# MichaelAxtmann/InPlaceMSDradixsort

Measured on AMD Instinct MI355X. Metric: Gkeys/s + achieved HBM GB/s, 2^30 uniform u32 keys, 1/2/4/8 MI355X, higher is better.
Workload: dtype u32; 1 GPU; 2^30 uniform u32 keys per GPU, in-place MSD radix sort, 8-bit digits; config_id=c2, elements_per_gpu=1073741824, steps_verified=0, verified_by=not checked in a plain run (bench.py --full verifies every timed step), workspace_bytes=360054784

## Files before the change

### inplacemsdradixsort_amd/csrc/msd_device.hpp

```cpp
#pragma once

#include <hip/hip_runtime.h>
#include <stdint.h>

namespace msd {

constexpr int kP = 256;
constexpr uint32_t kXBase = 0x80000000u;
constexpr uint32_t kNoOwner = 0xFFFFFFFFu;
constexpr uint32_t kRposStride = 32;

struct NoVal {};
typedef uint32_t u32x4 __attribute__((ext_vector_type(4)));

template <typename V> struct has_val { static constexpr bool value = true; };
template <> struct has_val<NoVal> { static constexpr bool value = false; };

template <typename K, typename V> struct Cfg;
template <> struct Cfg<uint32_t, NoVal> {
	static constexpr int B = 64, T = 4096, TH = 1024;
	static constexpr int SORT_TH = 1024, SORT_KPT = 24;
};
template <> struct Cfg<uint64_t, NoVal> {
	static constexpr int B = 32, T = 4096, TH = 1024;
	static constexpr int SORT_TH = 1024, SORT_KPT = 17;
};
template <> struct Cfg<uint64_t, uint64_t> {
	static constexpr int B = 32, T = 2048, TH = 1024;
#ifndef MSD_PAIR_LEAF_TH
#define MSD_PAIR_LEAF_TH 512
#endif
	static constexpr int SORT_TH = MSD_PAIR_LEAF_TH, SORT_KPT = 6;
};

struct Parent {
	uint64_t start, count;
	uint32_t shift;
	uint32_t width;
	uint32_t child_base;
	uint32_t stripe_lo, stripe_hi;
	uint32_t pad;
};

struct Stripe {
	uint64_t begin, end;
	uint64_t lo_base;
	uint32_t parent;
	uint32_t slot_lo, slot_hi;
	uint32_t pad;
};

struct Segment {
	uint64_t start, count;
	uint32_t bits;
	uint32_t pad;
};

struct ListEntry {
	uint32_t slot;
	uint32_t owner;
};

struct Counters {
	uint32_t nholes;
	uint32_t hole_cursor;
	uint32_t next_parents;
	uint32_t nsmall;
	uint32_t errors;
	uint32_t chain_steps;
	uint32_t ncount;
	uint32_t nfallback;
	uint32_t nbig;
	uint32_t count_ticket;
	uint32_t direct_uneven;
	uint32_t nslow;
	uint32_t count_ticket2;
	uint32_t nevict;
	uint32_t leaf_ticket[2];
	uint32_t count_ticket3;
	uint32_t nslow16;
	uint32_t next_max;
	uint32_t rp_children;
	uint32_t nhot;
	uint32_t nslow2;
	uint32_t count_ticket4;
	uint32_t l17_slow;
	uint32_t err_sites;
	uint32_t nexcess;
};
__device__ __forceinline__ void msd_note_error(Counters *ctr, uint32_t site)
{
	atomicAdd(&ctr->errors, 1u);
	atomicOr(&ctr->err_sites, 1u << site);
}
static_assert(sizeof(Counters) % 8 == 0, "the words behind the counters are used for 64-bit atomics");

#ifdef MSD_STAMPS
__device__ unsigned long long g_stamps[2][16];
#define MSD_STAMP_DECL(id)                          \
	constexpr bool kStampThis = MSD_STAMPS == (id); \
	unsigned long long st_acc[12] = {}, st_last = 0
#define MSD_STAMP_START()                                                                              \
	do {                                                                                            \
		if constexpr (kStampThis) {                                                             \
			__builtin_amdgcn_sched_barrier(0);                                              \
			asm volatile("s_memtime %0\n\ts_waitcnt lgkmcnt(0)" : "=s"(st_last)::"memory"); \
			__builtin_amdgcn_sched_barrier(0);                                              \
		}                                                                                       \
	} while (0)
#define MSD_STAMP(i)                                                                                    \
	do {                                                                                            \
		if constexpr (kStampThis) {                                                             \
			unsigned long long now_;                                                        \
			__builtin_amdgcn_sched_barrier(0);                                              \
			asm volatile("s_memtime %0\n\ts_waitcnt lgkmcnt(0)" : "=s"(now_)::"memory");    \
			__builtin_amdgcn_sched_barrier(0);                                              \
			st_acc[i] += now_ - st_last;                                                    \
			st_last = now_;                                                                 \
		}                                                                                       \
	} while (0)
#define MSD_STAMP_TICK(i)                            \
	do {                                         \
		if constexpr (kStampThis) st_acc[i] += 1; \
	} while (0)
#define MSD_STAMP_FLUSH(nwaves)                                                                         \
	do {                                                                                            \
		if constexpr (kStampThis) {                                                             \
			const unsigned wv_ = threadIdx.x >> 6;                                          \
			if ((threadIdx.x & 63) == 0 && (wv_ == 0 || wv_ == (nwaves) - 1)) {            \
				for (int i_ = 0; i_ < 12; ++i_) atomicAdd(&g_stamps[wv_ ? 1 : 0][i_], st_acc[i_]); \
			}                                                                               \
		}                                                                                       \
	} while (0)
#else
#define MSD_STAMP_DECL(id)
#define MSD_STAMP_START() do {} while (0)
#define MSD_STAMP(i) do {} while (0)
#define MSD_STAMP_TICK(i) do {} while (0)
#define MSD_STAMP_FLUSH(nwaves) do {} while (0)
#endif


template <typename K> __device__ __forceinline__ uint32_t digit_of(K key, uint32_t shift, uint32_t mask)
{
	return (uint32_t)(key >> shift) & mask;
}

__device__ __forceinline__ uint32_t lane_id() { return threadIdx.x & 63; }

__device__ __forceinline__ uint32_t wave_incl_scan(uint32_t v)
{
	v += (uint32_t)__builtin_amdgcn_update_dpp(0, (int)v, 0x111, 0xf, 0xf, false);
	v += (uint32_t)__builtin_amdgcn_update_dpp(0, (int)v, 0x112, 0xf, 0xf, false);
	v += (uint32_t)__builtin_amdgcn_update_dpp(0, (int)v, 0x114, 0xf, 0xf, false);
	v += (uint32_t)__builtin_amdgcn_update_dpp(0, (int)v, 0x118, 0xf, 0xf, false);
	v += (uint32_t)__builtin_amdgcn_update_dpp(0, (int)v, 0x142, 0xa, 0xf, false);
	v += (uint32_t)__builtin_amdgcn_update_dpp(0, (int)v, 0x143, 0xc, 0xf, false);
	return v;
}
__device__ __forceinline__ uint64_t wave_incl_scan64(uint64_t v)
{
#pragma unroll
	for (int o = 1; o < 64; o <<= 1) {
		uint64_t t = __shfl_up(v, o);
		if ((int)lane_id() >= o) v += t;
	}
	return v;
}

__device__ __forceinline__ uint32_t popc_below_lane(uint64_t m)
{
	return __builtin_amdgcn_mbcnt_hi((uint32_t)(m >> 32), __builtin_amdgcn_mbcnt_lo((uint32_t)m, 0u));
}
__device__ __forceinline__ bool lane_bit(uint64_t m)
{
	const uint32_t lane = threadIdx.x & 63u;
	const uint32_t half = lane < 32u ? (uint32_t)m : (uint32_t)(m >> 32);
	return (half >> (lane & 31u)) & 1u;
}

__device__ __forceinline__ uint32_t block_excl_scan256(uint32_t v, uint32_t *tmp, uint32_t &total)
{
	const uint32_t tid = threadIdx.x;
	if (tid >= 256) v = 0;
	uint32_t inc = wave_incl_scan(v);
	if (tid < 256 && lane_id() == 63) tmp[tid >> 6] = inc;
	__syncthreads();
	uint32_t base = 0;
	if (tid < 256) {
		const uint32_t w = tid >> 6;
		if (w > 0) base += tmp[0];
		if (w > 1) base += tmp[1];
		if (w > 2) base += tmp[2];
	}
	total = tmp[0] + tmp[1] + tmp[2] + tmp[3];
	__syncthreads();
	return base + inc - v;
}
__device__ __forceinline__ uint64_t block_excl_scan256_64(uint64_t v, uint64_t *tmp, uint64_t &total)
{
	const uint32_t tid = threadIdx.x;
	if (tid >= 256) v = 0;
	uint64_t inc = wave_incl_scan64(v);
	if (tid < 256 && lane_id() == 63) tmp[tid >> 6] = inc;
	__syncthreads();
	uint64_t base = 0;
	if (tid < 256) {
		const uint32_t w = tid >> 6;
		if (w > 0) base += tmp[0];
		if (w > 1) base += tmp[1];
		if (w > 2) base += tmp[2];
	}
	total = tmp[0] + tmp[1] + tmp[2] + tmp[3];
	__syncthreads();
	return base + inc - v;
}

template <typename K> struct Vec16;
template <> struct Vec16<uint32_t> { static constexpr int N = 4; };
template <> struct Vec16<uint64_t> { static constexpr int N = 2; };


struct DirectPlan {
	uint32_t est_cnt[kP];
	uint32_t bound[kP + 1];
	uint32_t adj_seen, adj_same;
};

template <typename K>
__global__ __launch_bounds__(256) void direct_sample_kernel(const K *__restrict__ keys, const Parent *__restrict__ parents,
	DirectPlan *__restrict__ plan, uint32_t every)
{
	__shared__ uint32_t h[kP];
	const Parent pa = parents[0];
	const uint32_t mask = (1u << pa.width) - 1u;
	h[threadIdx.x] = 0;
	uint32_t seen = 0, same = 0;
	__syncthreads();
	const uint64_t nruns = pa.count / 256;
	const uint64_t step = (uint64_t)gridDim.x * every;
	for (uint64_t r = (uint64_t)blockIdx.x * every; r < nruns; r += 4 * step) {
		K k4[4];
#pragma unroll
		for (int u = 0; u < 4; ++u)
			if (r + u * step < nruns) k4[u] = keys[pa.start + (r + u * step) * 256 + threadIdx.x];
#pragma unroll
		for (int u = 0; u < 4; ++u) {
			if (r + u * step < nruns) {
				const uint32_t d = digit_of(k4[u], pa.shift, mask);
				atomicAdd(&h[d], 1u);
				if (u == 0 && (blockIdx.x & 7u) == 0) {
					same += __popcll(__ballot(d == (uint32_t)__shfl_down((int)d, 1) && (threadIdx.x & 63) != 63));
					seen += 63;
				}
			}
		}
	}
	__syncthreads();
	if (h[threadIdx.x]) atomicAdd(&plan->est_cnt[threadIdx.x], h[threadIdx.x]);
	if ((threadIdx.x & 63) == 0 && seen) {
		atomicAdd(&plan->adj_seen, seen);
		atomicAdd(&plan->adj_same, same);
	}
}

template <typename K>
__global__ __launch_bounds__(1024) void direct_hist_kernel(const K *__restrict__ keys, const Stripe *__restrict__ stripes,
	const Parent *__restrict__ parents, DirectPlan *__restrict__ plans,
	unsigned long long *__restrict__ vres)
{
	constexpr int VEC = Vec16<K>::N;
	K v_or = 0, v_and = ~(K)0;
	auto seen_key = [&](K k) {
		v_or |= k;
		v_and &= k;
		return k;
	};
	__shared__ uint32_t h[kP];
	const Stripe st = stripes[blockIdx.x];
	const Parent pa = parents[st.parent];
	const uint32_t shift = pa.shift, mask = (1u << pa.width) - 1u, tid = threadIdx.x;
	if (tid < kP) h[tid] = 0;
	uint32_t seen = 0, same = 0;
	__syncthreads();
	const uint64_t a0 = (st.begin + VEC - 1) / VEC * VEC, a1 = st.end / VEC * VEC;
	if (a0 < a1) {
		for (uint64_t i = st.begin + tid; i < a0; i += 1024) atomicAdd(&h[digit_of(seen_key(keys[i]), shift, mask)], 1u);
		const uint32_t nvec = (uint32_t)((a1 - a0) / VEC);
		const K *kp = keys + a0;
		constexpr int U = 8;
		for (uint32_t v = tid; v < nvec; v += U * 1024) {
			K kk[U][VEC];
#pragma unroll
			for (int u = 0; u < U; ++u) {
				const uint32_t vv = min(v + (uint32_t)u * 1024u, nvec - 1u);
				if constexpr (sizeof(K) == 4) {
					const u32x4 q = __builtin_nontemporal_load(reinterpret_cast<const u32x4 *>(kp + (size_t)vv * VEC));
					kk[u][0] = q.x; kk[u][1] = q.y; kk[u][2] = q.z; kk[u][3] = q.w;
				} else {
					const u32x4 q = __builtin_nontemporal_load(reinterpret_cast<const u32x4 *>(kp + (size_t)vv * VEC));
					kk[u][0] = (K)q.x | ((K)q.y << 32); kk[u][1] = (K)q.z | ((K)q.w << 32);
				}
			}
#pragma unroll
			for (int u = 0; u < U; ++u) {
				if (v + (uint32_t)u * 1024u < nvec) {
#pragma unroll
					for (int e = 0; e < VEC; ++e) atomicAdd(&h[digit_of(seen_key(kk[u][e]), shift, mask)], 1u);
					seen += 1;
					same += digit_of(kk[u][0], shift, mask) == digit_of(kk[u][VEC - 1], shift, mask) ? 1u : 0u;
				}
			}
		}
		for (uint64_t i = a1 + tid; i < st.end; i += 1024) atomicAdd(&h[digit_of(seen_key(keys[i]), shift, mask)], 1u);
	} else
		for (uint64_t i = st.begin + tid; i < st.end; i += 1024) atomicAdd(&h[digit_of(seen_key(keys[i]), shift, mask)], 1u);
	__syncthreads();
	if (tid < kP && h[tid]) atomicAdd(&plans[st.parent].est_cnt[tid], h[tid]);
	if (vres) {
		unsigned long long o = (unsigned long long)v_or, a = (unsigned long long)v_and | (sizeof(K) == 4 ? 0xFFFFFFFF00000000ull : 0ull);
#pragma unroll
		for (int s = 32; s > 0; s >>= 1) {
			o |= __shfl_xor(o, s);
			a &= __shfl_xor(a, s);
		}
		if ((tid & 63) == 0) {
			atomicOr(&vres[0], o);
			atomicAnd(&vres[1], a);
		}
	}
#pragma unroll
	for (int o = 32; o > 0; o >>= 1) {
		seen += (uint32_t)__shfl_xor((int)seen, o);
		same += (uint32_t)__shfl_xor((int)same, o);
	}
	if ((tid & 63) == 0 && seen) {
		atomicAdd(&plans[st.parent].adj_seen, seen);
		atomicAdd(&plans[st.parent].adj_same, same);
	}
}

template <int B>
__global__ __launch_bounds__(256) void direct_plan_kernel(const Parent *__restrict__ parents, DirectPlan *__restrict__ plans,
	Counters *__restrict__ ctr)
{
	__shared__ uint64_t tmp[8];
	__shared__ uint32_t s_mn, s_mx;
	const Parent pa = parents[blockIdx.x];
	DirectPlan *plan = plans + blockIdx.x;
	const uint32_t d = threadIdx.x;
	if (d == 0) {
		s_mn = 0xFFFFFFFFu;
		s_mx = 0;
	}
	const uint64_t s0 = (pa.start + B - 1) / B, s1 = (pa.start + pa.count) / B;
	uint64_t total;
	const uint64_t c = plan->est_cnt[d];
	const uint64_t ex = block_excl_scan256_64(c, tmp, total);
	const uint64_t ns = s1 > s0 ? s1 - s0 : 0;
	plan->bound[d] = (uint32_t)(s0 + (total ? ex * ns / total : (uint64_t)d * ns / kP));
	if (d == 0) plan->bound[kP] = (uint32_t)s1;
	if (d < (1u << pa.width)) {
		atomicMin(&s_mn, (uint32_t)c);
		atomicMax(&s_mx, (uint32_t)c);
	}
	__syncthreads();
	const bool runs = (uint64_t)plan->adj_same * 8u > plan->adj_seen;
#ifndef MSD_UNEVEN_PCT
#define MSD_UNEVEN_PCT 125
#endif
	if (d == 0 && (runs || !(s_mn > 0 && (double)s_mx * 100.0 <= (double)MSD_UNEVEN_PCT * (double)s_mn))) atomicAdd(&ctr->direct_uneven, 1u);
}

__device__ __forceinline__ bool wave_select_smallest(uint32_t v, bool elig, int need, uint64_t &mask_out)
{
	uint64_t cand = __ballot(elig), selm = 0;
	if ((int)__popcll(cand) > need) {
#pragma unroll
		for (int bit = 9; bit >= 0; --bit) {
			const uint64_t zeros = cand & ~__ballot((v >> bit) & 1u);
			const int cz = __popcll(zeros);
			if (cz >= need)
				cand = zeros;
			else {
				selm |= zeros;
				need -= cz;
				cand &= ~zeros;
			}
		}
		const bool mine = lane_bit(cand) && (int)popc_below_lane(cand) < need;
		selm |= __ballot(mine);
	} else
		selm = cand;
	mask_out = selm;
	return lane_bit(selm);
}

}
#include "msd_direct.hpp"
#include "msd_stream2.hpp"
namespace msd {


struct ChildArrays {
	uint64_t *start;
	uint64_t *count;
// ... 615 lines not shown
		for (int i = 0; i < NI; ++i) {
			const int chain = i * BPI + (int)(lane / LPB);
			const uint32_t s = __shfl(src_safe, chain);
			kd[i] = *reinterpret_cast<const u32x4 *>(slot_ptr<K, B>(keys, xkeys, s) + sub * VEC);
			if constexpr (HV)
				vd[i] = *reinterpret_cast<const u32x4 *>(slot_ptr<uint64_t, B>(vals, xvals, s) + sub * VEC);
		}
#pragma unroll
		for (int i = 0; i < NI; ++i) {
			const int chain = i * BPI + (int)(lane / LPB);
			const uint32_t hdst = __shfl(hole, chain);
			if ((mv >> chain) & 1ull) {
				*reinterpret_cast<u32x4 *>(slot_ptr<K, B>(keys, xkeys, hdst) + sub * VEC) = kd[i];
				if constexpr (HV)
					*reinterpret_cast<u32x4 *>(slot_ptr<uint64_t, B>(vals, xvals, hdst) + sub * VEC) = vd[i];
			}
		}
		if (active && !retry) {
			if (last)
				active = false;
			else {
				hole = src;
				owner = src_owner;
				om = nom;
				ofl = nfl;
			}
		}
		MSD_STAMP(4);
	}
	MSD_STAMP_FLUSH(4);
	if (lane == 0 && steps) atomicAdd(&ctr->chain_steps, steps);
}

__device__ __forceinline__ void chains_verify(const ChildArrays &ca, uint32_t ci, uint32_t flags, Counters *ctr)
{
	const uint32_t len = (uint32_t)ca.list_len[ci], hot = flags >> 8;
	if (!hot) {
		if (ca.rpos[(size_t)ci * kRposStride] != len) msd_note_error(ctr, 3u);
		return;
	}
	const uint32_t nint = ca.n_int[ci];
	for (uint32_t sh = 0; sh < kHotShards; ++sh) {
		const uint32_t sb = (uint32_t)((uint64_t)nint * sh / kHotShards), se = (uint32_t)((uint64_t)nint * (sh + 1) / kHotShards);
		if (ca.hot_cur[(size_t)((hot - 1) * kHotShards + sh) * kRposStride] < se - sb) msd_note_error(ctr, 4u);
	}
	if (ca.rpos[(size_t)ci * kRposStride] != len - nint) msd_note_error(ctr, 5u);
}


template <int B>
__device__ __forceinline__ uint64_t fringe_pos(uint64_t start, uint32_t is, uint32_t I, uint64_t o)
{
	if (I == 0) return start + o;
	const uint64_t head = (uint64_t)is * B - start;
	return o < head ? start + o : (uint64_t)(is + I) * B + (o - head);
}

template <typename K, typename V>
__global__ __launch_bounds__(256) void cleanup_kernel(const Stripe *__restrict__ stripes,
	const Parent *__restrict__ parents, const uint32_t *__restrict__ lo_cnt,
	const uint32_t *__restrict__ lo_off, const uint32_t *__restrict__ lo_dst, ChildArrays ca,
	const K *__restrict__ lo_keys, const uint64_t *__restrict__ lo_vals,
	K *__restrict__ keys, uint64_t *__restrict__ vals,
	const K *__restrict__ xkeys, const uint64_t *__restrict__ xvals, Counters *__restrict__ ctr)
{
	constexpr int B = Cfg<K, V>::B;
	constexpr bool HV = has_val<V>::value;
	__shared__ uint32_t s_off[kP + 1], s_dst[kP], s_is[kP], s_I[kP], s_ex[kP], s_nex;
	__shared__ uint64_t s_start[kP];
	const Stripe st = stripes[blockIdx.x];
	const Parent pa = parents[st.parent];
	const uint32_t tid = threadIdx.x, W = 1u << pa.width;
	const bool first = blockIdx.x == pa.stripe_lo;
	const size_t so = (size_t)blockIdx.x * kP + tid;
	s_off[tid] = lo_off[so];
	s_dst[tid] = lo_dst[so];
	if (tid == kP - 1) s_off[kP] = lo_off[so] + lo_cnt[so];
	if (tid == 0) s_nex = 0;
	if (tid < W) {
		s_is[tid] = ca.is[pa.child_base + tid];
		s_I[tid] = ca.I[pa.child_base + tid];
		s_start[tid] = ca.start[pa.child_base + tid];
	}
	__syncthreads();
	if (first && tid < W) {
		const uint32_t fl = ca.flags[pa.child_base + tid];
		chains_verify(ca, pa.child_base + tid, fl, ctr);
		if (fl & 2u) s_ex[atomicAdd(&s_nex, 1u)] = tid;
	}
	{
		constexpr uint32_t LG = 32, NB = 4, NG = 256 / LG;
		const uint32_t grp = tid / LG, l = tid % LG;
		for (uint32_t d0 = grp; d0 < kP; d0 += NG * NB) {
			K k[NB];
			uint64_t v[NB];
			uint32_t off[NB], cnt[NB];
#pragma unroll
			for (uint32_t q = 0; q < NB; ++q) {
				const uint32_t d = d0 + q * NG;
				off[q] = s_off[d];
				cnt[q] = s_off[d + 1] - off[q];
				if (l < cnt[q]) {
					k[q] = lo_keys[st.lo_base + off[q] + l];
					if constexpr (HV) v[q] = lo_vals[st.lo_base + off[q] + l];
				}
			}
#pragma unroll
			for (uint32_t q = 0; q < NB; ++q) {
				const uint32_t d = d0 + q * NG;
				if (l < cnt[q]) {
					const uint64_t p = fringe_pos<B>(s_start[d], s_is[d], s_I[d], (uint64_t)s_dst[d] + l);
					keys[p] = k[q];
					if constexpr (HV) vals[p] = v[q];
				}
			}
#pragma unroll
			for (uint32_t q = 0; q < NB; ++q) {
				const uint32_t d = d0 + q * NG;
				for (uint32_t j = l + LG; j < cnt[q]; j += LG) {
					const uint64_t p = fringe_pos<B>(s_start[d], s_is[d], s_I[d], (uint64_t)s_dst[d] + j);
					keys[p] = lo_keys[st.lo_base + off[q] + j];
					if constexpr (HV) vals[p] = lo_vals[st.lo_base + off[q] + j];
				}
			}
		}
		static_assert(kP % (NG * NB) == 0, "every bucket has its half-wave");
	}
	if (!first) return;
	__syncthreads();
	const uint32_t nex = s_nex;
	if (tid == 0 && nex) atomicAdd(&ctr->nexcess, nex);
	for (uint32_t e = tid / B; e < nex; e += 256 / B) {
		const uint32_t d = s_ex[e], ci = pa.child_base + d, j = tid % B;
		const uint64_t p = fringe_pos<B>(s_start[d], s_is[d], s_I[d], (uint64_t)ca.lsum[ci] + j);
		keys[p] = xkeys[(uint64_t)(2 * ci + 1) * B + j];
		if constexpr (HV) vals[p] = xvals[(uint64_t)(2 * ci + 1) * B + j];
	}
}

enum Route : int { kRouteDone = -1, kRouteSmall = 0, kRouteCount = 1, kRouteBig = 2, kRouteNext = 3 };
__host__ __device__ inline Route route_child(uint64_t count, uint32_t bits, uint32_t stop_bits, uint32_t count_bits, uint64_t small_max,
	uint64_t med_max, bool has_big)
{
	if (count <= 1 || bits <= stop_bits) return kRouteDone;
	const bool countable = bits <= count_bits;
	if (countable && count >= 64 && count <= med_max) return kRouteCount;
	if (count > small_max) return has_big && countable && count < 0xFFFF0000ull ? kRouteBig : kRouteNext;
	return kRouteSmall;
}

__global__ __launch_bounds__(256) void collect_kernel(const Parent *__restrict__ parents, uint32_t nparents, uint32_t wmax, ChildArrays ca,
	uint64_t small_max, uint64_t med_max, uint32_t small_cap, uint32_t count_bits, Segment *__restrict__ next_parents,
	Segment *__restrict__ small, Segment *__restrict__ small_count, Segment *__restrict__ big, uint32_t big_cap,
	Counters *__restrict__ ctr, uint64_t *__restrict__ count_out, uint32_t count_n, uint32_t stop_bits)
{
	__shared__ uint32_t s_n[4], s_base[4], s_max;
	const uint32_t tid = threadIdx.x;
	if (tid < 4) s_n[tid] = 0;
	if (tid == 0) s_max = 0;
	__syncthreads();
	const uint32_t pi = blockIdx.x * (256u >> wmax) + (tid >> wmax), d = tid & ((1u << wmax) - 1u);
	int which = -1;
	uint32_t rank = 0;
	Segment s = {};
	if (pi < nparents) {
		const Parent pa = parents[pi];
		if (d < (1u << pa.width)) {
			const uint32_t ci = pa.child_base + d;
			const uint64_t c = ca.count[ci];
			if (count_out && ci < count_n) count_out[ci] = c;
			which = route_child(c, pa.shift, stop_bits, count_bits, small_max, med_max, big != nullptr);
			if (which >= 0) {
				s.start = ca.start[ci];
				s.count = c;
				s.bits = pa.shift;
				s.pad = 0;
				rank = atomicAdd(&s_n[which], 1u);
				if (which == 3) atomicMax(&s_max, (uint32_t)(c < 0xFFFFFFFFull ? c : 0xFFFFFFFFull));
			}
		}
	}
	__syncthreads();
	if (tid < 4 && s_n[tid]) {
		uint32_t *cnt = tid == 0 ? &ctr->nsmall : tid == 1 ? &ctr->ncount : tid == 2 ? &ctr->nbig : &ctr->next_parents;
		s_base[tid] = atomicAdd(cnt, s_n[tid]);
		if (tid == 3) atomicMax(&ctr->next_max, s_max);
	}
	__syncthreads();
	if (which < 0) return;
	uint32_t at = s_base[which] + rank;
	if (which == 2 && at >= big_cap) {
		which = 3;
		at = atomicAdd(&ctr->next_parents, 1u);
		atomicMax(&ctr->next_max, (uint32_t)(s.count < 0xFFFFFFFFull ? s.count : 0xFFFFFFFFull));
	}
	if (which == 3)
		next_parents[at] = s;
	else if (which == 2)
		big[at] = s;
	else if (at < small_cap)
		(which == 0 ? small : small_count)[at] = s;
	else
		msd_note_error(ctr, 6u);
}

}
#include "msd_regpart.hpp"
namespace msd {


constexpr int kCountTh = 1024;
constexpr int kCountMaxBits = 16;
#ifndef MSD_COUNT_MED_LOG
#define MSD_COUNT_MED_LOG 17
#endif
constexpr uint64_t kCountMedMax = 1ull << MSD_COUNT_MED_LOG;
constexpr size_t kCountCwBytes = (((size_t)1 << kCountMaxBits) / 4 + ((size_t)1 << kCountMaxBits) / 128 + 4) * 4;
constexpr int kCountStageBytes = 14080;
constexpr size_t kCountLds = kCountCwBytes + kCountStageBytes + 128;
__device__ __forceinline__ uint32_t cw_at(uint32_t i) { return i + (i >> 5); }

template <typename K>
__global__ __launch_bounds__(kCountTh, 8) void count_place_kernel(K *__restrict__ keys,
	const Segment *__restrict__ segs, uint32_t nsegs_host, const uint32_t *__restrict__ nsegs_dev,
	Segment *__restrict__ slow, Counters *__restrict__ ctr)
{
	const uint32_t nsegs = nsegs_dev ? *nsegs_dev : nsegs_host;
	constexpr int PF = sizeof(K) == 4 ? 17 : 9;
	extern __shared__ __attribute__((aligned(16))) unsigned char smem[];
	uint32_t *cw = reinterpret_cast<uint32_t *>(smem);
	uint32_t *tbase = reinterpret_cast<uint32_t *>(smem + kCountCwBytes);
	K *out = reinterpret_cast<K *>(smem);
	uint32_t *wtot = reinterpret_cast<uint32_t *>(smem + kCountCwBytes + kCountStageBytes);
	uint32_t *nexti = wtot + 17;
	K *hi_l = reinterpret_cast<K *>(wtot + 18);
	uint32_t *crowded = wtot + 21;
	static_assert((size_t)PF * kCountTh * sizeof(K) <= kCountCwBytes + kCountStageBytes, "output buffer");
	const uint32_t tid = threadIdx.x, lane = tid & 63, w = tid >> 6;
	if (blockIdx.x >= nsegs) return;
	Segment sg = segs[blockIdx.x];
	K pk[PF];
	auto prefetch = [&](const Segment &g) {
		const K *src = keys + g.start;
		const uint32_t cnt = g.count <= (uint64_t)(PF * kCountTh) ? (uint32_t)g.count : 1u;
#pragma unroll
		for (int u = 0; u < PF; ++u) {
			const uint32_t idx = min((uint32_t)(u * kCountTh) + tid, cnt - 1u);
			pk[u] = src[idx];
		}
	};
	prefetch(sg);
	MSD_STAMP_DECL(2);
	MSD_STAMP_START();
	for (;;) {
		const uint32_t n = (uint32_t)sg.count;
		const uint32_t nv = 1u << sg.bits, mask = nv - 1u;
		const uint32_t nwords = nv >= 4 ? nv / 4 : 1;
		K *seg = keys + sg.start;
		const bool in_regs = n <= (uint32_t)(PF * kCountTh);
		MSD_STAMP(9);
		MSD_STAMP_TICK(11);

		if (in_regs)
			for (uint32_t j = tid; j < cw_at(nwords) + 1; j += kCountTh) cw[j] = 0;
		if (tid == 0) {
			*nexti = atomicAdd(&ctr->count_ticket, 1u) + gridDim.x;
			*crowded = 0;
			*hi_l = pk[0] & ~(K)mask;
		}
		MSD_STAMP(0);
		__syncthreads();
		MSD_STAMP(1);
		uint32_t rk[PF];
		if (in_regs) {
#pragma unroll
			for (int u = 0; u < PF; ++u) {
				const uint32_t left = n > (uint32_t)(u * kCountTh) ? n - u * kCountTh : 0u;
				rk[u] = 0;
				if (tid < left) {
					const uint32_t v = (uint32_t)pk[u] & mask, sh = (v & 3u) * 8u;
					rk[u] = v | (((atomicAdd(&cw[cw_at(v >> 2)], 1u << sh) >> sh) & 0xFFu) << 16);
				}
			}
		}
		MSD_STAMP(2);
		__syncthreads();
		MSD_STAMP(3);
		const uint32_t nxt = *nexti;
		const K hi = *hi_l;
		const uint32_t wpt = nwords >= kCountTh ? nwords / kCountTh : 1;
		const uint32_t w0 = tid * wpt;
		uint32_t *cww = cw + cw_at(w0);
		uint32_t tot = 0;
		if (in_regs && w0 < nwords) {
#pragma unroll 4
			for (uint32_t j = 0; j < wpt; ++j) tot = __builtin_amdgcn_sad_u8(cww[j], 0u, tot);
		}
		if (tot > 255u) *crowded = 1;
		const uint32_t inc = wave_incl_scan(tot);
		if (lane == 63) wtot[w] = inc;
		MSD_STAMP(4);
		__syncthreads();
		uint32_t pos = inc - tot, all = 0;
#pragma unroll 2
		for (uint32_t ww = 0; ww < kCountTh / 64; ++ww) {
			const uint32_t t = wtot[ww];
			if (ww < w) pos += t;
			all += t;
		}
		const bool ok = in_regs && all == n && *crowded == 0;
		MSD_STAMP(5);
		if (ok) {
			uint32_t run = 0;
			if (w0 < nwords) {
#pragma unroll 4
				for (uint32_t j = 0; j < wpt; ++j) {
					const uint32_t x = cww[j], y = x * 0x01010101u;
					cww[j] = (y - x) + run * 0x01010101u;
					run += y >> 24;
				}
			}
			tbase[tid] = pos;
			MSD_STAMP(6);
			__syncthreads();
			const uint32_t lgw = (uint32_t)__builtin_ctz(wpt);
#pragma unroll
			for (int u = 0; u < PF; ++u) {
				const uint32_t left = n > (uint32_t)(u * kCountTh) ? n - u * kCountTh : 0u;
				if (tid < left) {
					const uint32_t v = rk[u] & 0xFFFFu, wi = v >> 2;
					rk[u] += (tbase[wi >> lgw] + ((cw[cw_at(wi)] >> ((v & 3u) * 8u)) & 0xFFu)) << 16;
				}
			}
			MSD_STAMP(7);
			__syncthreads();
#pragma unroll
			for (int u = 0; u < PF; ++u) {
				const uint32_t left = n > (uint32_t)(u * kCountTh) ? n - u * kCountTh : 0u;
				if (tid < left) out[rk[u] >> 16] = hi | (K)(rk[u] & 0xFFFFu);
			}
			__syncthreads();
			MSD_STAMP(8);
		} else if (tid == 0)
			slow[atomicAdd(&ctr->nslow, 1u)] = sg;
		Segment nsg = sg;
		if (nxt < nsegs) {
			nsg = segs[nxt];
			prefetch(nsg);
		}
		if (ok) {
			for (uint32_t i = tid; i < n; i += kCountTh) seg[i] = out[i];
		}
		MSD_STAMP(10);
		if (nxt >= nsegs) break;
		sg = nsg;
		__syncthreads();
	}
	MSD_STAMP_FLUSH(kCountTh / 64);
}

template <typename K>
__global__ __launch_bounds__(kCountTh, 8) void count_walk_kernel(K *__restrict__ keys,
	const Segment *__restrict__ segs, const uint32_t *__restrict__ nsegs_dev, Segment *__restrict__ fallback,
	uint32_t fallback_base, uint32_t lds_cap, Segment *__restrict__ big, uint32_t big_cap, Counters *__restrict__ ctr)
{
	constexpr uint32_t WS = kCountStageBytes / sizeof(K);
	extern __shared__ __attribute__((aligned(16))) unsigned char smem[];
	uint32_t *cw = reinterpret_cast<uint32_t *>(smem);
	K *stage = reinterpret_cast<K *>(smem + kCountCwBytes);
	uint32_t *wtot = reinterpret_cast<uint32_t *>(smem + kCountCwBytes + kCountStageBytes);
	uint32_t *nexti = wtot + 17;
	K *hi_l = reinterpret_cast<K *>(wtot + 18);
	uint32_t *tfree = wtot + 20;
	const uint32_t tid = threadIdx.x, lane = tid & 63, w = tid >> 6;
	const uint32_t nsegs = *nsegs_dev;
	if (blockIdx.x >= nsegs) return;
	Segment sg = segs[blockIdx.x];
	for (;;) {
		const uint32_t n = (uint32_t)sg.count;
		const uint32_t nv = 1u << sg.bits, mask = nv - 1u;
		const uint32_t nwords = nv >= 4 ? nv / 4 : 1;
		K *seg = keys + sg.start;

		for (uint32_t j = tid; j < cw_at(nwords) + 1; j += kCountTh) cw[j] = 0;
		if (tid == 0) {
			*nexti = atomicAdd(&ctr->count_ticket2, 1u) + gridDim.x;
			*hi_l = seg[0] & ~(K)mask;
		}
		__syncthreads();
		constexpr int LB = 16 / (int)sizeof(K) * 4;
		for (uint32_t i0 = 0; i0 < n; i0 += LB * kCountTh) {
			K kb[LB];
#pragma unroll
			for (int u = 0; u < LB; ++u) kb[u] = seg[min(i0 + u * kCountTh + tid, n - 1u)];
#pragma unroll
			for (int u = 0; u < LB; ++u) {
				if (i0 + u * kCountTh + tid < n) {
					const uint32_t v = (uint32_t)kb[u] & mask;
					atomicAdd(&cw[cw_at(v >> 2)], 1u << ((v & 3u) * 8u));
				}
			}
		}
		__syncthreads();
		const uint32_t nxt = *nexti;
		const K hi = *hi_l;
		const uint32_t wpt = nwords >= kCountTh ? nwords / kCountTh : 1;
		const uint32_t w0 = tid * wpt;
		const uint32_t *cwp = cw + cw_at(w0);
		uint32_t tot = 0;
		uint64_t nz = 0;
		if (w0 < nwords) {
#pragma unroll 4
			for (uint32_t j = 0; j < wpt; ++j) {
				const uint32_t x = cwp[j];
				tot = __builtin_amdgcn_sad_u8(x, 0u, tot);
				const uint32_t hb = (x | ((x & 0x7F7F7F7Fu) + 0x7F7F7F7Fu)) & 0x80808080u;
				nz |= (uint64_t)((((hb >> 7) * 0x01020408u) >> 24) & 0xFu) << (4u * j);
			}
		}
		const uint32_t inc = wave_incl_scan(tot);
		if (lane == 63) wtot[w] = inc;
		__syncthreads();
		uint32_t pos = inc - tot, all = 0;
#pragma unroll 2
		for (uint32_t ww = 0; ww < kCountTh / 64; ++ww) {
			const uint32_t t = wtot[ww];
			if (ww < w) pos += t;
			all += t;
		}
		if (all != n) {
			if (tid == 0) {
				if (n <= lds_cap) {
					const uint32_t at = atomicAdd(&ctr->nfallback, 1u);
					fallback[fallback_base + at] = sg;
				} else {
					const uint32_t at = big ? atomicAdd(&ctr->nbig, 1u) : 0xFFFFFFFFu;
					if (at < big_cap) big[at] = sg; else msd_note_error(ctr, 7u);
				}
			}
		} else {
			const uint32_t end = pos + tot;
			const K hi4 = hi | (K)(w0 * 4u);
			uint32_t c = 0;
			K cur = 0;
			K *cwk = reinterpret_cast<K *>(cw);
			auto window = [&](uint32_t wbeg, uint32_t wend) -> uint32_t {
				if (pos <= wend && wend < end) *tfree = tid;
				while (pos < end && pos < wend) {
					if (c == 0) {
						const uint32_t i = (uint32_t)__ffsll((long long)nz) - 1u;
						nz &= nz - 1;
						c = (cwp[i >> 2] >> (8u * (i & 3u))) & 0xFFu;
						cur = hi4 + (K)i;
					}
					const uint32_t r = pos - wbeg;
					if (r < WS) stage[r]= cur; else cwk[r - WS] = cur;
					++pos;
					--c;
				}
				__syncthreads();
				const uint32_t tf = *tfree;
				for (uint32_t i = tid; i < wend - wbeg; i += kCountTh) seg[wbeg + i] = i < WS ? stage[i] : cwk[i - WS];
				__syncthreads();
				return (uint32_t)(cw_at(tf * wpt) * 4u / sizeof(K));
			};
			uint32_t wbeg = 0, wend = WS < n ? WS : n;
			for (;;) {
				const uint32_t room = window(wbeg, wend);
				if (wend >= n) break;
				wbeg = wend;
				wend = wbeg + WS + room < n ? wbeg + WS + room : n;
			}
		}
		if (nxt >= nsegs) break;
		sg = segs[nxt];
		__syncthreads();
	}
}

}
#include "msd_count16.hpp"
#include "msd_merge16.hpp"
#include "msd_scatter16.hpp"
namespace msd {


constexpr int kLeafCountBits = 14;
template <typename K, typename V> struct LeafBits {
	static constexpr int value = (sizeof(K) == 8 && (!has_val<V>::value || Cfg<K, V>::SORT_TH < 1024)) ? 13 : kLeafCountBits;
};
template <typename K, typename V> struct LeafCountLds {
	static constexpr int CAP = Cfg<K, V>::SORT_TH * Cfg<K, V>::SORT_KPT;
	static constexpr size_t bytes = (size_t)CAP * (sizeof(K) + (has_val<V>::value ? 8 : 0)) +
					((size_t)1 << LeafBits<K, V>::value) * 2 + 192;
};

template <typename K, typename V>
__global__ __launch_bounds__((Cfg<K, V>::SORT_TH)) void leaf_count_sort_kernel(K *__restrict__ keys,
	uint64_t *__restrict__ vals, const Segment *__restrict__ segs, uint32_t nsegs,
	Segment *__restrict__ fallback, Counters *__restrict__ ctr, uint32_t *__restrict__ ticket,
	const uint32_t *__restrict__ nsegs_dev)
{
	if (nsegs_dev) nsegs = *nsegs_dev;
	using C = Cfg<K, V>;
	constexpr bool HV = has_val<V>::value;
	constexpr int TH = C::SORT_TH, KPT = C::SORT_KPT, CAP = TH * KPT, LB = LeafBits<K, V>::value;
	extern __shared__ __attribute__((aligned(16))) unsigned char smem[];
	K *xk = reinterpret_cast<K *>(smem);
	uint64_t *xv = reinterpret_cast<uint64_t *>(smem + (size_t)CAP * sizeof(K));
	uint32_t *cw = reinterpret_cast<uint32_t *>(smem + (size_t)CAP * (sizeof(K) + (HV ? 8 : 0)));
	uint32_t *wtot = cw + ((size_t)1 << LB) / 2;
	K *s_or = reinterpret_cast<K *>(wtot + 32);
	if (blockIdx.x >= nsegs) return;
	const uint32_t tid = threadIdx.x, lane = tid & 63, w = tid >> 6;
	Segment sg = segs[blockIdx.x];
	K kr[KPT];
	uint64_t vr[HV ? KPT : 1];
	auto prefetch = [&](const Segment &g) {
		const uint32_t cnt = (uint32_t)g.count;
#pragma unroll
		for (int i = 0; i < KPT; ++i) {
			if ((uint32_t)(i * TH) < cnt) {
				const uint32_t idx = min((uint32_t)(i * TH) + tid, cnt - 1u);
				kr[i] = keys[g.start + idx];
				if constexpr (HV) vr[i] = vals[g.start + idx];
			}
		}
	};
	prefetch(sg);
	if (tid == 0) wtot[19] = 0;
	MSD_STAMP_DECL(3);
	MSD_STAMP_START();
	for (;;) {
		MSD_STAMP(9);
		MSD_STAMP_TICK(11);
		const uint32_t n = (uint32_t)sg.count;
#ifndef MSD_LEAF_NARROW
#define MSD_LEAF_NARROW 1
#endif
		const bool narrow = MSD_LEAF_NARROW && sg.bits <= (uint32_t)LB;
		K k_or = 0, k_and = ~(K)0;
		if (!narrow) {
#pragma unroll
			for (int i = 0; i < KPT; ++i) {
				if ((uint32_t)(i * TH) + tid < n) {
					k_or |= kr[i];
					k_and &= kr[i];
				}
			}
		}
		if (tid == 0) {
			s_or[0] = 0;
			s_or[1] = ~(K)0;
			wtot[16] = 0;
			if (wtot[19] == 0) {
				const uint32_t take = nsegs > 64u * gridDim.x ? 4u : 1u;
				wtot[18] = atomicAdd(ticket, take) + gridDim.x;
				wtot[19] = take;
			}
			wtot[17] = wtot[18];
			wtot[18] += 1;
			wtot[19] -= 1;
		}
		for (uint32_t j = tid; j < ((uint32_t)1 << LB) / 2; j += TH) cw[j] = 0;
		MSD_STAMP(0);
		__syncthreads();
		if (!narrow) {
#pragma unroll
			for (int o = 32; o > 0; o >>= 1) {
				k_or |= __shfl_xor(k_or, o);
				k_and &= __shfl_xor(k_and, o);
			}
			if (lane == 0) {
				if constexpr (sizeof(K) == 4) {
					atomicOr(reinterpret_cast<unsigned int *>(&s_or[0]), (unsigned int)k_or);
					atomicAnd(reinterpret_cast<unsigned int *>(&s_or[1]), (unsigned int)k_and);
				} else {
					atomicOr(reinterpret_cast<unsigned long long *>(&s_or[0]), (unsigned long long)k_or);
					atomicAnd(reinterpret_cast<unsigned long long *>(&s_or[1]), (unsigned long long)k_and);
				}
			}
			__syncthreads();
		}
		MSD_STAMP(1);
		const uint32_t nxt = wtot[17];
		const Segment nraw = segs[nxt < nsegs ? nxt : blockIdx.x];
		const K openmask = sg.bits >= sizeof(K) * 8 ? ~(K)0 : (((K)1 << sg.bits) - 1);
		const K vopen = narrow ? openmask : (s_or[0] ^ s_or[1]) & openmask;
		Segment nsg = sg;
		bool fetched = false;
		if (vopen != 0) {
			const uint32_t nbits = (uint32_t)(64 - __builtin_clzll((unsigned long long)vopen));
			const uint32_t shift = nbits > (uint32_t)LB ? nbits - LB : 0;
			const uint32_t mask = (1u << (nbits - shift)) - 1u;
			uint32_t rk[KPT];
#pragma unroll
			for (int i = 0; i < KPT; ++i) {
				rk[i] = 0;
				if ((uint32_t)(i * TH) + tid < n) {
					const uint32_t v = (uint32_t)(kr[i] >> shift) & mask, sh = 16u * (v & 1u);
					rk[i] = (atomicAdd(&cw[v >> 1], 1u << sh) >> sh) & 0xFFFFu;
				}
			}
			MSD_STAMP(2);
			__syncthreads();
			constexpr uint32_t WPT = (((uint32_t)1 << LB) / 2) / TH;
			static_assert(WPT >= 1, "counter words per thread");
			const uint32_t w0 = tid * WPT;
			uint32_t tot = 0;
#pragma unroll
			for (uint32_t j = 0; j < WPT; ++j) {
				const uint32_t x = cw[w0 + j];
				tot += (x & 0xFFFFu) + (x >> 16);
			}
			const uint32_t inc = wave_incl_scan(tot);
			if (lane == 63) wtot[w] = inc;
			__syncthreads();
			uint32_t run = inc - tot;
			for (uint32_t ww = 0; ww < w; ++ww) run += wtot[ww];
#pragma unroll
			for (uint32_t j = 0; j < WPT; ++j) {
				const uint32_t x = cw[w0 + j];
				const uint32_t lo = x & 0xFFFFu, hi = x >> 16;
				cw[w0 + j] = run | ((run + lo) << 16);
				run += lo + hi;
			}
			MSD_STAMP(3);
			__syncthreads();
#pragma unroll
			for (int i = 0; i < KPT; ++i) {
				if ((uint32_t)(i * TH) + tid < n) {
					const uint32_t v = (uint32_t)(kr[i] >> shift) & mask;
					const uint32_t p = ((cw[v >> 1] >> (16u * (v & 1u))) & 0xFFFFu) + rk[i];
					xk[p] = kr[i];
					if constexpr (HV) xv[p] = vr[i];
				}
			}
			MSD_STAMP(4);
			if (nxt < nsegs) {
				nsg = nraw;
				prefetch(nsg);
				fetched = true;
			}
			MSD_STAMP(5);
			__syncthreads();
			bool bad = false;
			const K lowmask = shift ? ((K)1 << shift) - 1 : (K)0;
			const bool groups = shift && (vopen & lowmask) != 0;
			constexpr uint32_t kMaxGroup = 48;
			const K glim = (K)1 << shift;
			if (groups) {
				bool too_long = false;
				for (uint32_t i = tid; i + kMaxGroup < n; i += TH)
					if ((K)(xk[i] ^ xk[i + kMaxGroup]) < glim) too_long = true;
				if (too_long) wtot[16] = 1;
				__syncthreads();
				bad = wtot[16] != 0;
				if (bad && tid == 0) fallback[atomicAdd(&ctr->nfallback, 1u)] = sg;
			}
			MSD_STAMP(6);
			if (!bad && groups) {
				constexpr uint32_t WIN = 3;
#pragma unroll 1
				for (uint32_t idx = tid; idx < n; idx += TH) {
					const K me = xk[idx];
					K lk[WIN], rkk[WIN];
#pragma unroll
					for (uint32_t d = 0; d < WIN; ++d) {
						lk[d] = xk[idx > d ? idx - d - 1 : 0u];
						rkk[d] = xk[min(idx + d + 1, n - 1u)];
					}
					uint32_t left = 0, before = 0, right = 0;
					bool ml = true, mr = true;
#pragma unroll
					for (uint32_t d = 0; d < WIN; ++d) {
						ml = ml && idx > d && (K)(lk[d] ^ me) < glim;
						before += ml && lk[d] <= me ? 1u : 0u;
						left += ml ? 1u : 0u;
						mr = mr && idx + d + 1 < n && (K)(rkk[d] ^ me) < glim;
						before += mr && rkk[d] < me ? 1u : 0u;
						right += mr ? 1u : 0u;
					}
					if (ml) {
						while (idx > left) {
							const K o = xk[idx - left - 1];
							if ((K)(o ^ me) >= glim) break;
							before += o <= me ? 1u : 0u;
							++left;
						}
					}
					if (mr) {
						for (uint32_t e = idx + right + 1; e < n; ++e) {
							const K o = xk[e];
							if ((K)(o ^ me) >= glim) break;
							before += o < me ? 1u : 0u;
						}
					}
					const uint64_t at = sg.start + idx - left + before;
					keys[at] = me;
					if constexpr (HV) vals[at] = xv[idx];
				}
			} else if (!bad) {
				for (uint32_t idx = tid; idx < n; idx += TH) {
					keys[sg.start + idx] = xk[idx];
					if constexpr (HV) vals[sg.start + idx] = xv[idx];
				}
			}
		}
		MSD_STAMP(7);
		if (nxt >= nsegs) break;
		if (!fetched) {
			nsg = nraw;
			prefetch(nsg);
		}
		sg = nsg;
		__syncthreads();
	}
	MSD_STAMP_FLUSH(TH / 64);
}

}
#include "msd_leaf17.hpp"
#include "msd_bigcount.hpp"
namespace msd {

__global__ __launch_bounds__(256) void round_init_kernel(Counters *__restrict__ ctr, uint32_t *__restrict__ plan_words,
	uint64_t nplan_words, unsigned long long *__restrict__ scan_state, uint64_t ntiles, uint32_t *__restrict__ scan_ctr,
	const uint32_t *__restrict__ staged, uint32_t *__restrict__ parents_out, uint64_t parent_words,
	uint32_t *__restrict__ stripes_out, uint64_t stripe_words, Counters *__restrict__ park)
{
	const uint64_t i0 = (uint64_t)blockIdx.x * 256 + threadIdx.x, step = (uint64_t)gridDim.x * 256;
	if (i0 == 0) {
		if (park) *park = *ctr;
		ctr->nholes = 0;
		ctr->hole_cursor = 0;
		ctr->next_parents = 0;
		ctr->nevict = 0;
		ctr->direct_uneven = 0;
		ctr->next_max = 0;
		ctr->rp_children = 0;
		ctr->nhot = 0;
		scan_ctr[0] = scan_ctr[1] = scan_ctr[2] = scan_ctr[3] = 0;
	}
	for (uint64_t i = i0; i < nplan_words; i += step) plan_words[i] = 0;
	for (uint64_t i = i0; i < ntiles; i += step) scan_state[i] = 0;
	if (staged) {
		for (uint64_t i = i0; i < parent_words; i += step) parents_out[i] = staged[i];
		for (uint64_t i = i0; i < stripe_words; i += step) stripes_out[i] = staged[parent_words + i];
	}
}


template <typename K, typename V>
__global__ __launch_bounds__((Cfg<K, V>::SORT_TH)) void lds_sort_kernel(K *__restrict__ keys,
	uint64_t *__restrict__ vals, const Segment *__restrict__ segs, uint32_t nsegs,
	const uint32_t *__restrict__ nsegs_dev)
{
	using C = Cfg<K, V>;
	constexpr bool HV = has_val<V>::value;
	constexpr int TH = C::SORT_TH, KPT = C::SORT_KPT, NW = TH / 64, CAP = TH * KPT;
	if (nsegs_dev) nsegs = *nsegs_dev;
	for (uint32_t sgi = blockIdx.x; sgi < nsegs; sgi += gridDim.x) {
	__syncthreads();
	extern __shared__ __attribute__((aligned(16))) unsigned char smem[];
	K *xk = reinterpret_cast<K *>(smem);
	uint64_t *xv = reinterpret_cast<uint64_t *>(smem + (size_t)CAP * sizeof(K));
	uint32_t *wcnt = reinterpret_cast<uint32_t *>(smem + (size_t)CAP * sizeof(K) + (HV ? (size_t)CAP * 8 : 0));
	uint32_t *dbase = wcnt + NW * kP;
	uint32_t *tmp = dbase + kP;
	K *s_or = reinterpret_cast<K *>(tmp + 8);

	const Segment sg = segs[sgi];
	const uint32_t n = (uint32_t)sg.count;
	const uint32_t tid = threadIdx.x, lane = tid & 63, w = tid >> 6;
	const int nitems = (int)((n + TH - 1) / TH);
	const uint32_t wbase = w * (uint32_t)nitems * 64;
	const uint64_t lt_mask = (1ull << lane) - 1ull;

	K kr[KPT];
	uint64_t vr[HV ? KPT : 1];
	K k_or = 0, k_and = ~(K)0;
#pragma unroll
	for (int i = 0; i < KPT; ++i) {
		kr[i] = ~(K)0;
		if constexpr (HV) vr[i] = 0;
		if (i < nitems) {
			const uint32_t idx = wbase + i * 64 + lane;
			if (idx < n) {
				kr[i] = keys[sg.start + idx];
				if constexpr (HV) vr[i] = vals[sg.start + idx];
				k_or |= kr[i];
				k_and &= kr[i];
			}
		}
	}
	if (tid == 0) { s_or[0] = 0; s_or[1] = ~(K)0; }
	__syncthreads();
#pragma unroll
	for (int o = 32; o > 0; o >>= 1) {
		k_or |= __shfl_xor(k_or, o);
		k_and &= __shfl_xor(k_and, o);
	}
	if (lane == 0) {
		if constexpr (sizeof(K) == 4) {
			atomicOr(reinterpret_cast<unsigned int *>(&s_or[0]), (unsigned int)k_or);
			atomicAnd(reinterpret_cast<unsigned int *>(&s_or[1]), (unsigned int)k_and);
		} else {
			atomicOr(reinterpret_cast<unsigned long long *>(&s_or[0]), (unsigned long long)k_or);
			atomicAnd(reinterpret_cast<unsigned long long *>(&s_or[1]), (unsigned long long)k_and);
		}
	}
	__syncthreads();
	const K vary = s_or[0] ^ s_or[1];
	__syncthreads();

	uint32_t *mycnt = wcnt + w * kP;
	bool in_lds = false;
	const K openmask = sg.bits >= sizeof(K) * 8 ? ~(K)0 : (((K)1 << sg.bits) - 1);
	const K vopen = vary & openmask;
	const uint32_t nbits = vopen ? (uint32_t)(64 - __builtin_clzll((unsigned long long)vopen)) : 0u;
	const uint32_t first_shift = nbits > 24 ? nbits - 16 : 0;
	bool msd_mode = first_shift != 0;
	for (uint32_t shift = first_shift; shift < nbits; shift += 8) {
		const uint32_t width = nbits - shift < 8 ? nbits - shift : 8;
		const uint32_t mask = (1u << width) - 1u;
		if (((uint32_t)(vary >> shift) & mask) == 0) continue;
		for (uint32_t j = tid; j < NW * kP; j += TH) wcnt[j] = 0;
		__syncthreads();
		uint32_t rk[(KPT + 1) / 2];
#pragma unroll
		for (int i = 0; i < KPT; ++i) {
			if (i < nitems) {
				const uint32_t d = digit_of(kr[i], shift, mask);
				uint32_t plo = ~0u, phi = ~0u;
#pragma unroll
				for (int b = 0; b < 8; ++b) {
					const uint32_t bit = (d >> b) & 1u;
					const uint64_t m = __ballot(bit != 0);
					const uint32_t ext = bit - 1u;
					plo &= (uint32_t)m ^ ext;
					phi &= (uint32_t)(m >> 32) ^ ext;
				}
				const uint32_t below = __popc(plo & (uint32_t)lt_mask) + __popc(phi & (uint32_t)(lt_mask >> 32));
				const uint32_t old = mycnt[d];
				if (below == 0) mycnt[d] = old + __popc(plo) + __popc(phi);
				const uint32_t r = old + below;
				if (i & 1) rk[i / 2] |= r << 16; else rk[i / 2] = r;
			}
			__builtin_amdgcn_sched_barrier(0);
		}
		__syncthreads();
		uint32_t tot_d = 0;
		if (tid < kP) {
#pragma unroll
			for (int ww = 0; ww < NW; ++ww) {
				const uint32_t t = wcnt[ww * kP + tid];
				wcnt[ww * kP + tid] = tot_d;
				tot_d += t;
			}
		}
		uint32_t gt;
		const uint32_t ex = block_excl_scan256(tot_d, tmp, gt);
		if (tid < kP) dbase[tid] = ex;
		__syncthreads();
#pragma unroll
		for (int i = 0; i < KPT; ++i) {
			if (i < nitems) {
				const uint32_t d = digit_of(kr[i], shift, mask);
				const uint32_t r = (i & 1) ? rk[i / 2] >> 16 : rk[i / 2] & 0xFFFFu;
				const uint32_t p = dbase[d] + mycnt[d] + r;
				xk[p] = kr[i];
				if constexpr (HV) xv[p] = vr[i];
			}
		}
		__syncthreads();
		in_lds = true;
		bool more = false;
		for (uint32_t s2 = shift + 8; s2 < nbits; s2 += 8) {
			const uint32_t w2 = nbits - s2 < 8 ? nbits - s2 : 8;
			if (((uint32_t)(vary >> s2) & ((1u << w2) - 1u)) != 0) more = true;
		}
		if (!more && msd_mode) {
			const K lowmask = ((K)1 << first_shift) - 1;
			if (tid == 0) tmp[0] = 0;
			__syncthreads();
			bool too_long = false;
			if ((vary & lowmask) != 0) {
				for (uint32_t i = tid; i < n; i += TH) {
					const K hi = xk[i] >> first_shift;
					if ((i == 0 || (xk[i - 1] >> first_shift) != hi) && i + 1 < n && (xk[i + 1] >> first_shift) == hi) {
						uint32_t e = i + 2;
						while (e < n && (xk[e] >> first_shift) == hi) ++e;
						if (e - i > 48) {
							too_long = true;
// ... 61 lines not shown
	const uint32_t parts = 1u << radix_bits, mask = parts - 1u;
	for (uint32_t j = threadIdx.x; j < parts; j += 256) h[j] = 0;
	__syncthreads();
	constexpr int VEC = Vec16<K>::N;
	const uint64_t nvec = n / VEC;
	const uint64_t stride = (uint64_t)gridDim.x * 256;
	for (uint64_t v = (uint64_t)blockIdx.x * 256 + threadIdx.x; v < nvec; v += stride) {
		if constexpr (sizeof(K) == 4) {
			const uint4 q = reinterpret_cast<const uint4 *>(keys)[v];
			atomicAdd(&h[(q.x >> shift) & mask], 1u);
			atomicAdd(&h[(q.y >> shift) & mask], 1u);
			atomicAdd(&h[(q.z >> shift) & mask], 1u);
			atomicAdd(&h[(q.w >> shift) & mask], 1u);
		} else {
			const ulonglong2 q = reinterpret_cast<const ulonglong2 *>(keys)[v];
			atomicAdd(&h[(uint32_t)(q.x >> shift) & mask], 1u);
			atomicAdd(&h[(uint32_t)(q.y >> shift) & mask], 1u);
		}
	}
	if (blockIdx.x == 0)
		for (uint64_t i = nvec * VEC + threadIdx.x; i < n; i += 256)
			atomicAdd(&h[(uint32_t)(keys[i] >> shift) & mask], 1u);
	__syncthreads();
	for (uint32_t j = threadIdx.x; j < parts; j += 256)
		if (h[j]) atomicAdd(&count[j], (unsigned long long)h[j]);
}


constexpr int kScanTh = 256, kScanIpt = 8, kScanTile = kScanTh * kScanIpt;
constexpr uint64_t kFlagAgg = 1ull << 62, kFlagPre = 2ull << 62, kFlagMask = 3ull << 62;

__global__ __launch_bounds__(kScanTh) void scan_lookback_kernel(const uint64_t *__restrict__ in,
	uint64_t *__restrict__ out, uint64_t n, unsigned long long *__restrict__ tile_state,
	uint32_t *__restrict__ tile_counter, uint32_t *__restrict__ err)
{
	__shared__ uint64_t tmp[8];
	__shared__ uint32_t s_tile;
	__shared__ uint64_t s_prefix;
	const uint32_t tid = threadIdx.x;
	if (tid == 0) s_tile = atomicAdd(tile_counter, 1u);
	__syncthreads();
	const uint32_t tile = s_tile;
	const uint64_t base = (uint64_t)tile * kScanTile + (uint64_t)tid * kScanIpt;
	uint64_t v[kScanIpt], sum = 0;
#pragma unroll
	for (int i = 0; i < kScanIpt; ++i) {
		v[i] = base + i < n ? in[base + i] : 0;
		sum += v[i];
	}
	uint64_t agg;
	const uint64_t tex = block_excl_scan256_64(sum, tmp, agg);
	if (tid == 0) {
		uint64_t prefix = 0;
		if (tile == 0) {
			__hip_atomic_store(&tile_state[0], kFlagPre | agg, __ATOMIC_RELAXED, __HIP_MEMORY_SCOPE_AGENT);
		} else {
			__hip_atomic_store(&tile_state[tile], kFlagAgg | agg, __ATOMIC_RELAXED, __HIP_MEMORY_SCOPE_AGENT);
			uint32_t t = tile - 1;
			uint32_t spins = 0;
			for (;;) {
				const uint64_t s = __hip_atomic_load(&tile_state[t], __ATOMIC_RELAXED, __HIP_MEMORY_SCOPE_AGENT);
				const uint64_t f = s & kFlagMask;
				if (f == 0) {
					if (++spins > (1u << 26)) {
						atomicAdd(err, 1u);
						break;
					}
					__builtin_amdgcn_s_sleep(1);
					continue;
				}
				prefix += s & ~kFlagMask;
				if (f == kFlagPre) break;
				--t;
			}
			__hip_atomic_store(&tile_state[tile], kFlagPre | (prefix + agg), __ATOMIC_RELAXED, __HIP_MEMORY_SCOPE_AGENT);
		}
		s_prefix = prefix;
	}
	__syncthreads();
	uint64_t run = s_prefix + tex;
#pragma unroll
	for (int i = 0; i < kScanIpt; ++i) {
		if (base + i < n) out[base + i] = run;
		run += v[i];
	}
}


struct GatherRun {
	uint64_t src, dst, len;
	uint32_t first_chunk;
	uint32_t pad;
};
#ifndef MSD_GATHER_CHUNK
#define MSD_GATHER_CHUNK 2048
#endif
constexpr uint32_t kGatherChunk = MSD_GATHER_CHUNK;

template <typename K>
__global__ __launch_bounds__(256) void gather_runs_kernel(K *__restrict__ dst, const K *__restrict__ src,
	const GatherRun *__restrict__ runs, uint32_t nruns, uint32_t nchunks, const uint32_t *__restrict__ coarse)
{
	constexpr int VEC = 16 / (int)sizeof(K);
	for (uint32_t c = blockIdx.x; c < nchunks; c += gridDim.x) {
		uint32_t lo = coarse[c >> 6], hi = min(coarse[(c >> 6) + 1] + 1u, nruns);
		while (hi - lo > 1) {
			const uint32_t mid = (lo + hi) >> 1;
			if (runs[mid].first_chunk <= c) lo = mid; else hi = mid;
		}
		const GatherRun r = runs[lo];
		const uint64_t off = (uint64_t)(c - r.first_chunk) * kGatherChunk;
		const uint32_t len = (uint32_t)(r.len - off < (uint64_t)kGatherChunk ? r.len - off : (uint64_t)kGatherChunk);
		K *d = dst + r.dst + off;
		const K *s = src + r.src + off;
		const uint32_t lead = min(len, (uint32_t)((VEC - (int)(((uintptr_t)d / sizeof(K)) % VEC)) % VEC));
		const uint32_t nvec = (len - lead) / VEC, tail0 = lead + nvec * VEC;
		if (threadIdx.x < lead) d[threadIdx.x] = s[threadIdx.x];
		if (tail0 + threadIdx.x < len) d[tail0 + threadIdx.x] = s[tail0 + threadIdx.x];
		const uint32_t kw = (uint32_t)(((uintptr_t)(s + lead) & 15u) >> 2);
		const u32x4 *sa = reinterpret_cast<const u32x4 *>(reinterpret_cast<const unsigned char *>(s + lead) - 4u * kw);
		u32x4 *dv = reinterpret_cast<u32x4 *>(d + lead);
		const bool last_lane = (threadIdx.x & 63u) == 63u;
#ifndef MSD_GATHER_NF
#define MSD_GATHER_NF 2
#endif
		constexpr int NF = MSD_GATHER_NF;
		for (uint32_t q0 = 0; q0 < nvec; q0 += NF * 256) {
			const uint32_t q = q0 + threadIdx.x;
			u32x4 a[NF], nx[NF];
#pragma unroll
			for (int u = 0; u < NF; ++u) {
				const uint32_t qq = min(q + u * 256u, kw ? nvec : nvec - 1u);
				a[u] = sa[qq];
				if (kw && last_lane) nx[u] = sa[min(qq + 1u, nvec)];
			}
#pragma unroll
			for (int u = 0; u < NF; ++u) {
				u32x4 o = a[u];
				if (kw) {
					const uint32_t sx = (uint32_t)__shfl_down((int)a[u].x, 1), sy = (uint32_t)__shfl_down((int)a[u].y, 1),
						       sz = (uint32_t)__shfl_down((int)a[u].z, 1);
					const uint32_t bx = last_lane ? nx[u].x : sx, by = last_lane ? nx[u].y : sy, bz = last_lane ? nx[u].z : sz;
					o = kw == 1 ? u32x4{ a[u].y, a[u].z, a[u].w, bx } : kw == 2 ? u32x4{ a[u].z, a[u].w, bx, by } : u32x4{ a[u].w, bx, by, bz };
				}
				if (q + u * 256u < nvec) dv[q + u * 256u] = o;
			}
		}
	}
}


template <typename K>
__global__ __launch_bounds__(256) void vary_kernel(const K *__restrict__ keys, uint64_t n, uint64_t stride,
	unsigned long long *__restrict__ res)
{
	K o = 0, a = ~(K)0;
	const uint64_t cnt = (n + stride - 1) / stride;
	const uint64_t step = (uint64_t)gridDim.x * 256, t0 = (uint64_t)blockIdx.x * 256 + threadIdx.x;
	if (stride == 1) {
		constexpr int VEC = 16 / (int)sizeof(K);
		const uint64_t lead = min(n, (uint64_t)((VEC - (int)(((uintptr_t)keys / sizeof(K)) % VEC)) % VEC));
		const uint64_t nvec = (n - lead) / VEC;
		const u32x4 *v = reinterpret_cast<const u32x4 *>(keys + lead);
		auto take = [&](const u32x4 &q) {
			if constexpr (sizeof(K) == 4) {
				o |= (K)(q.x | q.y | q.z | q.w);
				a &= (K)(q.x & q.y & q.z & q.w);
			} else {
				const K k0 = (K)q.x | ((K)q.y << 32), k1 = (K)q.z | ((K)q.w << 32);
				o |= k0 | k1;
				a &= k0 & k1;
			}
		};
		uint64_t i = t0;
		for (; i + 3 * step < nvec; i += 4 * step) {
			const u32x4 q0 = __builtin_nontemporal_load(v + i), q1 = __builtin_nontemporal_load(v + i + step);
			const u32x4 q2 = __builtin_nontemporal_load(v + i + 2 * step), q3 = __builtin_nontemporal_load(v + i + 3 * step);
			take(q0); take(q1); take(q2); take(q3);
		}
		for (; i < nvec; i += step) take(__builtin_nontemporal_load(v + i));
		const uint64_t tail0 = lead + nvec * VEC;
		if (t0 < lead) {
			o |= keys[t0];
			a &= keys[t0];
		}
		if (tail0 + t0 < n) {
			o |= keys[tail0 + t0];
			a &= keys[tail0 + t0];
		}
	} else
		for (uint64_t i = t0; i < cnt; i += step) {
			const K k = keys[i * stride];
			o |= k;
			a &= k;
		}
#pragma unroll
	for (int s = 32; s > 0; s >>= 1) {
		o |= __shfl_xor(o, s);
		a &= __shfl_xor(a, s);
	}
	if (lane_id() == 0) {
		atomicOr(&res[0], (unsigned long long)o);
		atomicAnd(&res[1], (unsigned long long)a | (sizeof(K) == 4 ? 0xFFFFFFFF00000000ull : 0ull));
	}
}


struct CheckResult {
	unsigned long long violations, sum, xr;
};

template <typename K>
__global__ __launch_bounds__(256) void check_kernel(const K *__restrict__ keys, const uint64_t *__restrict__ rids,
	uint64_t n, CheckResult *__restrict__ res)
{
	unsigned long long bad = 0, sum = 0, xr = 0;
	const uint64_t stride = (uint64_t)gridDim.x * 256;
	for (uint64_t i = (uint64_t)blockIdx.x * 256 + threadIdx.x; i < n; i += stride) {
		const K k = keys[i];
		if (i > 0 && k < keys[i - 1]) ++bad;
		if (rids && rids[i] != (uint64_t)k) ++bad;
		sum += (unsigned long long)k;
		xr ^= (unsigned long long)k;
	}
#pragma unroll
	for (int o = 32; o > 0; o >>= 1) {
		bad += __shfl_xor(bad, o);
		sum += __shfl_xor(sum, o);
		xr ^= __shfl_xor(xr, o);
	}
	if (lane_id() == 0) {
		if (bad) atomicAdd(&res->violations, bad);
		atomicAdd(&res->sum, sum);
		atomicXor(&res->xr, xr);
	}
}


__device__ __forceinline__ uint64_t splitmix64(uint64_t x)
{
	x += 0x9E3779B97F4A7C15ull;
	uint64_t z = (x ^ (x >> 30)) * 0xBF58476D1CE4E5B9ull;
	z = (z ^ (z >> 27)) * 0x94D049BB133111EBull;
	return z ^ (z >> 31);
}

__global__ void gen_uniform_u32_kernel(uint32_t *out, uint64_t n, uint64_t seed)
{
	const uint64_t stride = (uint64_t)gridDim.x * blockDim.x;
	for (uint64_t i = (uint64_t)blockIdx.x * blockDim.x + threadIdx.x; i < n; i += stride)
		out[i] = (uint32_t)(splitmix64(seed + i) >> 32);
}
__global__ void gen_uniform_u64_kernel(uint64_t *out, uint64_t n, uint64_t seed, int shr)
{
	const uint64_t stride = (uint64_t)gridDim.x * blockDim.x;
	for (uint64_t i = (uint64_t)blockIdx.x * blockDim.x + threadIdx.x; i < n; i += stride)
		out[i] = splitmix64(seed + i) >> shr;
}
__global__ void gen_zipf_u32_kernel(uint32_t *out, uint64_t n, uint64_t seed)
{
	const double U = 4294967296.0;
	const double lnU1 = log(U + 1.0);
	const uint64_t stride = (uint64_t)gridDim.x * blockDim.x;
	for (uint64_t i = (uint64_t)blockIdx.x * blockDim.x + threadIdx.x; i < n; i += stride) {
		const double u = (double)(splitmix64(seed + i) >> 11) * 0x1.0p-53;
		double r = floor(exp(u * lnU1));
		r = r < 1.0 ? 1.0 : (r > U ? U : r);
		out[i] = (uint32_t)((uint64_t)r - 1);
	}
}
__global__ void gen_iota_u64_kernel(uint64_t *out, uint64_t n, uint64_t first)
{
	const uint64_t stride = (uint64_t)gridDim.x * blockDim.x;
	for (uint64_t i = (uint64_t)blockIdx.x * blockDim.x + threadIdx.x; i < n; i += stride)
		out[i] = first + i;
}

__global__ void gen_dup_u32_kernel(uint32_t *out, uint64_t n, uint64_t seed, uint64_t distinct)
{
	const uint64_t stride = (uint64_t)gridDim.x * blockDim.x;
	for (uint64_t i = (uint64_t)blockIdx.x * blockDim.x + threadIdx.x; i < n; i += stride)
		out[i] = (uint32_t)(splitmix64((splitmix64(seed + i) % distinct) ^ 0xD0B1E5ull) >> 32);
}

__global__ __launch_bounds__(320) void gen_mt19937_64_kernel(uint64_t *out, uint64_t n, uint64_t seed, int shr)
{
	__shared__ uint64_t st[313];
	const uint32_t t = threadIdx.x;
	if (t == 0) {
		st[0] = seed;
		for (uint32_t i = 0; i != 311; ++i) st[i + 1] = 6364136223846793005ull * (st[i] ^ (st[i] >> 62)) + i + 1;
	}
	__syncthreads();
	auto twist = [](uint64_t a, uint64_t b, uint64_t far) -> uint64_t {
		const uint64_t x = (a & 0xffffffff80000000ull) | (b & 0x7fffffffull);
		return far ^ (x >> 1) ^ (0xb5026f5aa96619e9ull & (0ull - (x & 1ull)));
	};
	for (uint64_t base = 0; base < n; base += 312) {
		uint64_t v = 0;
		if (t < 156) v = twist(st[t], st[t + 1], st[t + 156]);
		__syncthreads();
		if (t < 156) st[t] = v;
		__syncthreads();
		if (t >= 156 && t < 312) v = twist(st[t], t == 311 ? st[0] : st[t + 1], st[t - 156]);
		__syncthreads();
		if (t >= 156 && t < 312) st[t] = v;
		__syncthreads();
		if (t < 312 && base + t < n) {
			uint64_t x = st[t];
			x ^= (x >> 29) & 0x5555555555555555ull;
			x ^= (x << 17) & 0x71d67fffeda60000ull;
			x ^= (x << 37) & 0xfff7eee000000000ull;
			x ^= (x >> 43);
			out[base + t] = x >> shr;
		}
	}
}


template <typename K>
__global__ __launch_bounds__(256) void sample_kernel(const K *__restrict__ keys, uint64_t n, uint64_t m, uint64_t seed,
	K *__restrict__ out)
{
	const uint64_t stride = (uint64_t)gridDim.x * blockDim.x;
	for (uint64_t i = (uint64_t)blockIdx.x * blockDim.x + threadIdx.x; i < m; i += stride)
		out[i] = keys[__umul64hi(splitmix64(seed + i), n)];
}

template <typename K>
__global__ __launch_bounds__(256) void splitters_kernel(const K *__restrict__ sample, uint64_t m, uint32_t parts, K *__restrict__ delim)
{
	const uint32_t i = blockIdx.x * blockDim.x + threadIdx.x;
	if (i + 1 >= parts) return;
	const double pct = __ddiv_rn((double)m, (double)parts);
	const uint64_t idx = (uint64_t)__dsub_rn(__dmul_rn(pct, (double)(i + 1)), 0.001);
	K v = sample[idx];
	uint64_t lo = 0, hi = idx;
	while (lo < hi) {
		const uint64_t mid = (lo + hi) >> 1;
		if (sample[mid] < v) lo = mid + 1; else hi = mid;
	}
	const uint64_t start = lo ? lo - 1 : 0;
	uint64_t lo2 = idx, hi2 = m;
	while (lo2 < hi2) {
		const uint64_t mid = (lo2 + hi2) >> 1;
		if (sample[mid] <= v) lo2 = mid + 1; else hi2 = mid;
	}
	if (idx - start < lo2 - idx && v) --v;
	delim[i] = v;
}

}
```

### inplacemsdradixsort_amd/csrc/msd_radix.hip

```cpp
#include "msd_device.hpp"
#include "msd_select.hpp"
#include "msd_select_rows.hpp"
#include "msd_reverse.hpp"
#include "msd_sort_rows.hpp"
#include "msd_runs.hpp"
#include "msd_reduce.hpp"
#include "msd_search.hpp"
#include "msd_merge2.hpp"
#include "msd_setops.hpp"
#include "msd_args.hpp"
#include "../../include/msd_radix_hip.h"
#include "../../include/msd_sort_keys_hip.h"
#include "../../include/msd_sort_rows_hip.h"
#include "../../include/msd_runs_hip.h"
#include "../../include/msd_reduce_hip.h"
#include "../../include/msd_search_hip.h"
#include "../../include/msd_merge_hip.h"
#include "../../include/msd_setops_hip.h"

#include <algorithm>
#include <cstdarg>
#include <cstdio>
#include <cstring>
#include <initializer_list>
#include <string>
#include <type_traits>
#include <vector>

using namespace msd;

#define MSD_VERSION "inplacemsdradixsort_amd 0.2 (gfx950)"

struct PhaseRec {
	const char *name;
	hipEvent_t ev;
};

struct msd_ctx {
	int device = 0;
	hipStream_t stream = nullptr;
	char *slab = nullptr;
	size_t slab_bytes = 0;
	char *keep = nullptr;
	size_t keep_bytes = 0;
	Segment *lists = nullptr;
	size_t lists_cap = 0;
	void *pinned = nullptr;
	size_t pinned_bytes = 0;
	hipEvent_t ev_early = nullptr;
	std::string err;
	bool profiling = false;
	hipEvent_t ev_start = nullptr;
	std::vector<PhaseRec> phases;
	std::vector<hipEvent_t> ev_pool;
	size_t ev_used = 0;
	std::vector<std::pair<std::string, double>> phase_us;
	std::vector<std::pair<std::string, uint64_t>> stats;
	int sm_count = 256;
	int chains_per_cu[3] = { 4, 4, 2 };
	int direct_mode = 1;
	uint64_t direct_min = 1ull << 22;
	uint64_t direct_min_parent = 1ull << 17;
	int regpart = 1;
	int count16 = 1;
	int leaf17 = 1;
	int mid_leaf = 1;
	int early_leaves = 1;
	int early_plan = 1;
	const uint32_t *order_keys = nullptr;
	uint64_t order_n = 0;
	int merge_leaf = 0;
	char *sel = nullptr;
	size_t sel_bytes = 0;
	uint64_t select_cap = 1ull << 20;
	int topk_rows_mode = 0;
	int topk_rows_lanes = 0;
	char *rows_stage = nullptr;
	size_t rows_stage_bytes = 0;
	int sort_rows_mode = 0;
	int sort_rows_lanes = 0;
	uint64_t *fix_plan = nullptr;
	int fix_stats = 0;
	uint64_t fix_split = 0;
	int search_mode = 0;
	uint64_t search_merge_ratio = 32;
};

static int fail(msd_ctx *c, int code, const char *fmt, ...)
{
	char buf[512];
	va_list ap;
	va_start(ap, fmt);
	vsnprintf(buf, sizeof buf, fmt, ap);
	va_end(ap);
	if (c) c->err = buf;
	return code;
}

#define HIPCHK(c, call)                                                                   \
	do {                                                                              \
		hipError_t e_ = (call);                                                   \
		if (e_ != hipSuccess)                                                     \
			return fail(c, MSD_EHIP, "%s failed: %s (%s:%d)", #call,          \
				    hipGetErrorString(e_), __FILE__, __LINE__);           \
	} while (0)

template <typename... P, typename... A>
static int launch_at(msd_ctx *c, const char *what, const char *file, int line, void (*kernel)(P...), dim3 grid, dim3 block, size_t lds, const A &...args)
{
	hipLaunchKernelGGL(kernel, grid, block, lds, c->stream, static_cast<P>(args)...);
	const hipError_t e = hipGetLastError();
	return e == hipSuccess ? MSD_OK : fail(c, MSD_EHIP, "launch of %s failed: %s (%s:%d)", what, hipGetErrorString(e), file, line);
}
#define LAUNCH_RC(c, kernel, grid, block, lds, ...) launch_at(c, #kernel, __FILE__, __LINE__, kernel, dim3(grid), dim3(block), lds, __VA_ARGS__)
#define LAUNCH(c, kernel, grid, block, lds, ...)                                                    \
	do {                                                                                        \
		if (int rc_ = LAUNCH_RC(c, kernel, grid, block, lds, __VA_ARGS__)) return rc_;      \
	} while (0)

static void set_stat(msd_ctx *c, const char *name, uint64_t v)
{
	for (auto &s : c->stats)
		if (s.first == name) {
			s.second = v;
			return;
		}
	c->stats.emplace_back(name, v);
}
static void add_stat(msd_ctx *c, const char *name, uint64_t v)
{
	for (auto &s : c->stats)
		if (s.first == name) {
			s.second += v;
			return;
		}
	c->stats.emplace_back(name, v);
}


static size_t align_up(size_t x, size_t a) { return (x + a - 1) / a * a; }

static int dev_reserve(msd_ctx *c, char *&p, size_t &have, size_t bytes, bool exact = false)
{
	if (bytes <= have) return MSD_OK;
	if (p) {
		HIPCHK(c, hipStreamSynchronize(c->stream));
		HIPCHK(c, hipFree(p));
		p = nullptr;
		have = 0;
	}
	bytes = align_up(exact ? bytes : bytes + bytes / 8, 1 << 20);
	hipError_t e = hipMalloc((void **)&p, bytes);
	if (e != hipSuccess) return fail(c, MSD_ENOMEM, "workspace hipMalloc(%zu) failed: %s", bytes, hipGetErrorString(e));
	have = bytes;
	return MSD_OK;
}
static int slab_reserve(msd_ctx *c, size_t bytes, bool exact = false)
{
	c->order_keys = nullptr;
	return dev_reserve(c, c->slab, c->slab_bytes, bytes, exact);
}
static int keep_reserve(msd_ctx *c, size_t bytes, bool exact = false) { return dev_reserve(c, c->keep, c->keep_bytes, bytes, exact); }

static int lists_reserve(msd_ctx *c, size_t need, size_t live_general, size_t live_count, bool exact = false)
{
	if (need <= c->lists_cap) return MSD_OK;
	const size_t cap = align_up(exact ? need : need + need / 2, 4096);
	Segment *nb = nullptr;
	hipError_t e = hipMalloc((void **)&nb, 4 * cap * sizeof(Segment));
	if (e != hipSuccess) return fail(c, MSD_ENOMEM, "leaf list hipMalloc failed: %s", hipGetErrorString(e));
	if (c->lists) {
		HIPCHK(c, hipStreamSynchronize(c->stream));
		if (live_general) HIPCHK(c, hipMemcpy(nb, c->lists, live_general * sizeof(Segment), hipMemcpyDeviceToDevice));
		if (live_count) HIPCHK(c, hipMemcpy(nb + 3 * cap, c->lists + 3 * c->lists_cap, live_count * sizeof(Segment), hipMemcpyDeviceToDevice));
		HIPCHK(c, hipFree(c->lists));
	}
	c->lists = nb;
	c->lists_cap = cap;
	return MSD_OK;
}

struct Bump {
	char *base;
	size_t off = 0;
	explicit Bump(char *b) : base(b) {}
	template <typename T> T *take(size_t n)
	{
		off = align_up(off, 256);
		T *p = base ? reinterpret_cast<T *>(base + off) : nullptr;
		off += n * sizeof(T);
		return p;
	}
};

static int pinned_reserve(msd_ctx *c, size_t bytes)
{
	if (bytes <= c->pinned_bytes) return MSD_OK;
	if (c->pinned) {
		HIPCHK(c, hipStreamSynchronize(c->stream));
		HIPCHK(c, hipHostFree(c->pinned));
		c->pinned = nullptr;
	}
	bytes = align_up(bytes * 2, 4096);
	HIPCHK(c, hipHostMalloc(&c->pinned, bytes, hipHostMallocDefault));
	c->pinned_bytes = bytes;
	return MSD_OK;
}

template <typename F> static int slab_carve(msd_ctx *c, F &&carve, size_t min_bytes = 0, bool exact = false)
{
	Bump sz(nullptr);
	carve(sz);
	if (int rc = slab_reserve(c, std::max(sz.off + 4096, min_bytes), exact)) return rc;
	Bump real(c->slab);
	carve(real);
	return MSD_OK;
}


struct ToDevice { void *dst; const void *src; size_t bytes; };
static int upload(msd_ctx *c, std::initializer_list<ToDevice> pieces)
{
	HIPCHK(c, hipStreamSynchronize(c->stream));
	char *at = (char *)c->pinned;
	for (const ToDevice &p : pieces) {
		if (!p.bytes) continue;
		memcpy(at, p.src, p.bytes);
		HIPCHK(c, hipMemcpyAsync(p.dst, at, p.bytes, hipMemcpyHostToDevice, c->stream));
		at += p.bytes;
	}
	return MSD_OK;
}

struct ToHost { size_t at; const void *src; size_t bytes; };
static int read_counters(msd_ctx *c, const Counters *ctr, Counters &hc, std::initializer_list<ToHost> extra = {})
{
	HIPCHK(c, hipMemcpyAsync(c->pinned, ctr, sizeof(Counters), hipMemcpyDeviceToHost, c->stream));
	for (const ToHost &p : extra)
		if (p.bytes) HIPCHK(c, hipMemcpyAsync((char *)c->pinned + p.at, p.src, p.bytes, hipMemcpyDeviceToHost, c->stream));
	HIPCHK(c, hipStreamSynchronize(c->stream));
	memcpy(&hc, c->pinned, sizeof hc);
	return MSD_OK;
}

template <typename T> static int fetch(msd_ctx *c, const T *src, size_t count, std::vector<T> &out)
{
	if (int rc = pinned_reserve(c, count * sizeof(T))) return rc;
	HIPCHK(c, hipMemcpyAsync(c->pinned, src, count * sizeof(T), hipMemcpyDeviceToHost, c->stream));
	HIPCHK(c, hipStreamSynchronize(c->stream));
	out.insert(out.end(), (const T *)c->pinned, (const T *)c->pinned + count);
	return MSD_OK;
}

static void sort_by_start(std::vector<Segment> &v)
{
	std::sort(v.begin(), v.end(), [](const Segment &a, const Segment &b) { return a.start < b.start; });
}

static int fetch_segments(msd_ctx *c, const Segment *src, uint32_t count, std::vector<Segment> &out, const void *pre = nullptr,
			  size_t ahead = 0)
{
	if (count <= ahead)
		out.insert(out.end(), (const Segment *)pre, (const Segment *)pre + count);
	else if (int rc = fetch(c, src, count, out))
		return rc;
	sort_by_start(out);
	return MSD_OK;
}


static void phase_begin(msd_ctx *c)
{
	c->phases.clear();
	c->ev_used = 0;
	c->phase_us.clear();
	if (!c->profiling) return;
	if (!c->ev_start) (void)hipEventCreate(&c->ev_start);
	(void)hipEventRecord(c->ev_start, c->stream);
}
static void phase_mark(msd_ctx *c, const char *name)
{
	if (!c->profiling) return;
	if (c->ev_used == c->ev_pool.size()) {
		hipEvent_t e;
		(void)hipEventCreate(&e);
		c->ev_pool.push_back(e);
	}
	hipEvent_t e = c->ev_pool[c->ev_used++];
	(void)hipEventRecord(e, c->stream);
	c->phases.push_back({ name, e });
}
static void phase_add(std::vector<std::pair<std::string, double>> &list, const std::string &name, double us)
{
	for (auto &q : list)
		if (q.first == name) {
			q.second += us;
			return;
		}
	list.emplace_back(name, us);
}
static void phase_end(msd_ctx *c)
{
	if (!c->profiling) return;
	(void)hipStreamSynchronize(c->stream);
	hipEvent_t prev = c->ev_start;
	for (auto &p : c->phases) {
		float ms = 0;
		(void)hipEventElapsedTime(&ms, prev, p.ev);
		phase_add(c->phase_us, p.name, ms * 1000.0);
		prev = p.ev;
	}
}


struct RoundPlan {
	std::vector<Parent> parents;
	std::vector<Stripe> stripes;
	uint32_t nchildren = 0;
	uint64_t lo_elems = 0;
	uint64_t nslots = 0;
	uint64_t round_keys = 0;
};

static uint32_t ceil_log2_u64(uint64_t x)
{
	uint32_t p = 0;
	while (((uint64_t)1 << p) < x) ++p;
	return p;
}

static uint32_t pick_width(uint64_t count, uint32_t bits, uint64_t small_max, uint32_t leaf_bits)
{
	uint64_t target = small_max / 2;
	uint32_t w = ceil_log2_u64((count + target - 1) / target);
	w = std::max(1u, std::min(8u, w));
	w = std::min(w, bits);
	if (leaf_bits && bits - w > leaf_bits && bits <= leaf_bits + 8 && (count >> (bits - leaf_bits)) <= small_max &&
	    (count >> (bits - leaf_bits)) >= 2048)
		w = bits - leaf_bits;
	return w;
}

template <typename K, typename V>
static void plan_round(const std::vector<Segment> &segs, uint64_t small_max, int sm_count, RoundPlan &rp, uint32_t leaf_bits = 0,
		       uint32_t forced_width = 0, uint32_t nsplit = 0)
{
	using C = Cfg<K, V>;
	constexpr uint64_t B = C::B, T = C::T;
	rp = RoundPlan();
	uint64_t total = 0;
	for (auto &s : segs) total += s.count;
	rp.round_keys = total;
#ifndef MSD_STRIPE_WANT
#define MSD_STRIPE_WANT 4
#endif
#ifndef MSD_STRIPE_CAP_LOG
#define MSD_STRIPE_CAP_LOG 20
#endif
	static_assert(MSD_STRIPE_WANT >= 1 && MSD_STRIPE_WANT <= 64 && MSD_STRIPE_CAP_LOG >= 12 && MSD_STRIPE_CAP_LOG <= 20, "stripe geometry knobs out of range (a stripe has at most 2^20 elements)");
	constexpr int want_mul = MSD_STRIPE_WANT, cap_log = MSD_STRIPE_CAP_LOG;
	uint64_t want = std::max<uint64_t>(1, (uint64_t)sm_count * want_mul);
	uint64_t slen = (total + want - 1) / want;
	slen = std::max<uint64_t>(slen, 4 * T);
	slen = std::min<uint64_t>(slen, (uint64_t)1 << cap_log);
	slen = (slen + T - 1) / T * T;
	for (auto &s : segs) {
		Parent p;
		p.start = s.start;
		p.count = s.count;
		p.width = forced_width ? forced_width : pick_width(s.count, s.bits, small_max, leaf_bits);
		p.shift = s.bits - p.width;
		p.child_base = rp.nchildren;
		p.stripe_lo = (uint32_t)rp.stripes.size();
		p.pad = nsplit;
		rp.nchildren += 1u << p.width;
		const uint64_t end = s.start + s.count;
		const uint64_t a0 = (s.start + B - 1) / B * B;
		uint64_t b = s.start;
		while (b < end) {
			uint64_t e = (b == s.start ? a0 : b) + slen;
			if (e + slen / 2 > end) e = end;
			Stripe st;
			st.begin = b;
			st.end = e;
			st.parent = (uint32_t)rp.parents.size();
			st.slot_lo = (uint32_t)((b + B - 1) / B);
			st.slot_hi = (uint32_t)(e / B);
			if (st.slot_hi < st.slot_lo) st.slot_hi = st.slot_lo;
			st.lo_base = rp.lo_elems;
			st.pad = 0;
			rp.lo_elems += std::min<uint64_t>(e - b, ((uint64_t)1 << p.width) * (B - 1) + 2 * B);
			rp.nslots += st.slot_hi - st.slot_lo;
			rp.stripes.push_back(st);
			b = e;
		}
// ... 87 lines not shown

namespace {

struct KeepBufs {
	uint8_t *block_map, *slot_full;
	Counters *ctr;
	uint32_t big_cap;
	Segment *big;
	Segment *dev_list;
	template <typename K, typename V> void carve_keep(Bump &b, uint64_t n)
	{
		constexpr uint64_t B = Cfg<K, V>::B, small_max = (uint64_t)Cfg<K, V>::SORT_TH * Cfg<K, V>::SORT_KPT;
		block_map = b.take<uint8_t>(n / B + 2);
		slot_full = b.take<uint8_t>(n / B + 2);
		ctr = b.take<Counters>(3);
		big_cap = (uint32_t)std::min<uint64_t>(n / small_max + 16, 0x7FFFFFFFu);
		big = b.take<Segment>(big_cap);
		dev_list = sizeof(K) == 8 ? b.take<Segment>(n / (small_max + 1) + 2) : nullptr;
	}
};

template <typename K, typename V> static size_t keep_bytes_for(uint64_t n)
{
	Bump b(nullptr);
	KeepBufs().carve_keep<K, V>(b, n);
	return b.off + 4096;
}

template <typename K, typename V>
static size_t round_bytes_estimate(uint64_t n, int sm_count)
{
	using C = Cfg<K, V>;
	const uint64_t small_max = (uint64_t)C::SORT_TH * C::SORT_KPT;
	size_t worst = 0;
	for (int shape = 0; shape < 2; ++shape) {
		std::vector<Segment> segs;
		if (shape == 0)
			segs.push_back({ 0, n, (uint32_t)(sizeof(K) * 8), 0 });
		else if (n > 512 * small_max)
			for (int i = 0; i < 256; ++i) segs.push_back({ n / 256 * i, n / 256, (uint32_t)(sizeof(K) * 8 - 8), 0 });
		if (segs.empty()) continue;
		RoundPlan rp;
		plan_round<K, V>(segs, small_max, sm_count, rp);
		Bump b(nullptr);
		RoundBufs rb;
		carve_round<K, V>(b, rp, small_max, rb);
		worst = std::max(worst, b.off);
	}
	return worst + 4096;
}

template <typename K> struct SortJob {
	enum Kind {
		kWhole,
		kDigit,
		kRanges,
		kOffsets,
		kList,
	} kind = kWhole;
	uint32_t stop_bits = 0;
	unsigned shift = 0, width = 0;
	uint64_t *counts = nullptr;
	const K *splitters = nullptr;
	const uint64_t *seg_off = nullptr;
	uint32_t nsplit = 0, nseg = 0;
	const std::vector<Segment> *segs = nullptr;

	static SortJob whole(uint32_t stop_bits = 0) { return { kWhole, stop_bits }; }
	static SortJob digit(unsigned shift, unsigned width, uint64_t *counts) { return { kDigit, 0, shift, width, counts }; }
	static SortJob ranges(const K *delims, uint32_t nsplit, unsigned width, uint64_t *counts) { return { kRanges, 0, 0, width, counts, delims, nullptr, nsplit }; }
	static SortJob offsets(const uint64_t *seg_off, uint32_t nseg) { return { kOffsets, 0, 0, 0, nullptr, nullptr, seg_off, 0, nseg }; }
	static SortJob list(const std::vector<Segment> &segs) { return { kList, 0, 0, 0, nullptr, nullptr, nullptr, 0, 0, &segs }; }
	bool single_pass() const { return kind == kDigit || kind == kRanges; }
	bool segmented() const { return kind == kOffsets || kind == kList; }
};

constexpr int kRestart = 1;

template <typename K, typename V> struct SortRun : KeepBufs {
	using C = Cfg<K, V>;
	static constexpr bool HV = has_val<V>::value;
	static constexpr int B = C::B;
	static constexpr uint64_t small_max = (uint64_t)C::SORT_TH * C::SORT_KPT;
	static constexpr uint32_t count_bits = HV ? (uint32_t)kLeafCountBits : (uint32_t)kCountMaxBits;

	msd_ctx *const c;
	K *const keys;
	uint64_t *const vals;
	const uint64_t n, low_mask;
	const int end_bit;
	const SortJob<K> &job;

	std::vector<Segment> cur;
	uint32_t dev_np = 0;
	uint32_t nsmall_host = 0, ncount_host = 0, nbig_host = 0;
	unsigned long long *vres = nullptr;
	int round = 0;
	bool prev_direct;
	bool unverified = false;
	uint64_t claimed_const = 0;
	uint64_t exact_vary = 0;
	bool leaf17_ok = true;
	uint32_t nfallback_known = 0xFFFFFFFFu;

	SortRun(msd_ctx *c_, K *keys_, uint64_t *vals_, uint64_t n_, int end_bit_, const SortJob<K> &job_)
		: c(c_), keys(keys_), vals(vals_), n(n_), low_mask(end_bit_ >= 64 ? ~0ull : ((1ull << end_bit_) - 1ull)), end_bit(end_bit_), job(job_),
		  prev_direct(job_.kind == SortJob<K>::kOffsets) {}

	Segment *small() const { return c->lists; }
	Segment *small_count() const { return c->lists + 3 * c->lists_cap; }

	int initial_segments()
	{
		if (job.single_pass()) {
			if (job.width < 1 || job.width > 8 || job.shift + job.width > sizeof(K) * 8)
				return fail(c, MSD_EINVAL, "partition: radix_bits must be 1..8 and shift+radix_bits within the key");
			cur.push_back({ 0, n, job.shift + job.width, 0 });
		} else if (job.kind == SortJob<K>::kOffsets) {
			const uint64_t *off = job.seg_off;
			for (uint32_t i = 0; i < job.nseg; ++i) {
				if (off[i] > off[i + 1] || off[i + 1] > n) return fail(c, MSD_EINVAL, "segments: offsets must ascend and stay within n");
				if (end_bit > 0 && off[i + 1] - off[i] > 1) cur.push_back({ off[i], off[i + 1] - off[i], (uint32_t)end_bit, 0 });
			}
		} else if (job.kind == SortJob<K>::kList) {
			for (auto &sg : *job.segs) {
				if (sg.start + sg.count > n || sg.bits > sizeof(K) * 8) return fail(c, MSD_EINVAL, "segments: a segment lies outside the array");
				if (sg.bits > 0 && sg.count > 1) cur.push_back(sg);
			}
			sort_by_start(cur);
		} else if (end_bit > 0 && n > 1 && (uint32_t)end_bit > job.stop_bits)
			cur.push_back({ 0, n, (uint32_t)end_bit, 0 });
		return MSD_OK;
	}

	int reserve_keep()
	{
		int rc = keep_reserve(c, keep_bytes_for<K, V>(n), true);
		if (!rc) rc = pinned_reserve(c, 1 << 16);
		if (!rc) rc = lists_reserve(c, 4096, 0, 0);
		if (rc) return rc;
		Bump kb(c->keep);
		carve_keep<K, V>(kb, n);
		vres = reinterpret_cast<unsigned long long *>(ctr + 1);
		HIPCHK(c, hipMemsetAsync(ctr, 0, sizeof(Counters), c->stream));
		return MSD_OK;
	}

	int vres_init()
	{
		HIPCHK(c, hipMemsetAsync(vres, 0x00, sizeof(unsigned long long), c->stream));
		HIPCHK(c, hipMemsetAsync(vres + 1, 0xFF, sizeof(unsigned long long), c->stream));
		return MSD_OK;
	}
	int run_vary(uint64_t stride, uint64_t *vary_out)
	{
		if (int rc = vres_init()) return rc;
		const uint64_t cnt = (n + stride - 1) / stride;
		const unsigned grid = (unsigned)std::min<uint64_t>((uint64_t)c->sm_count * 8, (cnt + 255) / 256);
		LAUNCH(c, (vary_kernel<K>), grid, 256, 0, keys, n, stride, vres);
		HIPCHK(c, hipMemcpyAsync(c->pinned, vres, 2 * sizeof(unsigned long long), hipMemcpyDeviceToHost, c->stream));
		HIPCHK(c, hipStreamSynchronize(c->stream));
		const unsigned long long *h = (const unsigned long long *)c->pinned;
		*vary_out = h[0] ^ h[1];
		return MSD_OK;
	}

	int skip_leading_bits()
	{
		if (job.single_pass() || job.segmented() || cur.empty() || n < 4096) return MSD_OK;
		uint64_t vary = 0;
		int rc = run_vary(std::max<uint64_t>(1, n / 8192), &vary);
		if (rc) return rc;
		vary &= low_mask;
		const int top_sample = vary ? 64 - __builtin_clzll(vary) : 0;
		if (top_sample + 8 <= end_bit) {
			if (top_sample > 0 && c->direct_mode != 0 && n >= c->direct_min && n >= ((uint64_t)1 << 24)) {
				unverified = true;
				claimed_const = low_mask & ~(((uint64_t)1 << top_sample) - 1ull);
				cur[0].bits = (uint32_t)top_sample;
				set_stat(c, "skipped_bits", (uint64_t)(end_bit - top_sample));
			} else {
				rc = run_vary(1, &vary);
				if (rc) return rc;
				vary &= low_mask;
				const int top = vary ? 64 - __builtin_clzll(vary) : 0;
				set_stat(c, "skipped_bits", (uint64_t)(end_bit - top));
				if (top == 0)
					cur.clear();
				else
					cur[0].bits = (uint32_t)top;
			}
		}
		phase_mark(c, "bit skip");
		if (!cur.empty() && cur[0].bits <= job.stop_bits) cur.clear();
		return MSD_OK;
	}

	int route_to_leaves()
	{
		if (job.segmented() && !cur.empty()) {
			std::vector<Segment> l_small, l_count, l_big, parents;
			for (auto &sg : cur) {
				Route to = route_child(sg.count, sg.bits, job.stop_bits, HV ? 0u : count_bits, small_max, std::max<uint64_t>(small_max, kCountMedMax), !HV);
				if (to == kRouteDone) continue;
				if (to == kRouteBig && l_big.size() >= big_cap) to = kRouteNext;
				(to == kRouteSmall ? l_small : to == kRouteCount ? l_count : to == kRouteBig ? l_big : parents).push_back(sg);
			}
			int rc = lists_reserve(c, std::max(l_small.size(), l_count.size()) + 16, 0, 0);
			if (!rc) rc = pinned_reserve(c, (l_small.size() + l_count.size() + l_big.size()) * sizeof(Segment) + sizeof(Counters));
			if (rc) return rc;
			nsmall_host = (uint32_t)l_small.size();
			ncount_host = (uint32_t)l_count.size();
			nbig_host = (uint32_t)l_big.size();
			Counters hc0 = {};
			hc0.nsmall = nsmall_host;
			hc0.ncount = ncount_host;
			hc0.nbig = nbig_host;
			rc = upload(c, { { small(), l_small.data(), l_small.size() * sizeof(Segment) },
					 { small_count(), l_count.data(), l_count.size() * sizeof(Segment) },
					 { big, l_big.data(), l_big.size() * sizeof(Segment) },
					 { ctr, &hc0, sizeof hc0 } });
			if (rc) return rc;
			cur = parents;
		}
		const bool whole = !job.single_pass() && !job.segmented();
		if constexpr (!HV) {
			if (whole && !cur.empty() && n > small_max && cur[0].bits <= count_bits && n < 0xFFFF0000ull) {
				if (int rc = upload(c, { { big, &cur[0], sizeof(Segment) } })) return rc;
				nbig_host = 1;
				cur.clear();
			}
		}
		if (whole && !cur.empty() && n <= small_max) {
			if (int rc = upload(c, { { small(), &cur[0], sizeof(Segment) } })) return rc;
			nsmall_host = 1;
			cur.clear();
		}
		return MSD_OK;
	}

	int rounds()
	{
		while (!cur.empty() || dev_np) {
			int rc;
			if constexpr (sizeof(K) == 8) {
				if (!job.single_pass() && c->regpart) {
					std::vector<Segment> fit, rest;
					if (!dev_np)
						for (auto &sg : cur) (sg.count + 1 <= kRpCap && sg.count > small_max ? fit : rest).push_back(sg);
					if (dev_np || fit.size() >= 64 || (!fit.empty() && rest.empty())) {
						if constexpr (HV)
							rc = c->leaf17 && leaf17_ok && !unverified ? leaf17_pass(fit, rest) : regpart_round(fit, rest);
						else
							rc = regpart_round(fit, rest);
						if (rc) return rc;
						continue;
					}
				}
			}
			Round r;
			if ((rc = plan_upload(r)) || (rc = classify(r)) || (rc = permute_blocks(r)) || (rc = cleanup_collect(r)) ||
			    (rc = r.leaves_follow ? early_summary(r) : r.plan_ahead ? plan_next_early(r) : round_summary(r)))
				return rc;
		}
		return MSD_OK;
	}

	int leaf17_pass(const std::vector<Segment> &fit, const std::vector<Segment> &rest)
	{
		const bool on_device = dev_np != 0;
		const uint32_t np = on_device ? dev_np : (uint32_t)fit.size();
		dev_np = 0;
		int rc = slab_reserve(c, 2 * (size_t)np * sizeof(Segment) + 4096);
		if (!rc) rc = pinned_reserve(c, (size_t)np * sizeof(Segment) + 4096);
		if (rc) return rc;
		Segment *d_segs = reinterpret_cast<Segment *>(c->slab), *d_rej = d_segs + np;
		if (on_device)
			HIPCHK(c, hipMemcpyAsync(d_segs, dev_list, (size_t)np * sizeof(Segment), hipMemcpyDeviceToDevice, c->stream));
		else if ((rc = upload(c, { { d_segs, fit.data(), (size_t)np * sizeof(Segment) } })))
			return rc;
		HIPCHK(c, hipMemsetAsync(&ctr->nslow2, 0, sizeof(uint32_t), c->stream));
		HIPCHK(c, hipMemsetAsync(&ctr->l17_slow, 0, sizeof(uint32_t), c->stream));
		phase_mark(c, "plan+upload");
		LAUNCH(c, (leaf17_kernel<V>), std::min<uint32_t>(np, (uint32_t)c->sm_count), kL17Th, kL17Lds, keys, vals, d_segs, np, d_rej, &ctr->nslow2, ctr, 0);
		phase_mark(c, "leaf17");
		Counters hc;
		if ((rc = read_counters(c, ctr, hc))) return rc;
		if (hc.errors) return fail(c, MSD_EINTERNAL, "leaf17: %u internal invariant violations (checks 0x%x)", hc.errors, hc.err_sites);
		add_stat(c, "leaf17_segments", np - hc.nslow2);
		add_stat(c, "leaf17_slow_segments", hc.l17_slow);
		cur = rest;
		if (hc.nslow2) {
			if ((rc = fetch_segments(c, d_rej, hc.nslow2, cur))) return rc;
			leaf17_ok = false;
			add_stat(c, "leaf17_rejected", hc.nslow2);
		}
		phase_mark(c, "readback");
		return MSD_OK;
	}

	int regpart_round(const std::vector<Segment> &fit, const std::vector<Segment> &rest)
	{
		const bool on_device = dev_np != 0;
		const uint32_t wmax = regpart_width(kRpCap, 64, small_max);
		std::vector<Parent> ps;
		uint32_t nc = 0;
		for (const Segment &sg : fit) {
			const uint32_t w = regpart_width(sg.count, sg.bits, small_max);
			ps.push_back({ sg.start, sg.count, sg.bits - w, w, nc, 0, 0, 0 });
			nc += 1u << w;
		}
		if (on_device) nc = dev_np << wmax;
		const uint32_t np = on_device ? dev_np : (uint32_t)ps.size();
		dev_np = 0;
		const size_t next_cap = (size_t)nc + 2;
		Parent *d_parents = nullptr;
		ChildArrays ca = {};
		Segment *d_next = nullptr;
		uint32_t *d_scr = nullptr;
		int rc = slab_carve(c, [&](Bump &b) {
			d_parents = b.take<Parent>(np);
			ca.start = b.take<uint64_t>(nc);
			ca.count = b.take<uint64_t>(nc);
			d_next = b.take<Segment>(next_cap);
			d_scr = b.take<uint32_t>(64);
		});
		if (!rc) rc = lists_reserve(c, (size_t)std::max(nsmall_host, ncount_host) + nc + 16, nsmall_host, ncount_host);
		if (!rc) rc = pinned_reserve(c, std::max<size_t>(on_device ? 0 : np * sizeof(Parent), 256 + 2048 * sizeof(Segment)));
		if (rc) return rc;
		LAUNCH(c, round_init_kernel, 1, 256, 0, ctr, d_scr + 16, 0, reinterpret_cast<unsigned long long *>(d_scr + 32), 0, d_scr,
		       nullptr, nullptr, 0, nullptr, 0, nullptr);
		if (on_device)
			LAUNCH(c, regpart_plan_kernel, (np + 255) / 256, 256, 0, dev_list, np, small_max, d_parents, ctr);
		else if ((rc = upload(c, { { d_parents, ps.data(), np * sizeof(Parent) } })))
			return rc;
		phase_mark(c, "plan+upload");
		LAUNCH(c, (regpart_kernel<V>), std::min<uint32_t>(np, (uint32_t)c->sm_count), kRpTh, kRpLds, keys, vals, d_parents, np, ca, ctr);
		phase_mark(c, "A register partition");
		LAUNCH(c, collect_kernel, (np + (256u >> wmax) - 1) / (256u >> wmax), 256, 0, d_parents, np, wmax, ca, small_max, small_max,
		       std::min<size_t>(c->lists_cap, 0xFFFFFFFFu), count_bits, d_next, small(), small_count(), HV ? nullptr : big, big_cap, ctr,
		       nullptr, nc, job.stop_bits);
		phase_mark(c, "C cleanup");
		Counters hc;
		const size_t ahead = std::min<size_t>(next_cap, 2048);
		if ((rc = read_counters(c, ctr, hc, { { 256, d_next, ahead * sizeof(Segment) } }))) return rc;
		if (hc.errors) return fail(c, MSD_EINTERNAL, "register partition round: %u internal invariant violations (checks 0x%x)", hc.errors, hc.err_sites);
		nsmall_host = hc.nsmall;
		ncount_host = hc.ncount;
		nbig_host = hc.nbig;
		add_stat(c, "rounds", 1);
		add_stat(c, "regpart_rounds", 1);
		add_stat(c, "parents", np);
		add_stat(c, "children", nc);
		cur = rest;
		if (hc.next_parents && (rc = fetch_segments(c, d_next, hc.next_parents, cur, (char *)c->pinned + 256, ahead))) return rc;
		phase_mark(c, "readback");
		prev_direct = false;
		++round;
		return MSD_OK;
	}

	struct Round {
		RoundPlan rp;
		RoundBufs rb;
		uint32_t np = 0, ns = 0, nc = 0;
		bool tried_direct = false;
		bool hist_checks = false;
		bool leaves_follow = false;
		size_t plan_ahead = 0;
	};
	static constexpr size_t kReadAhead = 2048, kSegOff = 256, kVresOff = kSegOff - 2 * sizeof(unsigned long long);
	static constexpr size_t kEarlyOff = kSegOff + kReadAhead * sizeof(Segment), kStagingBytes = kEarlyOff + sizeof(Counters);
	static_assert(sizeof(Counters) <= kVresOff, "counters and the OR/AND words share the head of the staging buffer");
	static constexpr size_t kPlanCtrOff = (kStagingBytes + 255) / 256 * 256, kPlanSegOff = kPlanCtrOff + 256;
	static constexpr size_t kParkOff = kPlanSegOff + kReadAhead * sizeof(Segment), kStage2Off = (kParkOff + sizeof(Counters) + 255) / 256 * 256;
	static_assert(sizeof(Counters) <= 256, "the early copy of the counters has 256 bytes");
	struct Pending {
		bool open = false;
		int round = 0;
		uint32_t np = 0, ns = 0, nc = 0;
		uint64_t nslots = 0;
	} pending;
	Pending parked;
	bool parked_direct = false;
	bool enqueue_ahead = false;
	Counters *park() const { return ctr + 2; }
	static size_t stage2_bytes(size_t np, size_t ns) { return kStage2Off + np * sizeof(Parent) + ns * sizeof(Stripe); }
	void plan_next(const std::vector<Segment> &segs, RoundPlan &rp) const
	{
		plan_round<K, V>(segs, small_max, c->sm_count, rp, count_bits, job.single_pass() ? job.width : 0u, job.splitters ? job.nsplit : 0u);
	}
	int plan_upload(Round &r)
	{
		const bool ahead = enqueue_ahead;
		enqueue_ahead = false;
		plan_next(cur, r.rp);
		const bool first = round == 0;
		int rc = slab_carve(c, [&](Bump &b) { carve_round<K, V>(b, r.rp, small_max, r.rb); },
				    first && !job.single_pass() ? round_bytes_estimate<K, V>(n, c->sm_count) : 0, first);
		if (rc) return rc;
		r.np = (uint32_t)r.rp.parents.size(), r.ns = (uint32_t)r.rp.stripes.size(), r.nc = r.rp.nchildren;
		if constexpr (!HV) {
			r.leaves_follow = !job.single_pass() && !unverified && c->early_leaves;
			for (size_t i = 0; i < r.np && r.leaves_follow; ++i) r.leaves_follow = r.rp.parents[i].shift <= count_bits;
		}
		if ((rc = lists_reserve(c, (size_t)std::max(nsmall_host, ncount_host) + r.nc + 16, nsmall_host, ncount_host))) return rc;
		{
			static_assert(sizeof(Parent) % 4 == 0 && sizeof(Stripe) % 4 == 0, "the plan travels as 32-bit words");
			const uint64_t plan_words = (r.np <= kDirectMaxParents ? r.np : 1) * sizeof(DirectPlan) / sizeof(uint32_t);
			const uint64_t ntiles = (r.nc + kScanTile - 1) / kScanTile + 1;
			const uint64_t parent_words = r.np * sizeof(Parent) / 4, stripe_words = r.ns * sizeof(Stripe) / 4;
			const size_t next_stripes = (size_t)std::max<uint64_t>((uint64_t)c->sm_count * MSD_STRIPE_WANT, n >> MSD_STRIPE_CAP_LOG) + 2 * kReadAhead + 64;
			const size_t want = !ahead && c->early_plan && !job.single_pass() ? stage2_bytes(kReadAhead, next_stripes) : 0;
			if ((rc = pinned_reserve(c, std::max({ kStagingBytes, r.np * sizeof(Parent) + r.ns * sizeof(Stripe), want })))) return rc;
			char *stage = (char *)c->pinned + (ahead ? kStage2Off : 0);
			if (!ahead) HIPCHK(c, hipStreamSynchronize(c->stream));
			memcpy(stage, r.rp.parents.data(), r.np * sizeof(Parent));
			memcpy(stage + r.np * sizeof(Parent), r.rp.stripes.data(), r.ns * sizeof(Stripe));
			void *staged = nullptr;
			HIPCHK(c, hipHostGetDevicePointer(&staged, c->pinned, 0));
			staged = (char *)staged + (stage - (char *)c->pinned);
			const unsigned grid = (unsigned)std::min<uint64_t>(1024, (std::max({ plan_words, ntiles, parent_words, stripe_words }) + 255) / 256 + 1);
			LAUNCH(c, round_init_kernel, grid, 256, 0, ctr, reinterpret_cast<uint32_t *>(r.rb.plans), plan_words, r.rb.scan_state, ntiles, r.rb.scan_ctr,
			       static_cast<const uint32_t *>(staged), reinterpret_cast<uint32_t *>(r.rb.parents), parent_words,
			       reinterpret_cast<uint32_t *>(r.rb.stripes), stripe_words, ahead ? park() : nullptr);
		}
		phase_mark(c, "plan+upload");
		return MSD_OK;
	}

	int classify_direct(Round &r)
	{
		const RoundPlan &rp = r.rp;
		const uint32_t np = r.np, ns = r.ns;
		bool try_direct = c->direct_mode != 0 && rp.round_keys >= c->direct_min && !job.splitters;
		for (size_t i = 0; i < np && try_direct; ++i) try_direct = rp.parents[i].width == 8 || c->direct_mode == 2;
		if (try_direct && np > 1) {
			try_direct = prev_direct && np <= kDirectMaxParents;
			for (size_t i = 0; i < np && try_direct; ++i) try_direct = rp.parents[i].count >= c->direct_min_parent;
		}
		for (size_t i = 0; i < ns && try_direct; ++i)
			try_direct = rp.stripes[i].end - rp.stripes[i].begin >= (((uint64_t)1 << rp.parents[rp.stripes[i].parent].width) * (B - 1) + 2 * B);
		uint64_t max_piece = 0;
		for (size_t i = 0; i < np && try_direct; ++i)
			max_piece = std::max<uint64_t>(max_piece, rp.parents[i].count / B / (rp.parents[i].stripe_hi - rp.parents[i].stripe_lo) + 2);
		if (!try_direct || max_piece >= 65535) return MSD_OK;
		const RoundBufs &rb = r.rb;
		if (np == 1) {
			const uint64_t nruns = rp.parents[0].count / 256;
			const uint32_t every = (uint32_t)std::min<uint64_t>(64, std::max<uint64_t>(1, nruns / 16384));
			const uint32_t sgrid = (uint32_t)std::min<uint64_t>(1024, std::max<uint64_t>(1, nruns / every / 4));
			LAUNCH(c, (direct_sample_kernel<K>), sgrid, 256, 0, keys, rb.parents, rb.plans, every);
		} else {
			r.hist_checks = unverified && rp.round_keys == n;
			if (r.hist_checks) {
				if (int rc = vres_init()) return rc;
				add_stat(c, "bit_skip_checked_by_histogram", 1);
			}
			LAUNCH(c, (direct_hist_kernel<K>), ns, 1024, 0, keys, rb.stripes, rb.parents, rb.plans, r.hist_checks ? vres : nullptr);
		}
		LAUNCH(c, (direct_plan_kernel<B>), np, 256, 0, rb.parents, rb.plans, ctr);
		phase_mark(c, np == 1 ? "A sample" : "A histogram");
		r.tried_direct = true;
		const uint32_t force = c->direct_mode == 2 ? 1u : 0u;
		LAUNCH(c, (classify_direct2_kernel<K, V>), ns, (Direct2Cfg<K, V>::TH), (Direct2Lds<K, V>::bytes), keys, vals, rb.stripes, rb.parents, rb.plans,
		       block_map, slot_full, rb.fb, rb.lo_cnt, rb.lo_off, rb.lo_keys, rb.lo_vals, rb.nfull, ctr, force);
		phase_mark(c, "A classify direct");
		return MSD_OK;
	}

	int classify(Round &r)
	{
		if (int rc = classify_direct(r)) return rc;
		if (!r.tried_direct || c->direct_mode != 2) {
			const RoundBufs &rb = r.rb;
			const uint32_t *run_if = r.tried_direct ? &ctr->direct_uneven : nullptr;
			if (job.splitters)
				LAUNCH(c, (classify_stream2_kernel<K, V, true>), r.ns, (Stream2Cfg<K, V>::TH), (Stream2Lds<K, V>::range_bytes), keys, vals, rb.stripes,
				       rb.parents, block_map, rb.fb, rb.lo_cnt, rb.lo_off, rb.lo_keys, rb.lo_vals, rb.nfull, job.splitters, run_if);
			else
				LAUNCH(c, (classify_stream2_kernel<K, V, false>), r.ns, (Stream2Cfg<K, V>::TH), (Stream2Lds<K, V>::bytes), keys, vals, rb.stripes,
				       rb.parents, block_map, rb.fb, rb.lo_cnt, rb.lo_off, rb.lo_keys, rb.lo_vals, rb.nfull, nullptr, run_if);
		}
		phase_mark(c, "A classify");
		return MSD_OK;
	}

	int permute_blocks(Round &r)
	{
		const RoundBufs &rb = r.rb;
		const uint32_t np = r.np, ns = r.ns, nc = r.nc;
		const uint8_t *full_map = r.tried_direct ? slot_full : nullptr;
		const uint32_t force_map = c->direct_mode == 2 ? 1u : 0u;
		if (const uint32_t groups = child_scan_groups(r.rp); groups > 1) {
			LAUNCH(c, child_scan_part_kernel, dim3(np, groups), 256, 0, rb.parents, rb.fb, rb.lo_cnt, rb.scan_part);
			LAUNCH(c, (child_scan_split_kernel<B>), dim3(np, groups), 256, 0, rb.parents, rb.lo_cnt, rb.scan_part, rb.lo_dst, rb.ca);
			add_stat(c, "child_scan_split_rounds", 1);
		} else
			LAUNCH(c, (child_scan_kernel<B>), np, 1024, 0, rb.parents, rb.fb, rb.lo_cnt, rb.lo_dst, rb.ca);
		if (int rc = collect(r)) return rc;
		LAUNCH(c, (slot_classify_kernel<false>), ns * kSlotParts, 256, 0, rb.stripes, rb.parents, block_map, rb.nfull, rb.ca, rb.list, rb.holes, ctr,
		       full_map, force_map);
		LAUNCH(c, list_prepare_kernel, (nc + 255) / 256, 256, 0, nc, rb.ca, ctr, std::min<uint64_t>(r.rp.nslots, 0xFFFFFFFFu), 2 * nc + kMinChains);
		LAUNCH(c, scan_lookback_kernel, (unsigned)((nc + kScanTile - 1) / kScanTile), kScanTh, 0,
		       rb.ca.list_len, rb.ca.list_base, nc, rb.scan_state, rb.scan_ctr, &ctr->errors);
		LAUNCH(c, (slot_classify_kernel<true>), ns * kSlotParts, 256, 0, rb.stripes, rb.parents, block_map, rb.nfull, rb.ca, rb.list, rb.holes, ctr,
		       full_map, force_map);
		const uint32_t evict_waves = nc > 16384 ? 0u : (uint32_t)std::min<uint64_t>(64, std::max<uint64_t>(1, 16384 / nc));
		const unsigned evict_grid = evict_waves ? (unsigned)(((uint64_t)nc * evict_waves + 3) / 4) : (unsigned)((nc + 255) / 256);
		LAUNCH(c, (evict_kernel<K, V>), evict_grid, 256, 0, nc, rb.ca, rb.list, rb.holes, ctr, keys, vals, rb.xkeys, rb.xvals, evict_waves);
		phase_mark(c, "B metadata");

		const unsigned grid = (unsigned)std::min<uint64_t>((uint64_t)c->sm_count * c->chains_per_cu[HV ? 2 : sizeof(K) == 8 ? 1 : 0],
								 std::max<uint64_t>(1, (r.rp.nslots + 255) / 256));
		LAUNCH(c, (chains_kernel<K, V>), grid, 256, 0, rb.ca, rb.list, rb.holes, ctr, keys, vals, rb.xkeys, rb.xvals, n / B, 4 * nc + kMinChains);
		phase_mark(c, "B block permute");
		return MSD_OK;
	}

	bool may_leave_parents(const Round &r) const
	{
		uint64_t leaf_max = small_max;
		if constexpr (sizeof(K) == 8)
			if (c->regpart) leaf_max = std::max<uint64_t>(leaf_max, kRpCap - 1);
		for (const Parent &p : r.rp.parents)
			if ((p.count >> p.width) > leaf_max) return true;
		return false;
	}

	int collect(Round &r)
	{
		const RoundBufs &rb = r.rb;
		const uint32_t np = r.np, nc = r.nc;
		const bool sp = job.single_pass();
		uint32_t wmax = 1;
		for (size_t i = 0; i < np; ++i) wmax = std::max(wmax, r.rp.parents[i].width);
		const uint32_t small_cap = (uint32_t)std::min<size_t>(c->lists_cap, 0xFFFFFFFFu);
		LAUNCH(c, collect_kernel, (np + (256u >> wmax) - 1) / (256u >> wmax), 256, 0, rb.parents, np, wmax, rb.ca,
		       sp ? ~0ull : small_max, (HV || sp) ? small_max : std::max<uint64_t>(small_max, kCountMedMax),
		       small_cap, sp ? 0u : count_bits,
		       rb.next_parents, small(), small_count(), (HV || sp) ? nullptr : big, big_cap, ctr,
		       (sp && job.counts) ? job.counts : nullptr, job.splitters ? job.nsplit + 1u : nc, job.stop_bits);
		if (r.leaves_follow) {
			if (!c->ev_early) HIPCHK(c, hipEventCreateWithFlags(&c->ev_early, hipEventDisableTiming));
			HIPCHK(c, hipMemcpyAsync((char *)c->pinned + kEarlyOff, ctr, sizeof(Counters), hipMemcpyDeviceToHost, c->stream));
			HIPCHK(c, hipEventRecord(c->ev_early, c->stream));
		} else if (c->early_plan && !sp && !r.hist_checks && !parked.open && c->pinned_bytes >= kStage2Off && may_leave_parents(r)) {
			r.plan_ahead = std::min<size_t>(r.rp.round_keys / (small_max + 1) + 2, kReadAhead);
			if (!c->ev_early) HIPCHK(c, hipEventCreateWithFlags(&c->ev_early, hipEventDisableTiming));
			HIPCHK(c, hipMemcpyAsync((char *)c->pinned + kPlanCtrOff, ctr, sizeof(Counters), hipMemcpyDeviceToHost, c->stream));
			HIPCHK(c, hipMemcpyAsync((char *)c->pinned + kPlanSegOff, rb.next_parents, r.plan_ahead * sizeof(Segment), hipMemcpyDeviceToHost, c->stream));
			HIPCHK(c, hipEventRecord(c->ev_early, c->stream));
		}
		return MSD_OK;
	}

	int cleanup_collect(Round &r)
	{
		const RoundBufs &rb = r.rb;
		LAUNCH(c, (cleanup_kernel<K, V>), r.ns, 256, 0, rb.stripes, rb.parents, rb.lo_cnt, rb.lo_off, rb.lo_dst, rb.ca, rb.lo_keys, rb.lo_vals, keys, vals,
		       rb.xkeys, rb.xvals, ctr);
		phase_mark(c, "C cleanup");
		return MSD_OK;
	}

	int round_errors(const Counters &hc, int rnd, uint32_t np, uint32_t ns, const char *direct)
	{
		return fail(c, MSD_EINTERNAL, "round %d: %u internal invariant violations (checks 0x%x: bit = site of msd_note_error in csrc/; 0 = a scan tile's look-back timed out; "
					      "%u parents, %u stripes, direct placement %s)",
			    rnd, hc.errors, hc.err_sites, np, ns, direct);
	}
	void round_stats(const Counters &hc, uint32_t np, uint32_t ns, uint32_t nc, uint64_t nslots)
	{
		add_stat(c, "rounds", 1);
		add_stat(c, "parents", np);
		add_stat(c, "stripes", ns);
		add_stat(c, "children", nc);
		add_stat(c, "slots", nslots);
		add_stat(c, "holes", hc.nholes);
		set_stat(c, "chain_steps", hc.chain_steps);
		set_stat(c, "excess_blocks", hc.nexcess);
	}

	int parked_summary()
	{
		if (!parked.open) return MSD_OK;
		parked.open = false;
		Counters pc;
		memcpy(&pc, (char *)c->pinned + kParkOff, sizeof pc);
		if (pc.errors) return round_errors(pc, parked.round, parked.np, parked.ns, parked_direct ? "used" : "not used");
		round_stats(pc, parked.np, parked.ns, parked.nc, parked.nslots);
		return MSD_OK;
	}
	ToHost parked_piece() const { return { kParkOff, park(), parked.open ? sizeof(Counters) : 0 }; }

	int plan_next_early(Round &r)
	{
		HIPCHK(c, hipEventSynchronize(c->ev_early));
		Counters hc;
		memcpy(&hc, (char *)c->pinned + kPlanCtrOff, sizeof hc);
		bool ok = !hc.errors && hc.next_parents != 0 && hc.next_parents <= r.plan_ahead;
		std::vector<Segment> next;
		if (ok) {
			const Segment *sg = (const Segment *)((char *)c->pinned + kPlanSegOff);
			next.assign(sg, sg + hc.next_parents);
			sort_by_start(next);
			if constexpr (sizeof(K) == 8) {
				if (c->regpart) {
					size_t fit = 0;
					for (auto &s : next) fit += s.count + 1 <= kRpCap && s.count > small_max;
					if (fit >= 64 || (fit && fit == next.size())) ok = false;
				}
			}
		}
		if (ok) {
			RoundPlan rp;
			RoundBufs rb;
			plan_next(next, rp);
			Bump sz(nullptr);
			carve_round<K, V>(sz, rp, small_max, rb);
			ok = sz.off + 4096 <= c->slab_bytes && (size_t)std::max(hc.nsmall, hc.ncount) + rp.nchildren + 16 <= c->lists_cap &&
			     stage2_bytes(rp.parents.size(), rp.stripes.size()) <= c->pinned_bytes;
		}
		if (!ok) return round_summary(r);
		prev_direct = r.tried_direct && (hc.direct_uneven == 0 || c->direct_mode == 2);
		if (prev_direct) add_stat(c, "direct_rounds", 1);
		nsmall_host = hc.nsmall;
		ncount_host = hc.ncount;
		nbig_host = hc.nbig;
		parked = { true, round, r.np, r.ns, r.nc, r.rp.nslots };
		parked_direct = prev_direct;
		enqueue_ahead = true;
		add_stat(c, "rounds_planned_early", 1);
		cur = std::move(next);
		phase_mark(c, "readback");
		++round;
		return MSD_OK;
	}

	int early_summary(Round &r)
	{
		HIPCHK(c, hipEventSynchronize(c->ev_early));
		Counters hc;
		memcpy(&hc, (char *)c->pinned + kEarlyOff, sizeof hc);
		if (hc.next_parents || hc.ncount == 0 || hc.errors) return round_summary(r);
		prev_direct = r.tried_direct && (hc.direct_uneven == 0 || c->direct_mode == 2);
		if (prev_direct) add_stat(c, "direct_rounds", 1);
		nsmall_host = hc.nsmall;
		ncount_host = hc.ncount;
		nbig_host = hc.nbig;
		pending = { true, round, r.np, r.ns, r.nc, r.rp.nslots };
		add_stat(c, "leaves_behind_round", 1);
		cur.clear();
		phase_mark(c, "readback");
		++round;
		return MSD_OK;
	}

	int round_summary(Round &r)
	{
		const size_t np_cap = r.rp.round_keys / (small_max + 1) + 2, ahead = job.single_pass() ? 0 : std::min(np_cap, kReadAhead);
		Counters hc;
		int rc = pinned_reserve(c, kStagingBytes);
		if (rc || (rc = read_counters(c, ctr, hc, { { kSegOff, r.rb.next_parents, ahead * sizeof(Segment) },
							    { kVresOff, vres, r.hist_checks ? 2 * sizeof(unsigned long long) : 0 }, parked_piece() })))
			return rc;
		if ((rc = parked_summary())) return rc;
		if (hc.errors) return round_errors(hc, round, r.np, r.ns, r.tried_direct ? (hc.direct_uneven ? "declined" : "used") : "not tried");
		if (r.hist_checks) {
			const unsigned long long *h = (const unsigned long long *)((char *)c->pinned + kVresOff);
			if ((h[0] ^ h[1]) & claimed_const) {
				exact_vary = h[0] ^ h[1];
				phase_mark(c, "readback");
				return kRestart;
			}
			unverified = false;
		}
		prev_direct = r.tried_direct && (hc.direct_uneven == 0 || c->direct_mode == 2);
		if (prev_direct) add_stat(c, "direct_rounds", 1);
		nsmall_host = hc.nsmall;
		ncount_host = hc.ncount;
		nbig_host = hc.nbig;
		round_stats(hc, r.np, r.ns, r.nc, r.rp.nslots);
		cur.clear();
		if (job.single_pass()) return MSD_OK;
		bool stays_on_device = false;
		if constexpr (sizeof(K) == 8) {
			if (c->regpart && hc.next_parents >= 64 && (uint64_t)hc.next_max + 1 <= kRpCap) {
				HIPCHK(c, hipMemcpyAsync(dev_list, r.rb.next_parents, (size_t)hc.next_parents * sizeof(Segment), hipMemcpyDeviceToDevice, c->stream));
				dev_np = hc.next_parents;
				stays_on_device = true;
			}
		}
		if (hc.next_parents && !stays_on_device &&
		    (rc = fetch_segments(c, r.rb.next_parents, hc.next_parents, cur, (char *)c->pinned + kSegOff, ahead)))
			return rc;
		phase_mark(c, "readback");
		++round;
		return MSD_OK;
	}

	int verify_skip()
	{
		if (!unverified) return MSD_OK;
		uint64_t vary = 0;
		if (int rc = run_vary(1, &vary)) return rc;
		phase_mark(c, "bit skip");
		if (vary & claimed_const) {
			exact_vary = vary;
			return kRestart;
		}
		unverified = false;
		return MSD_OK;
	}

	int start_over()
	{
		const uint64_t vary = exact_vary & low_mask;
		const int top = vary ? 64 - __builtin_clzll(vary) : 0;
		set_stat(c, "skipped_bits", (uint64_t)(end_bit - top));
		add_stat(c, "bit_skip_restarts", 1);
		cur.clear();
		if (top > 0 && (uint32_t)top > job.stop_bits) cur.push_back({ 0, n, (uint32_t)top, 0 });
		nsmall_host = ncount_host = nbig_host = dev_np = 0;
		round = 0;
		pending.open = parked.open = enqueue_ahead = false;
		prev_direct = unverified = false;
		HIPCHK(c, hipMemsetAsync(ctr, 0, sizeof(Counters), c->stream));
		return MSD_OK;
	}

	int count_leaves()
	{
		if constexpr (!HV) {
			if (!ncount_host || job.single_pass()) return MSD_OK;
			int rc = slab_reserve(c, 3 * (size_t)ncount_host * sizeof(Segment) + 4096);
			if (rc) return rc;
			Segment *slow = reinterpret_cast<Segment *>(c->slab), *rej16 = slow + ncount_host, *slow2 = rej16 + ncount_host;
			const uint32_t count_grid = std::min<uint32_t>(ncount_host, (uint32_t)c->sm_count * 2);
			const bool c16 = sizeof(K) == 4 && (c->count16 == 2 || (c->count16 == 1 && n / ncount_host >= 12000));
			if constexpr (sizeof(K) == 4)
				if (c16) LAUNCH(c, count_place16_kernel, count_grid, kC16Th, kC16Lds, keys, small_count(), ncount_host, rej16, ctr, n);
			LAUNCH(c, (count_place_kernel<K>), count_grid, kCountTh, kCountLds, keys, c16 ? rej16 : small_count(), c16 ? 0u : ncount_host,
			       c16 ? &ctr->nslow16 : nullptr, slow, ctr);
			const uint32_t *walk_n = &ctr->nslow;
			const Segment *walk_list = slow;
			if constexpr (sizeof(K) == 4) {
				if (c->mid_leaf) {
					LAUNCH(c, (merge_count_kernel<true>), std::min<uint32_t>(ncount_host, (uint32_t)c->sm_count), kMcTh, kMcLds, keys, keys, nullptr,
					       nullptr, nullptr, 0, 0, 0, 0, slow, &ctr->nslow, slow2, &ctr->nslow2, &ctr->count_ticket4, nullptr);
					walk_n = &ctr->nslow2;
					walk_list = slow2;
				}
			}
			LAUNCH(c, (count_walk_kernel<K>), count_grid, kCountTh, kCountLds, keys, walk_list, walk_n, small(), nsmall_host, small_max, big, big_cap, ctr);
			phase_mark(c, "count sort");
			Counters hc;
			if ((rc = read_counters(c, ctr, hc, { parked_piece() })) || (rc = parked_summary())) return rc;
			if (pending.open) {
				pending.open = false;
				if (hc.errors && (hc.err_sites & ~0x80u || !hc.err_sites))
					return round_errors(hc, pending.round, pending.np, pending.ns, prev_direct ? "used" : "not used");
				round_stats(hc, pending.np, pending.ns, pending.nc, pending.nslots);
			}
			if (hc.errors) return fail(c, MSD_EINTERNAL, "counting leaf: %u segments could not be queued", hc.errors);
			set_stat(c, "count16_rejected", hc.nslow16);
			set_stat(c, "count_slow_segments", hc.nslow);
			nbig_host = hc.nbig;
			nfallback_known = hc.nfallback;
		}
		return MSD_OK;
	}

	int big_count_sort()
	{
		if constexpr (!HV) {
			if (!nbig_host || job.single_pass()) return MSD_OK;
			std::vector<Segment> bs;
			int rc = fetch(c, big, nbig_host, bs);
			if (rc) return rc;
			const uint32_t batch_max = 4096;
			for (uint32_t b0 = 0; b0 < nbig_host; b0 += batch_max) {
				const uint32_t nb = std::min(batch_max, nbig_host - b0);
				constexpr uint32_t tile_elems = big_tile_elems<K>() * kBigGroup;
				std::vector<uint32_t> first(2 * ((size_t)nb + 1));
				uint32_t *first_chunk = first.data(), *first_tile = first.data() + nb + 1;
				uint64_t nchunks = 0, ntiles = 0;
				for (uint32_t i = 0; i < nb; ++i) {
					first_chunk[i] = (uint32_t)nchunks;
					first_tile[i] = (uint32_t)ntiles;
					nchunks += (bs[b0 + i].count + kBigChunk - 1) / kBigChunk;
					ntiles += (bs[b0 + i].count + tile_elems - 1) / tile_elems;
				}
				first_chunk[nb] = (uint32_t)nchunks;
				first_tile[nb] = (uint32_t)ntiles;
				uint32_t *ghist = nullptr, *d_first = nullptr;
				K *seg_hi = nullptr;
				uint16_t *tile_v = nullptr;
				rc = slab_carve(c, [&](Bump &b) {
					ghist = b.take<uint32_t>((size_t)nb * 65536);
					seg_hi = b.take<K>(nb);
					d_first = b.take<uint32_t>(first.size());
					tile_v = b.take<uint16_t>(ntiles * kBigGroup + nb + 8);
				});
				if (!rc) rc = pinned_reserve(c, first.size() * sizeof(uint32_t));
				if (!rc) rc = upload(c, { { d_first, first.data(), first.size() * sizeof(uint32_t) } });
				if (rc) return rc;
				HIPCHK(c, hipMemsetAsync(ghist, 0, (size_t)nb * 65536 * sizeof(uint32_t), c->stream));
				LAUNCH(c, (bigcount_hist_kernel<K>), (unsigned)std::min<uint64_t>(nchunks, (uint64_t)c->sm_count), kBigHistTh, kBigHistLds, keys, big + b0,
				       d_first, nb, ghist);
				LAUNCH(c, (bigcount_scan_kernel<K>), nb, 1024, 0, keys, big + b0, d_first + nb + 1, ghist, seg_hi, tile_v, ctr);
				LAUNCH(c, (bigcount_write_kernel<K>), (unsigned)ntiles, kBigWriteTh, kBigWriteLds, keys, big + b0, d_first + nb + 1, nb, ghist, seg_hi, tile_v);
			}
			phase_mark(c, "big count sort");
			Counters hc;
			if ((rc = read_counters(c, ctr, hc))) return rc;
			if (hc.errors) return fail(c, MSD_EINTERNAL, "counting sort: %u histogram totals disagree with segment sizes", hc.errors);
		}
		return MSD_OK;
	}

	int lds_leaves()
	{
		if (job.single_pass()) return MSD_OK;
		constexpr size_t leaf_lds = LeafCountLds<K, V>::bytes;
		const uint32_t leaf_per_cu = (uint32_t)std::max<size_t>(1, std::min<size_t>(2048 / C::SORT_TH, (160 * 1024) / (leaf_lds + 512)));
		const auto leaf_grid = [&](uint32_t nsegs) { return std::min<uint32_t>(nsegs, (uint32_t)c->sm_count * leaf_per_cu); };
		bool small_done = false;
		if constexpr (!HV && sizeof(K) == 8) {
			if (c->leaf17 && nsmall_host && n / nsmall_host >= 8192) {
				if (int rc = slab_reserve(c, (size_t)nsmall_host * sizeof(Segment) + 4096)) return rc;
				Segment *d_rej = reinterpret_cast<Segment *>(c->slab);
				HIPCHK(c, hipMemsetAsync(&ctr->nslow2, 0, sizeof(uint32_t), c->stream));
				HIPCHK(c, hipMemsetAsync(&ctr->l17_slow, 0, sizeof(uint32_t), c->stream));
				LAUNCH(c, (leaf17_kernel<NoVal>), std::min<uint32_t>(nsmall_host, (uint32_t)c->sm_count), kL17Th, kL17Lds, keys, nullptr, small(), nsmall_host,
				       d_rej, &ctr->nslow2, ctr, 4096);
				LAUNCH(c, (leaf_count_sort_kernel<K, V>), leaf_grid(nsmall_host), C::SORT_TH, leaf_lds, keys, vals, d_rej, nsmall_host, small() + nsmall_host,
				       ctr, &ctr->leaf_ticket[0], &ctr->nslow2);
				add_stat(c, "leaf17_launches", 1);
				small_done = true;
			}
		}
		if (nsmall_host && !small_done)
			LAUNCH(c, (leaf_count_sort_kernel<K, V>), leaf_grid(nsmall_host), C::SORT_TH, leaf_lds, keys, vals, small(), nsmall_host, small() + nsmall_host, ctr,
			       &ctr->leaf_ticket[0], nullptr);
		if (HV && ncount_host)
			LAUNCH(c, (leaf_count_sort_kernel<K, V>), leaf_grid(ncount_host), C::SORT_TH, leaf_lds, keys, vals, small_count(), ncount_host, small() + nsmall_host,
			       ctr, &ctr->leaf_ticket[1], nullptr);
		const bool may_fall_back = HV || nsmall_host != 0 || nfallback_known != 0;
		if (may_fall_back && nsmall_host + ncount_host)
			LAUNCH(c, (lds_sort_kernel<K, V>), std::min<uint32_t>(nsmall_host + ncount_host, 2 * c->sm_count), C::SORT_TH, (SortLds<K, V>::bytes), keys, vals,
			       small() + nsmall_host, 0, &ctr->nfallback);
		phase_mark(c, "LDS sort");
		return MSD_OK;
	}
};

}

template <typename K, typename V>
static int sort_impl(msd_ctx *c, K *keys, uint64_t *vals, uint64_t n, int end_bit, const SortJob<K> &job)
{
	constexpr bool HV = has_val<V>::value;
	if (n == 0) return MSD_OK;
	if (!keys || (HV && !vals)) return fail(c, MSD_EINVAL, "null data pointer");
	if (!aligned16(keys) || (HV && !aligned16(vals)))
		return fail(c, MSD_EINVAL, "keys/rids must be 16-byte aligned (the reference asserts the same, src/msb_64.c:2273)");
	if (end_bit < 0 || end_bit > (int)sizeof(K) * 8) return fail(c, MSD_EINVAL, "end_bit out of range");
	if (n >= ((uint64_t)1 << 36)) return fail(c, MSD_EINVAL, "n too large for 32-bit block slots");
	HIPCHK(c, hipSetDevice(c->device));
	c->stats.clear();
	phase_begin(c);
	SortRun<K, V> s(c, keys, vals, n, end_bit, job);
	int rc = s.initial_segments();
	if (!rc) rc = s.reserve_keep();
	if (!rc) rc = s.skip_leading_bits();
	if (!rc) rc = s.route_to_leaves();
	while (!rc) {
		rc = s.rounds();
		if (!rc) rc = s.verify_skip();
		if (rc != kRestart) break;
		rc = s.start_over();
	}
	if (!rc) rc = s.count_leaves();
	if (!rc) rc = s.big_count_sort();
	if (rc) return rc;
	set_stat(c, "big_count_segments", s.nbig_host);
	if ((rc = s.lds_leaves())) return rc;
	set_stat(c, "count_segments", s.ncount_host);
	set_stat(c, "small_segments", s.nsmall_host);
	set_stat(c, "workspace_bytes", c->slab_bytes + c->keep_bytes + 4 * c->lists_cap * sizeof(Segment));
	phase_end(c);
	return MSD_OK;
}

template <typename K, typename V> static int reserve_for(msd_ctx *c, uint64_t n)
{
	int rc = slab_reserve(c, round_bytes_estimate<K, V>(n, c->sm_count), true);
	if (!rc) rc = keep_reserve(c, keep_bytes_for<K, V>(n), true);
	if (!rc) rc = pinned_reserve(c, 1 << 20);
	if (!rc) rc = lists_reserve(c, leaf_list_guess<K, V>(n), 0, 0, true);
	return rc;
}

constexpr int kNoLayout = 1;
template <typename F> static int with_layout(int key_bytes, int val_bytes, F &&f)
{
	if (key_bytes == 4 && val_bytes == 0) return f(uint32_t(), NoVal());
	if (key_bytes == 8 && val_bytes == 0) return f(uint64_t(), NoVal());
	if (key_bytes == 8 && val_bytes == 8) return f(uint64_t(), uint64_t());
	return kNoLayout;
}

template <typename K, typename V> static int sort_bits(msd_ctx *c, K *k, uint64_t *r, uint64_t n, int end_bit)
{
	if (!c) return MSD_EINVAL;
	return sort_impl<K, V>(c, k, r, n, end_bit, SortJob<K>::whole());
}
template <typename K, typename V> static int partition(msd_ctx *c, K *k, uint64_t *r, uint64_t n, unsigned shift, unsigned rb, uint64_t *cnt)
{
	if (!c) return MSD_EINVAL;
	HIPCHK(c, hipSetDevice(c->device));
	if (cnt && rb <= 8) HIPCHK(c, hipMemsetAsync(cnt, 0, sizeof(uint64_t) << rb, c->stream));
	return sort_impl<K, V>(c, k, r, n, (int)sizeof(K) * 8, SortJob<K>::digit(shift, rb, cnt));
}
template <typename K, typename V> static int sort_top(msd_ctx *c, K *k, uint64_t *r, uint64_t n, int end_bit, int begin_bit)
{
	if (!c) return MSD_EINVAL;
	if (begin_bit < 0 || begin_bit > end_bit) return fail(c, MSD_EINVAL, "begin_bit must lie in [0, end_bit]");
	return sort_impl<K, V>(c, k, r, n, end_bit, SortJob<K>::whole((uint32_t)begin_bit));
}
template <typename K, typename V>
static int sort_segments(msd_ctx *c, K *k, uint64_t *r, uint64_t n, const uint64_t *seg_off, uint32_t nseg, int end_bit)
{
	if (!c) return MSD_EINVAL;
	if (nseg == 0) return MSD_OK;
	if (!seg_off) return fail(c, MSD_EINVAL, "segments: null offsets");
	return sort_impl<K, V>(c, k, r, n, end_bit, SortJob<K>::offsets(seg_off, nseg));
}

template <typename F> static hipError_t max_lds(F *kernel, size_t bytes)
{
	return hipFuncSetAttribute(reinterpret_cast<const void *>(kernel), hipFuncAttributeMaxDynamicSharedMemorySize, (int)bytes);
}

template <typename K, bool IDX, int LANES> static int set_row_kernels_lds_attrs_for(msd_ctx *c)
{
	HIPCHK(c, max_lds(&topk_rows_kernel<K, IDX, LANES>, RowsLds<K, IDX, LANES>::bytes));
	HIPCHK(c, max_lds(&sort_rows_kernel<K, IDX, LANES>, SortRowsLds<K, IDX, LANES>::bytes));
	return MSD_OK;
}
static int set_row_kernels_lds_attrs(msd_ctx *c)
{
	int rc = MSD_OK;
	for (const int key_bytes : { 4, 8 })
		for (const bool with_idx : { false, true })
			for (const int lanes_per_row : { 64, 256, 1024 })
				if (!rc) rc = with_width(key_bytes, [&](auto k0) {
					return with_flag(with_idx, [&](auto idx) {
						return with_lanes(lanes_per_row, [&](auto lanes) { return set_row_kernels_lds_attrs_for<decltype(k0), decltype(idx)::value, decltype(lanes)::value>(c); });
					});
				});
	return rc;
}

template <typename K, typename V> static int set_lds_attrs(msd_ctx *c)
{
	{
		int per_cu = 0;
		HIPCHK(c, hipOccupancyMaxActiveBlocksPerMultiprocessor(&per_cu, chains_kernel<K, V>, 256, 0));
		c->chains_per_cu[has_val<V>::value ? 2 : sizeof(K) == 8 ? 1 : 0] = std::max(1, per_cu);
	}
	HIPCHK(c, max_lds(&classify_stream2_kernel<K, V, false>, Stream2Lds<K, V>::bytes));
	HIPCHK(c, max_lds(&classify_stream2_kernel<K, V, true>, Stream2Lds<K, V>::range_bytes));
	HIPCHK(c, max_lds(&lds_sort_kernel<K, V>, SortLds<K, V>::bytes));
	HIPCHK(c, max_lds(&classify_direct2_kernel<K, V>, Direct2Lds<K, V>::bytes));
	if constexpr (sizeof(K) == 8) {
		HIPCHK(c, max_lds(&regpart_kernel<V>, kRpLds));
		HIPCHK(c, max_lds(&leaf17_kernel<V>, kL17Lds));
	}
	HIPCHK(c, max_lds(&leaf_count_sort_kernel<K, V>, LeafCountLds<K, V>::bytes));
	if constexpr (!has_val<V>::value) {
		if constexpr (sizeof(K) == 4) {
			HIPCHK(c, max_lds(&count_place16_kernel, kC16Lds));
			HIPCHK(c, max_lds(&merge_place16_kernel<2>, kC16Lds));
			HIPCHK(c, max_lds(&merge_place16_kernel<4>, kC16Lds));
			HIPCHK(c, max_lds(&merge_place16_kernel<8>, kC16Lds));
			HIPCHK(c, max_lds(&merge_count_kernel<false, uint32_t>, kMcLds));
			HIPCHK(c, max_lds(&merge_count_kernel<false, uint16_t>, kMcLds));
			HIPCHK(c, max_lds(&merge_count_kernel<false, Hist2>, kMcLds));
			HIPCHK(c, max_lds(&hist2_pack_kernel<uint32_t>, kH2Lds));
			HIPCHK(c, max_lds(&hist2_pack_kernel<uint16_t>, kH2Lds));
			HIPCHK(c, max_lds(&scatter_low16_kernel, kS16Lds));
			HIPCHK(c, max_lds(&merge_count_kernel<true, uint32_t>, kMcLds));
		}
		HIPCHK(c, max_lds(&count_place_kernel<K>, kCountLds));
		HIPCHK(c, max_lds(&count_walk_kernel<K>, kCountLds));
		HIPCHK(c, max_lds(&bigcount_hist_kernel<K>, kBigHistLds));
		HIPCHK(c, max_lds(&bigcount_write_kernel<K>, kBigWriteLds));
	}
	return MSD_OK;
}

template <typename K>
static int gather_impl(msd_ctx *c, K *dst, const K *src, const uint64_t *src_off, const uint64_t *dst_off, const uint64_t *len, uint32_t nruns)
{
	if (!c) return MSD_EINVAL;
	if (nruns == 0) return MSD_OK;
	if (!dst || !src || !src_off || !dst_off || !len) return fail(c, MSD_EINVAL, "gather: null pointer");
	HIPCHK(c, hipSetDevice(c->device));
	std::vector<GatherRun> runs;
	uint64_t nchunks = 0;
	for (uint32_t i = 0; i < nruns; ++i) {
		if (!len[i]) continue;
		runs.push_back({ src_off[i], dst_off[i], len[i], (uint32_t)nchunks, 0 });
		nchunks += (len[i] + kGatherChunk - 1) / kGatherChunk;
	}
	if (runs.empty()) return MSD_OK;
	if (nchunks >= 0xFFFFFFFFull) return fail(c, MSD_EINVAL, "gather: too many elements");
	runs.push_back({ 0, 0, 0, (uint32_t)nchunks, 0 });
	const size_t nreal = runs.size() - 1, ncoarse = (size_t)(nchunks >> 6) + 2;
	std::vector<uint32_t> coarse(ncoarse);
	for (size_t i = 0, r = 0; i < ncoarse; ++i) {
		const uint64_t ch = std::min<uint64_t>((uint64_t)i << 6, nchunks - 1);
		while (r + 1 < nreal && runs[r + 1].first_chunk <= ch) ++r;
		coarse[i] = (uint32_t)r;
	}
	const size_t runs_bytes = align_up(runs.size() * sizeof(GatherRun), 256), bytes = runs_bytes + ncoarse * sizeof(uint32_t);
	int rc = pinned_reserve(c, bytes);
	if (!rc) rc = slab_reserve(c, bytes + 4096);
	if (rc) return rc;
	HIPCHK(c, hipStreamSynchronize(c->stream));
	memcpy(c->pinned, runs.data(), runs.size() * sizeof(GatherRun));
	memcpy((char *)c->pinned + runs_bytes, coarse.data(), ncoarse * sizeof(uint32_t));
	GatherRun *d_runs = reinterpret_cast<GatherRun *>(c->slab);
	const uint32_t *d_coarse = reinterpret_cast<const uint32_t *>(c->slab + runs_bytes);
	HIPCHK(c, hipMemcpyAsync(d_runs, c->pinned, bytes, hipMemcpyHostToDevice, c->stream));
	const unsigned grid = (unsigned)nchunks;
	LAUNCH(c, (gather_runs_kernel<K>), grid, 256, 0, dst, src, d_runs, runs.size() - 1, nchunks, d_coarse);
	return MSD_OK;
}


extern "C" {

const char *msd_version(void) { return MSD_VERSION; }

int msd_create(msd_ctx **out, int device, void *stream)
{
	if (!out) return MSD_EINVAL;
	*out = nullptr;
	int ndev = 0;
	if (hipGetDeviceCount(&ndev) != hipSuccess || ndev == 0) return MSD_EHIP;
	if (device < 0 || device >= ndev) return MSD_EINVAL;
	msd_ctx *c = new msd_ctx();
	c->device = device;
	c->stream = (hipStream_t)stream;
	if (hipSetDevice(device) != hipSuccess) {
		delete c;
		return MSD_EHIP;
	}
	hipDeviceProp_t prop;
	if (hipGetDeviceProperties(&prop, device) == hipSuccess) c->sm_count = prop.multiProcessorCount;
	for (const char *name : { "direct_mode", "regpart", "count16" }) {
		const char *env = !strcmp(name, "direct_mode") ? "MSD_DIRECT" : !strcmp(name, "regpart") ? "MSD_REGPART" : "MSD_COUNT16";
		const char *v = getenv(env);
		if (!v) continue;
		char *end = nullptr;
		const long x = strtol(v, &end, 10);
		if (end == v || *end || msd_set_option(c, name, x) != MSD_OK) fprintf(stderr, "msd_create: ignoring %s=%s\n", env, v);
	}
	const auto attrs = [c](auto k, auto v) { return set_lds_attrs<decltype(k), decltype(v)>(c); };
	int rc = with_layout(4, 0, attrs);
	if (!rc) rc = with_layout(8, 0, attrs);
	if (!rc) rc = with_layout(8, 8, attrs);
	if (!rc) rc = set_row_kernels_lds_attrs(c);
	if (!rc && hipMalloc((void **)&c->fix_plan, kFixWords * sizeof(uint64_t)) != hipSuccess) rc = fail(c, MSD_ENOMEM, "plan words hipMalloc failed");
	if (rc) {
		fprintf(stderr, "msd_create: %s\n", c->err.c_str());
		delete c;
		return rc;
	}
	*out = c;
	return MSD_OK;
}

int msd_destroy(msd_ctx *c)
{
	if (!c) return MSD_EINVAL;
	(void)hipSetDevice(c->device);
	(void)hipStreamSynchronize(c->stream);
	if (c->slab) (void)hipFree(c->slab);
	if (c->keep) (void)hipFree(c->keep);
	if (c->lists) (void)hipFree(c->lists);
	if (c->sel) (void)hipFree(c->sel);
	if (c->rows_stage) (void)hipFree(c->rows_stage);
	if (c->fix_plan) (void)hipFree(c->fix_plan);
	if (c->pinned) (void)hipHostFree(c->pinned);
	if (c->ev_start) (void)hipEventDestroy(c->ev_start);
	if (c->ev_early) (void)hipEventDestroy(c->ev_early);
	for (auto e : c->ev_pool) (void)hipEventDestroy(e);
	delete c;
	return MSD_OK;
}

int msd_set_stream(msd_ctx *c, void *stream)
{
	if (!c) return MSD_EINVAL;
	c->stream = (hipStream_t)stream;
	return MSD_OK;
}

void *msd_get_stream(const msd_ctx *c) { return c ? (void *)c->stream : nullptr; }
int msd_get_device(const msd_ctx *c) { return c ? c->device : -1; }

int msd_reserve(msd_ctx *c, uint64_t n, int key_bytes, int val_bytes)
{
	if (!c) return MSD_EINVAL;
	HIPCHK(c, hipSetDevice(c->device));
	const int rc = with_layout(key_bytes, val_bytes, [&](auto k, auto v) { return reserve_for<decltype(k), decltype(v)>(c, n); });
	return rc != kNoLayout ? rc : fail(c, MSD_EINVAL, "unsupported element layout %d+%d bytes", key_bytes, val_bytes);
}

uint64_t msd_workspace_bytes(const msd_ctx *c) { return c ? c->slab_bytes + c->keep_bytes + 4 * c->lists_cap * sizeof(Segment) + c->sel_bytes + c->rows_stage_bytes : 0; }
const char *msd_last_error(const msd_ctx *c) { return c ? c->err.c_str() : "null context"; }

int msd_sort_u32_bits(msd_ctx *c, uint32_t *k, uint64_t n, int end_bit) { return sort_bits<uint32_t, NoVal>(c, k, nullptr, n, end_bit); }
int msd_sort_u64_bits(msd_ctx *c, uint64_t *k, uint64_t n, int end_bit) { return sort_bits<uint64_t, NoVal>(c, k, nullptr, n, end_bit); }
int msd_sort_pairs_u64_bits(msd_ctx *c, uint64_t *k, uint64_t *r, uint64_t n, int end_bit) { return sort_bits<uint64_t, uint64_t>(c, k, r, n, end_bit); }
int msd_sort_u32(msd_ctx *c, uint32_t *k, uint64_t n) { return msd_sort_u32_bits(c, k, n, 32); }
int msd_sort_u64(msd_ctx *c, uint64_t *k, uint64_t n) { return msd_sort_u64_bits(c, k, n, 64); }
int msd_sort_pairs_u64(msd_ctx *c, uint64_t *k, uint64_t *r, uint64_t n) { return msd_sort_pairs_u64_bits(c, k, r, n, 64); }

int msd_partition_u32(msd_ctx *c, uint32_t *k, uint64_t n, unsigned shift, unsigned rb, uint64_t *cnt) { return partition<uint32_t, NoVal>(c, k, nullptr, n, shift, rb, cnt); }
int msd_partition_u64(msd_ctx *c, uint64_t *k, uint64_t n, unsigned shift, unsigned rb, uint64_t *cnt) { return partition<uint64_t, NoVal>(c, k, nullptr, n, shift, rb, cnt); }
int msd_partition_pairs_u64(msd_ctx *c, uint64_t *k, uint64_t *r, uint64_t n, unsigned shift, unsigned rb, uint64_t *cnt) { return partition<uint64_t, uint64_t>(c, k, r, n, shift, rb, cnt); }

int msd_sort_u32_top(msd_ctx *c, uint32_t *k, uint64_t n, int end_bit, int begin_bit) { return sort_top<uint32_t, NoVal>(c, k, nullptr, n, end_bit, begin_bit); }
int msd_sort_u64_top(msd_ctx *c, uint64_t *k, uint64_t n, int end_bit, int begin_bit) { return sort_top<uint64_t, NoVal>(c, k, nullptr, n, end_bit, begin_bit); }
int msd_sort_pairs_u64_top(msd_ctx *c, uint64_t *k, uint64_t *r, uint64_t n, int end_bit, int begin_bit) { return sort_top<uint64_t, uint64_t>(c, k, r, n, end_bit, begin_bit); }

}

template <typename K>
static int bounds_impl(msd_ctx *c, const K *k, uint64_t n, unsigned shift, uint64_t first, uint32_t nbuckets, uint64_t *bounds)
{
	if (!c) return MSD_EINVAL;
	if (!bounds || (n && !k)) return fail(c, MSD_EINVAL, "bucket_bounds: null pointer");
	if (shift >= sizeof(K) * 8 || nbuckets == 0 || nbuckets > (1u << 24)) return fail(c, MSD_EINVAL, "bucket_bounds: shift or bucket count out of range");
	HIPCHK(c, hipSetDevice(c->device));
	LAUNCH(c, (bucket_bounds_kernel<K>), (nbuckets + 1 + 255) / 256, 256, 0, k, n, shift, first, nbuckets, bounds);
	return MSD_OK;
}

template <typename IN>
static int merge_impl(msd_ctx *c, const IN *src, uint64_t src_cap, const uint64_t *d_counts, const uint64_t *src_base, uint32_t nsrc,
		      uint32_t nb, int open_bits, uint32_t first_prefix, uint32_t *dst, uint64_t dst_cap, uint64_t n_expected)
{
	constexpr bool IN16 = sizeof(IN) == 2, HIST = sizeof(IN) == 1;
	if (!c) return MSD_EINVAL;
	if (!src || !dst || !d_counts || !src_base) return fail(c, MSD_EINVAL, "merge_buckets: null pointer");
	if (nsrc < 1 || nsrc > 8) return fail(c, MSD_EINVAL, "merge_buckets: 1..8 source runs per bucket");
	if (nb == 0 || nb > (1u << 24)) return fail(c, MSD_EINVAL, "merge_buckets: bucket count out of range");
	if (open_bits < 1 || open_bits > 16) return fail(c, MSD_EINVAL, "merge_buckets: 1..16 open bits");
	if ((IN16 || HIST) && open_bits != 16) return fail(c, MSD_EINVAL, "merge_buckets: extents of low halves need 16 open bits");
	if (HIST && src_cap < (uint64_t)nsrc * nb * kH2Rec) return fail(c, MSD_EINVAL, "merge_buckets: %u x %u records of %u bytes do not fit the source buffer", nsrc, nb, kH2Rec);
	if (!aligned16(src) || !aligned16(dst)) return fail(c, MSD_EINVAL, "merge_buckets: buffers must be 16-byte aligned");
	if (n_expected > dst_cap) return fail(c, MSD_EINVAL, "merge_buckets: the output buffer is too small");
	if ((uint64_t)first_prefix + nb > (1ull << (32 - open_bits))) return fail(c, MSD_EINVAL, "merge_buckets: bucket numbers exceed the key's prefix");
	if (ranges_overlap(src, src_cap * sizeof(IN), dst, dst_cap * 4)) return fail(c, MSD_EINVAL, "merge_buckets: source and destination overlap");
	HIPCHK(c, hipSetDevice(c->device));
	c->stats.clear();
	phase_begin(c);
	if (n_expected == 0) return MSD_OK;
	Counters *ctr = nullptr;
	uint32_t *status = nullptr, *cnt32 = nullptr;
	uint64_t *soff = nullptr, *doff = nullptr;
	Segment *rej = nullptr;
	int rc = slab_carve(c, [&](Bump &b) {
		ctr = b.take<Counters>(1);
		status = b.take<uint32_t>(64);
		cnt32 = b.take<uint32_t>((size_t)nsrc * nb);
		soff = b.take<uint64_t>((size_t)nsrc * nb);
		doff = b.take<uint64_t>((size_t)nb + 1);
		rej = b.take<Segment>(nb);
	});
	if (!rc) rc = pinned_reserve(c, 4096);
	if (rc) return rc;
	HIPCHK(c, hipMemsetAsync(ctr, 0, (char *)(status + 64) - (char *)ctr, c->stream));
	MergeBase mb = {};
	for (uint32_t x = 0; x < nsrc; ++x) mb.b[x] = src_base[x];
	LAUNCH(c, merge_plan_kernel, nsrc + 1, 1024, 0, d_counts, mb, nsrc, nb, n_expected, cnt32, soff, doff, status);
	const bool in_regs = !IN16 && !HIST && (c->merge_leaf == 1 || (c->merge_leaf == 0 && n_expected / nb <= 12000 && open_bits >= (int)kC16MinBits));
	if (in_regs) {
		if constexpr (!IN16 && !HIST) {
			const unsigned grid = (unsigned)std::min<uint64_t>(nb, (uint64_t)c->sm_count * 2);
			const auto place16 = nsrc <= 2 ? merge_place16_kernel<2> : nsrc <= 4 ? merge_place16_kernel<4> : merge_place16_kernel<8>;
			LAUNCH(c, place16, grid, kC16Th, kC16Lds, src, src_cap, dst, cnt32, soff, doff, nsrc, nb, open_bits, first_prefix, rej, ctr, status);
		}
	} else {
		const unsigned grid = (unsigned)std::min<uint64_t>(nb, (uint64_t)c->sm_count);
		LAUNCH(c, (merge_count_kernel<false, IN>), grid, kMcTh, kMcLds, src, dst, cnt32, soff, doff, nsrc, nb, open_bits, first_prefix, nullptr, nullptr,
		       rej, &ctr->nslow16, &ctr->count_ticket3, status);
	}
	phase_mark(c, "merge leaf");
	Counters hc;
	if ((rc = read_counters(c, ctr, hc, { { 1024, status, sizeof(uint32_t) } }))) return rc;
	if (*(const uint32_t *)((char *)c->pinned + 1024)) return fail(c, MSD_EINVAL, "merge_buckets: the counts do not add up to the expected %llu keys (or a count exceeds 32 bits)", (unsigned long long)n_expected);
	const uint32_t nrej = hc.nslow16;
	phase_end(c);
	if (nrej) {
		std::vector<Segment> segs;
		if ((rc = fetch(c, rej, nrej, segs))) return rc;
		if ((rc = sort_impl<uint32_t, NoVal>(c, dst, nullptr, n_expected, 32, SortJob<uint32_t>::list(segs)))) return rc;
	}
	set_stat(c, "merge_rejected", nrej);
	return MSD_OK;
}

extern "C" {

int msd_bucket_bounds_u32(msd_ctx *c, const uint32_t *k, uint64_t n, unsigned shift, uint64_t first, uint32_t nbuckets, uint64_t *bounds)
{
	return bounds_impl<uint32_t>(c, k, n, shift, first, nbuckets, bounds);
}
int msd_bucket_bounds_u64(msd_ctx *c, const uint64_t *k, uint64_t n, unsigned shift, uint64_t first, uint32_t nbuckets, uint64_t *bounds)
{
	return bounds_impl<uint64_t>(c, k, n, shift, first, nbuckets, bounds);
}
int msd_merge_buckets_u32(msd_ctx *c, const uint32_t *d_src, uint64_t src_cap, const uint64_t *d_counts, const uint64_t *src_base, uint32_t nsrc,
			  uint32_t nbuckets, int open_bits, uint32_t first_prefix, uint32_t *d_dst, uint64_t dst_cap, uint64_t n_expected)
{
	return merge_impl<uint32_t>(c, d_src, src_cap, d_counts, src_base, nsrc, nbuckets, open_bits, first_prefix, d_dst, dst_cap, n_expected);
}
int msd_merge_buckets_u32_low16(msd_ctx *c, const uint16_t *d_src, uint64_t src_cap, const uint64_t *d_counts, const uint64_t *src_base, uint32_t nsrc,
				uint32_t nbuckets, uint32_t first_prefix, uint32_t *d_dst, uint64_t dst_cap, uint64_t n_expected)
{
	return merge_impl<uint16_t>(c, d_src, src_cap, d_counts, src_base, nsrc, nbuckets, 16, first_prefix, d_dst, dst_cap, n_expected);
}
int msd_merge_buckets_u32_hist2(msd_ctx *c, const void *d_rec, uint64_t rec_bytes, const uint64_t *d_counts, uint32_t nsrc, uint32_t nbuckets,
				uint32_t first_prefix, uint32_t *d_dst, uint64_t dst_cap, uint64_t n_expected)
{
	const uint64_t zero[8] = { 0, 0, 0, 0, 0, 0, 0, 0 };
	return merge_impl<Hist2>(c, (const Hist2 *)d_rec, rec_bytes, d_counts, zero, nsrc, nbuckets, 16, first_prefix, d_dst, dst_cap, n_expected);
}
uint64_t msd_hist2_record_bytes(void) { return kH2Rec; }
}
template <typename IN>
static int hist2_pack_impl(msd_ctx *c, const IN *d_keys, uint64_t n, const uint64_t *d_bounds, uint32_t nbuckets, void *d_rec, uint64_t rec_bytes,
			   uint32_t *d_overflow)
// ... 1130 lines not shown
	if (n >= kMaxElems || m >= kMaxElems) return fail(c, MSD_EINVAL, "n or m too large: fewer than 2^36 elements each");
	if (outputs_overlap(buf, 2)) return fail(c, MSD_EINVAL, "d_out, d_out_origin and d_num_out must not overlap an input or each other (the operation is not in place)");
	HIPCHK(c, hipSetDevice(c->device));
	return with_width((int)es, [&](auto k0) {
		typedef decltype(k0) K;
		return set_sorted_impl<K>(c, op, (const K *)d_a, n, (const K *)d_b, m, key_type, cap, (K *)d_out, d_out_origin, d_num_out);
	});
}

}

template <typename K>
static int check_impl(msd_ctx *c, const K *k, const uint64_t *r, uint64_t n, uint64_t *viol, uint64_t *sum, uint64_t *xr)
{
	if (!c) return MSD_EINVAL;
	HIPCHK(c, hipSetDevice(c->device));
	int rc = slab_reserve(c, 4096);
	if (!rc) rc = pinned_reserve(c, 4096);
	if (rc) return rc;
	CheckResult *res = (CheckResult *)c->slab;
	HIPCHK(c, hipMemsetAsync(res, 0, sizeof *res, c->stream));
	if (n) {
		const unsigned grid = (unsigned)std::min<uint64_t>((uint64_t)c->sm_count * 8, (n + 255) / 256);
		LAUNCH(c, (check_kernel<K>), grid, 256, 0, k, r, n, res);
	}
	HIPCHK(c, hipMemcpyAsync(c->pinned, res, sizeof *res, hipMemcpyDeviceToHost, c->stream));
	HIPCHK(c, hipStreamSynchronize(c->stream));
	const CheckResult *h = (const CheckResult *)c->pinned;
	if (viol) *viol = h->violations;
	if (sum) *sum = h->sum;
	if (xr) *xr = h->xr;
	return MSD_OK;
}
extern "C" {

int msd_check_u32(msd_ctx *c, const uint32_t *k, uint64_t n, uint64_t *v, uint64_t *s, uint64_t *x) { return check_impl<uint32_t>(c, k, nullptr, n, v, s, x); }
int msd_check_u64(msd_ctx *c, const uint64_t *k, const uint64_t *r, uint64_t n, uint64_t *v, uint64_t *s, uint64_t *x) { return check_impl<uint64_t>(c, k, r, n, v, s, x); }

static unsigned gen_grid(const msd_ctx *c, uint64_t n) { return (unsigned)std::min<uint64_t>((uint64_t)c->sm_count * 16, (n + 255) / 256 + 1); }

int msd_gen_uniform_u32(msd_ctx *c, uint32_t *k, uint64_t n, uint64_t seed, uint64_t first)
{
	if (!c) return MSD_EINVAL;
	HIPCHK(c, hipSetDevice(c->device));
	LAUNCH(c, gen_uniform_u32_kernel, gen_grid(c, n), 256, 0, k, n, seed + first);
	return MSD_OK;
}
int msd_gen_uniform_u64(msd_ctx *c, uint64_t *k, uint64_t n, uint64_t seed, uint64_t first, int shr)
{
	if (!c) return MSD_EINVAL;
	HIPCHK(c, hipSetDevice(c->device));
	LAUNCH(c, gen_uniform_u64_kernel, gen_grid(c, n), 256, 0, k, n, seed + first, shr);
	return MSD_OK;
}
int msd_gen_zipf_u32(msd_ctx *c, uint32_t *k, uint64_t n, uint64_t seed, uint64_t first)
{
	if (!c) return MSD_EINVAL;
	HIPCHK(c, hipSetDevice(c->device));
	LAUNCH(c, gen_zipf_u32_kernel, gen_grid(c, n), 256, 0, k, n, seed + first);
	return MSD_OK;
}
int msd_gen_dup_u32(msd_ctx *c, uint32_t *k, uint64_t n, uint64_t seed, uint64_t first, uint64_t distinct)
{
	if (!c) return MSD_EINVAL;
	if (distinct == 0) return fail(c, MSD_EINVAL, "gen_dup: distinct must be positive");
	HIPCHK(c, hipSetDevice(c->device));
	LAUNCH(c, gen_dup_u32_kernel, gen_grid(c, n), 256, 0, k, n, seed + first, distinct);
	return MSD_OK;
}
int msd_gen_mt19937_64(msd_ctx *c, uint64_t *k, uint64_t n, uint64_t seed, int shr)
{
	if (!c) return MSD_EINVAL;
	if (shr < 0 || shr > 63) return fail(c, MSD_EINVAL, "gen_mt19937_64: shift_right must be 0..63");
	HIPCHK(c, hipSetDevice(c->device));
	if (n == 0) return MSD_OK;
	LAUNCH(c, gen_mt19937_64_kernel, 1, 320, 0, k, n, seed, shr);
	return MSD_OK;
}
int msd_gen_iota_u64(msd_ctx *c, uint64_t *v, uint64_t n, uint64_t first)
{
	if (!c) return MSD_EINVAL;
	HIPCHK(c, hipSetDevice(c->device));
	LAUNCH(c, gen_iota_u64_kernel, gen_grid(c, n), 256, 0, v, n, first);
	return MSD_OK;
}

}

template <typename K, typename V>
static int plan_describe(uint64_t n, int end_bit, int cus, msd_plan *out)
{
	using C = Cfg<K, V>;
	constexpr bool HV = has_val<V>::value;
	const uint64_t small_max = (uint64_t)C::SORT_TH * C::SORT_KPT;
	const uint32_t count_bits = HV ? (uint32_t)kLeafCountBits : (uint32_t)kCountMaxBits;
	memset(out, 0, sizeof *out);
	out->block_elems = C::B;
	out->tile_elems = C::T;
	out->leaf_capacity = small_max;
	out->leaf_count_bits = count_bits;
	if (n <= small_max || end_bit <= 0) return MSD_OK;
	std::vector<Segment> segs(1);
	segs[0] = { 0, n, (uint32_t)end_bit, 0 };
	RoundPlan rp;
	plan_round<K, V>(segs, small_max, cus, rp, count_bits);
	out->digit_width = rp.parents[0].width;
	out->digit_shift = rp.parents[0].shift;
	out->stripes = rp.stripes.size();
	out->stripe_elems = rp.stripes[0].end - rp.stripes[0].begin;
	uint64_t sz = n;
	uint32_t bits = (uint32_t)end_bit, rounds = 0;
	while (sz > small_max && bits > 0) {
		const uint32_t w = pick_width(sz, bits, small_max, count_bits);
		sz >>= w;
		bits -= w;
		++rounds;
	}
	out->expected_rounds = rounds;
	out->workspace_bytes = round_bytes_estimate<K, V>(n, cus) + keep_bytes_for<K, V>(n) + 4 * leaf_list_guess<K, V>(n) * sizeof(Segment);
	return MSD_OK;
}

extern "C" {

int msd_plan_first_round(uint64_t n, int key_bytes, int val_bytes, int end_bit, int cus, msd_plan *out)
{
	if (!out || cus <= 0 || end_bit < 0 || end_bit > key_bytes * 8) return MSD_EINVAL;
	const int rc = with_layout(key_bytes, val_bytes, [&](auto k, auto v) { return plan_describe<decltype(k), decltype(v)>(n, end_bit, cus, out); });
	return rc != kNoLayout ? rc : MSD_EINVAL;
}

int msd_set_option(msd_ctx *c, const char *name, int64_t value)
{
	if (!c || !name) return MSD_EINVAL;
	if (!strcmp(name, "direct_mode")) {
		if (value < 0 || value > 2) return fail(c, MSD_EINVAL, "direct_mode must be 0, 1 or 2");
		c->direct_mode = (int)value;
	} else if (!strcmp(name, "direct_min")) {
		if (value < 1) return fail(c, MSD_EINVAL, "direct_min must be positive");
		c->direct_min = (uint64_t)value;
	} else if (!strcmp(name, "regpart")) {
		c->regpart = value != 0;
	} else if (!strcmp(name, "count16")) {
		if (value < 0 || value > 2) return fail(c, MSD_EINVAL, "count16 must be 0, 1 or 2");
		c->count16 = (int)value;
	} else if (!strcmp(name, "leaf17")) {
		c->leaf17 = value != 0;
	} else if (!strcmp(name, "mid_leaf")) {
		c->mid_leaf = value != 0;
	} else if (!strcmp(name, "early_leaves")) {
		c->early_leaves = value != 0;
	} else if (!strcmp(name, "early_plan")) {
		c->early_plan = value != 0;
	} else if (!strcmp(name, "merge_leaf")) {
		if (value < 0 || value > 2) return fail(c, MSD_EINVAL, "merge_leaf must be 0, 1 or 2");
		c->merge_leaf = (int)value;
	} else if (!strcmp(name, "select_cap")) {
		if (value < 1 || value > ((int64_t)1 << 28)) return fail(c, MSD_EINVAL, "select_cap must be 1 .. 2^28 elements");
		c->select_cap = (uint64_t)value;
	} else if (!strcmp(name, "topk_rows_mode")) {
		if (value < 0 || value > 2) return fail(c, MSD_EINVAL, "topk_rows_mode must be 0, 1 or 2");
		c->topk_rows_mode = (int)value;
	} else if (!strcmp(name, "topk_rows_lanes")) {
		if (value != 0 && value != 64 && value != 256 && value != 1024) return fail(c, MSD_EINVAL, "topk_rows_lanes must be 0, 64, 256 or 1024");
		c->topk_rows_lanes = (int)value;
	} else if (!strcmp(name, "sort_rows_mode")) {
		if (value < 0 || value > 2) return fail(c, MSD_EINVAL, "sort_rows_mode must be 0, 1 or 2");
		c->sort_rows_mode = (int)value;
	} else if (!strcmp(name, "sort_rows_lanes")) {
		if (value != 0 && value != 64 && value != 256 && value != 1024) return fail(c, MSD_EINVAL, "sort_rows_lanes must be 0, 64, 256 or 1024");
		c->sort_rows_lanes = (int)value;
	} else if (!strcmp(name, "search_mode")) {
		if (value < 0 || value > 2) return fail(c, MSD_EINVAL, "search_mode must be 0, 1 or 2");
		c->search_mode = (int)value;
	} else if (!strcmp(name, "search_merge_ratio")) {
		if (value < 1) return fail(c, MSD_EINVAL, "search_merge_ratio must be at least 1");
		c->search_merge_ratio = (uint64_t)value;
	} else if (!strcmp(name, "direct_min_parent")) {
		if (value < 1) return fail(c, MSD_EINVAL, "direct_min_parent must be positive");
		c->direct_min_parent = (uint64_t)value;
	} else
		return fail(c, MSD_EINVAL, "unknown option %s", name);
	return MSD_OK;
}

#ifdef MSD_STAMPS
int msd_debug_stamps(uint64_t *out)
{
	unsigned long long h[2][16];
	if (hipMemcpyFromSymbol(h, HIP_SYMBOL(g_stamps), sizeof h) != hipSuccess) return MSD_EHIP;
	memcpy(out, h, sizeof h);
	memset(h, 0, sizeof h);
	if (hipMemcpyToSymbol(HIP_SYMBOL(g_stamps), h, sizeof h) != hipSuccess) return MSD_EHIP;
	return MSD_OK;
}
#endif

int msd_set_profiling(msd_ctx *c, int on)
{
	if (!c) return MSD_EINVAL;
	c->profiling = on != 0;
	return MSD_OK;
}
int msd_phase_count(const msd_ctx *c) { return c ? (int)c->phase_us.size() : 0; }
const char *msd_phase_name(const msd_ctx *c, int i) { return (c && i >= 0 && i < (int)c->phase_us.size()) ? c->phase_us[i].first.c_str() : ""; }
double msd_phase_us(const msd_ctx *c, int i) { return (c && i >= 0 && i < (int)c->phase_us.size()) ? c->phase_us[i].second : 0.0; }
int msd_stat(const msd_ctx *c, const char *name, uint64_t *v)
{
	if (!c || !name || !v) return MSD_EINVAL;
	const int fix_word = !strcmp(name, "sort_keys_split") ? kFixSplit : !strcmp(name, "sort_keys_reversed") ? kFixReversed : -1;
	if (fix_word >= 0) {
		if (c->fix_stats == 0) return MSD_EINVAL;
		*v = fix_word == kFixSplit ? c->fix_split : 0;
		if (c->fix_stats == 1) return MSD_OK;
		if (hipSetDevice(c->device) != hipSuccess || hipStreamSynchronize(c->stream) != hipSuccess ||
		    hipMemcpy(v, c->fix_plan + fix_word, sizeof *v, hipMemcpyDeviceToHost) != hipSuccess)
			return MSD_EHIP;
		return MSD_OK;
	}
	for (auto &s : c->stats)
		if (s.first == name) {
			*v = s.second;
			return MSD_OK;
		}
	return MSD_EINVAL;
}

}
```

Baseline: 156.6 Gkeys/s.

## Post kernel results to a host-mapped mailbox and plan round zero during vary scan

Kernels that produce small host-needed results (vary OR/AND, collect counters and next parents, count-walk counters) now have their last workgroup write them with system-scope stores into coherent host-mapped memory and post a sequence number. The host spin-waits on that word instead of issuing a memcpy plus stream or event synchronize. The front plan for round 0 is prepared while the vary kernel runs. The direct sample kernel is also reworked to use 16-byte vector loads and a grid sized to the CU count. The intent is to cut host-device round-trip latency between rounds, at the cost of last-block ticket atomics, host busy-polling and added complexity.

After: 157.7 Gkeys/s (median of 6 runs). Within noise of the previous version (+0.7%).

```diff
diff --git a/inplacemsdradixsort_amd/csrc/msd_device.hpp b/inplacemsdradixsort_amd/csrc/msd_device.hpp
--- a/inplacemsdradixsort_amd/csrc/msd_device.hpp
+++ b/inplacemsdradixsort_amd/csrc/msd_device.hpp
@@ -87,6 +87,8 @@
 	uint32_t l17_slow;
 	uint32_t err_sites;
 	uint32_t nexcess;
+	uint32_t mail_ticket;
+	uint32_t pad;
 };
 __device__ __forceinline__ void msd_note_error(Counters *ctr, uint32_t site)
 {
@@ -94,6 +96,45 @@
 	atomicOr(&ctr->err_sites, 1u << site);
 }
 static_assert(sizeof(Counters) % 8 == 0, "the words behind the counters are used for 64-bit atomics");
+
+constexpr uint32_t kMailSegs = 2048;
+struct MailFront { unsigned long long vor, vand, seq; };
+struct MailEarly { Counters ctr; Segment segs[kMailSegs]; unsigned long long seq; };
+struct MailEnd { Counters ctr, parked; unsigned long long seq; };
+struct Mailbox { MailFront front; MailEarly early; MailEnd end; };
+
+__device__ __forceinline__ bool mail_last_group(uint32_t *ticket, uint32_t *flag)
+{
+	asm volatile("s_waitcnt vmcnt(0)" ::: "memory");
+	__syncthreads();
+	if (threadIdx.x == 0) {
+		const bool last = atomicAdd(ticket, 1u) == gridDim.x * gridDim.y - 1u;
+		if (last) __hip_atomic_store(ticket, 0u, __ATOMIC_RELAXED, __HIP_MEMORY_SCOPE_AGENT);
+		*flag = last ? 1u : 0u;
+	}
+	__syncthreads();
+	const bool last = *flag != 0;
+	if (last) __builtin_amdgcn_fence(__ATOMIC_ACQUIRE, "agent");
+	return last;
+}
+__device__ __forceinline__ void mail_put(unsigned long long *dst, unsigned long long v) { __hip_atomic_store(dst, v, __ATOMIC_RELAXED, __HIP_MEMORY_SCOPE_SYSTEM); }
+__device__ __forceinline__ void mail_copy(void *dst, const void *src, uint32_t nwords)
+{
+	unsigned long long *d = static_cast<unsigned long long *>(dst);
+	const unsigned long long *s = static_cast<const unsigned long long *>(src);
+	for (uint32_t i = threadIdx.x; i < nwords; i += blockDim.x) mail_put(d + i, __hip_atomic_load(s + i, __ATOMIC_RELAXED, __HIP_MEMORY_SCOPE_AGENT));
+}
+__device__ __forceinline__ void mail_post(unsigned long long *seq_word, unsigned long long seq)
+{
+	asm volatile("s_waitcnt vmcnt(0)" ::: "memory");
+	__syncthreads();
+	if (threadIdx.x == 0) {
+		__threadfence_system();
+		asm volatile("s_waitcnt vmcnt(0)" ::: "memory");
+		mail_put(seq_word, seq);
+	}
+}
+static_assert(sizeof(Counters) % 8 == 0 && sizeof(Segment) % 8 == 0, "mail_copy moves 64-bit words");
 
 #ifdef MSD_STAMPS
 __device__ unsigned long long g_stamps[2][16];
@@ -227,31 +268,56 @@
 	uint32_t adj_seen, adj_same;
 };
 
+constexpr int kSampleLoads = 4;
+template <typename K> constexpr uint32_t kSampleRunsPerStep = kSampleLoads * Vec16<K>::N;
+typedef uint32_t u32x4_a4 __attribute__((ext_vector_type(4), aligned(4)));
+
 template <typename K>
 __global__ __launch_bounds__(256) void direct_sample_kernel(const K *__restrict__ keys, const Parent *__restrict__ parents,
 	DirectPlan *__restrict__ plan, uint32_t every)
 {
+	constexpr int VEC = Vec16<K>::N;
+	constexpr uint32_t LANES = 256 / VEC;
+	constexpr uint32_t RPW = 256 / LANES;
 	__shared__ uint32_t h[kP];
 	const Parent pa = parents[0];
 	const uint32_t mask = (1u << pa.width) - 1u;
 	h[threadIdx.x] = 0;
 	uint32_t seen = 0, same = 0;
 	__syncthreads();
-	const uint64_t nruns = pa.count / 256;
-	const uint64_t step = (uint64_t)gridDim.x * every;
-	for (uint64_t r = (uint64_t)blockIdx.x * every; r < nruns; r += 4 * step) {
-		K k4[4];
-#pragma unroll
-		for (int u = 0; u < 4; ++u)
-			if (r + u * step < nruns) k4[u] = keys[pa.start + (r + u * step) * 256 + threadIdx.x];
-#pragma unroll
-		for (int u = 0; u < 4; ++u) {
-			if (r + u * step < nruns) {
-				const uint32_t d = digit_of(k4[u], pa.shift, mask);
-				atomicAdd(&h[d], 1u);
-				if (u == 0 && (blockIdx.x & 7u) == 0) {
-					same += __popcll(__ballot(d == (uint32_t)__shfl_down((int)d, 1) && (threadIdx.x & 63) != 63));
-					seen += 63;
+	const uint64_t nruns = pa.count / 256, nsamp = (nruns + every - 1) / every;
+	const uint32_t sub = threadIdx.x / LANES;
+	const K *base = keys + pa.start + (uint64_t)(threadIdx.x % LANES) * VEC;
+	const uint64_t step = (uint64_t)gridDim.x * kSampleRunsPerStep<K>;
+	for (uint64_t m0 = (uint64_t)blockIdx.x * kSampleRunsPerStep<K>; m0 < nsamp; m0 += step) {
+		u32x4 q[kSampleLoads];
+#pragma unroll
+		for (int u = 0; u < kSampleLoads; ++u) {
+			const uint64_t m = m0 + (uint32_t)u * RPW + sub;
+			const u32x4_a4 *src = reinterpret_cast<const u32x4_a4 *>(base + (m < nsamp ? m : nsamp - 1) * every * 256);
+			q[u] = *src;
+		}
+#pragma unroll
+		for (int u = 0; u < kSampleLoads; ++u) {
+			const uint64_t m = m0 + (uint32_t)u * RPW + sub;
+			if (m < nsamp) {
+				uint32_t d[VEC];
+				if constexpr (VEC == 4) {
+					d[0] = digit_of((K)q[u].x, pa.shift, mask);
+					d[1] = digit_of((K)q[u].y, pa.shift, mask);
+					d[2] = digit_of((K)q[u].z, pa.shift, mask);
+					d[3] = digit_of((K)q[u].w, pa.shift, mask);
+				} else {
+					d[0] = digit_of((K)q[u].x | ((K)q[u].y << 32), pa.shift, mask);
+					d[1] = digit_of((K)q[u].z | ((K)q[u].w << 32), pa.shift, mask);
+				}
+#pragma unroll
+				for (int j = 0; j < VEC; ++j) atomicAdd(&h[d[j]], 1u);
+				if ((m & 31u) == 0) {
+					same += __popcll(__ballot(d[VEC - 1] == (uint32_t)__shfl_down((int)d[0], 1) && (threadIdx.x & 63) != 63));
+#pragma unroll
+					for (int j = 0; j + 1 < VEC; ++j) same += __popcll(__ballot(d[j] == d[j + 1]));
+					seen += 63 + 64 * (VEC - 1);
 				}
 			}
 		}
@@ -1173,9 +1239,10 @@
 __global__ __launch_bounds__(256) void collect_kernel(const Parent *__restrict__ parents, uint32_t nparents, uint32_t wmax, ChildArrays ca,
 	uint64_t small_max, uint64_t med_max, uint32_t small_cap, uint32_t count_bits, Segment *__restrict__ next_parents,
 	Segment *__restrict__ small, Segment *__restrict__ small_count, Segment *__restrict__ big, uint32_t big_cap,
-	Counters *__restrict__ ctr, uint64_t *__restrict__ count_out, uint32_t count_n, uint32_t stop_bits)
-{
-	__shared__ uint32_t s_n[4], s_base[4], s_max;
+	Counters *ctr, uint64_t *__restrict__ count_out, uint32_t count_n, uint32_t stop_bits, MailEarly *mail, uint32_t mail_segs,
+	unsigned long long seq)
+{
+	__shared__ uint32_t s_n[4], s_base[4], s_max, s_last;
 	const uint32_t tid = threadIdx.x;
 	if (tid < 4) s_n[tid] = 0;
 	if (tid == 0) s_max = 0;
@@ -1208,21 +1275,35 @@
 		if (tid == 3) atomicMax(&ctr->next_max, s_max);
 	}
 	__syncthreads();
-	if (which < 0) return;
-	uint32_t at = s_base[which] + rank;
-	if (which == 2 && at >= big_cap) {
-		which = 3;
-		at = atomicAdd(&ctr->next_parents, 1u);
-		atomicMax(&ctr->next_max, (uint32_t)(s.count < 0xFFFFFFFFull ? s.count : 0xFFFFFFFFull));
-	}
-	if (which == 3)
-		next_parents[at] = s;
-	else if (which == 2)
-		big[at] = s;
-	else if (at < small_cap)
-		(which == 0 ? small : small_count)[at] = s;
-	else
-		msd_note_error(ctr, 6u);
+	if (which >= 0) {
+		uint32_t at = s_base[which] + rank;
+		if (which == 2 && at >= big_cap) {
+			which = 3;
+			at = atomicAdd(&ctr->next_parents, 1u);
+			atomicMax(&ctr->next_max, (uint32_t)(s.count < 0xFFFFFFFFull ? s.count : 0xFFFFFFFFull));
+		}
+		if (which == 3) {
+			if (mail) {
+				unsigned long long *w = reinterpret_cast<unsigned long long *>(next_parents + at);
+				__hip_atomic_store(w, (unsigned long long)s.start, __ATOMIC_RELAXED, __HIP_MEMORY_SCOPE_AGENT);
+				__hip_atomic_store(w + 1, (unsigned long long)s.count, __ATOMIC_RELAXED, __HIP_MEMORY_SCOPE_AGENT);
+				__hip_atomic_store(w + 2, (unsigned long long)s.bits, __ATOMIC_RELAXED, __HIP_MEMORY_SCOPE_AGENT);
+			} else
+				next_parents[at] = s;
+		} else if (which == 2)
+			big[at] = s;
+		else if (at < small_cap)
+			(which == 0 ? small : small_count)[at] = s;
+		else
+			msd_note_error(ctr, 6u);
+	}
+	if (!mail) return;
+	if (mail_last_group(&ctr->mail_ticket, &s_last)) {
+		const uint32_t nnext = __hip_atomic_load(&ctr->next_parents, __ATOMIC_RELAXED, __HIP_MEMORY_SCOPE_AGENT);
+		mail_copy(&mail->ctr, ctr, sizeof(Counters) / 8);
+		mail_copy(mail->segs, next_parents, (nnext < mail_segs ? nnext : mail_segs) * (uint32_t)(sizeof(Segment) / 8));
+		mail_post(&mail->seq, seq);
+	}
 }
 
 }
@@ -1381,9 +1462,9 @@
 }
 
 template <typename K>
-__global__ __launch_bounds__(kCountTh, 8) void count_walk_kernel(K *__restrict__ keys,
+__device__ __forceinline__ void count_walk_segments(K *__restrict__ keys,
 	const Segment *__restrict__ segs, const uint32_t *__restrict__ nsegs_dev, Segment *__restrict__ fallback,
-	uint32_t fallback_base, uint32_t lds_cap, Segment *__restrict__ big, uint32_t big_cap, Counters *__restrict__ ctr)
+	uint32_t fallback_base, uint32_t lds_cap, Segment *__restrict__ big, uint32_t big_cap, Counters *ctr)
 {
 	constexpr uint32_t WS = kCountStageBytes / sizeof(K);
 	extern __shared__ __attribute__((aligned(16))) unsigned char smem[];
@@ -1496,6 +1577,24 @@
 		if (nxt >= nsegs) break;
 		sg = segs[nxt];
 		__syncthreads();
+	}
+}
+
+template <typename K>
+__global__ __launch_bounds__(kCountTh, 8) void count_walk_kernel(K *__restrict__ keys,
+	const Segment *__restrict__ segs, const uint32_t *__restrict__ nsegs_dev, Segment *__restrict__ fallback,
+	uint32_t fallback_base, uint32_t lds_cap, Segment *__restrict__ big, uint32_t big_cap, Counters *ctr, MailEnd *mail,
+	const Counters *park, unsigned long long seq)
+{
+	count_walk_segments<K>(keys, segs, nsegs_dev, fallback, fallback_base, lds_cap, big, big_cap, ctr);
+	if (!mail) return;
+	extern __shared__ __attribute__((aligned(16))) unsigned char smem[];
+	uint32_t *last = reinterpret_cast<uint32_t *>(smem + kCountCwBytes + kCountStageBytes) + 21;
+	__syncthreads();
+	if (mail_last_group(&ctr->mail_ticket, last)) {
+		mail_copy(&mail->ctr, ctr, sizeof(Counters) / 8);
+		if (park) mail_copy(&mail->parked, park, sizeof(Counters) / 8);
+		mail_post(&mail->seq, seq);
 	}
 }
 
@@ -1761,6 +1860,7 @@
 		ctr->next_max = 0;
 		ctr->rp_children = 0;
 		ctr->nhot = 0;
+		ctr->mail_ticket = 0;
 		scan_ctr[0] = scan_ctr[1] = scan_ctr[2] = scan_ctr[3] = 0;
 	}
 	for (uint64_t i = i0; i < nplan_words; i += step) plan_words[i] = 0;
@@ -2128,7 +2228,7 @@
 
 template <typename K>
 __global__ __launch_bounds__(256) void vary_kernel(const K *__restrict__ keys, uint64_t n, uint64_t stride,
-	unsigned long long *__restrict__ res)
+	unsigned long long *res, MailFront *mail, unsigned long long seq)
 {
 	K o = 0, a = ~(K)0;
 	const uint64_t cnt = (n + stride - 1) / stride;
@@ -2178,6 +2278,17 @@
 	if (lane_id() == 0) {
 		atomicOr(&res[0], (unsigned long long)o);
 		atomicAnd(&res[1], (unsigned long long)a | (sizeof(K) == 4 ? 0xFFFFFFFF00000000ull : 0ull));
+	}
+	if (!mail) return;
+	__shared__ uint32_t s_last;
+	if (mail_last_group(reinterpret_cast<uint32_t *>(res + 2), &s_last)) {
+		if (threadIdx.x == 0) {
+			mail_put(&mail->vor, __hip_atomic_load(&res[0], __ATOMIC_RELAXED, __HIP_MEMORY_SCOPE_AGENT));
+			mail_put(&mail->vand, __hip_atomic_load(&res[1], __ATOMIC_RELAXED, __HIP_MEMORY_SCOPE_AGENT));
+			__hip_atomic_store(&res[0], 0ull, __ATOMIC_RELAXED, __HIP_MEMORY_SCOPE_AGENT);
+			__hip_atomic_store(&res[1], ~0ull, __ATOMIC_RELAXED, __HIP_MEMORY_SCOPE_AGENT);
+		}
+		mail_post(&mail->seq, seq);
 	}
 }
 
diff --git a/inplacemsdradixsort_amd/csrc/msd_radix.hip b/inplacemsdradixsort_amd/csrc/msd_radix.hip
--- a/inplacemsdradixsort_amd/csrc/msd_radix.hip
+++ b/inplacemsdradixsort_amd/csrc/msd_radix.hip
@@ -22,6 +22,7 @@
 #include <cstdarg>
 #include <cstdio>
 #include <cstring>
+#include <chrono>
 #include <initializer_list>
 #include <string>
 #include <type_traits>
@@ -48,6 +49,10 @@
 	void *pinned = nullptr;
 	size_t pinned_bytes = 0;
 	hipEvent_t ev_early = nullptr;
+	Mailbox *mail = nullptr, *mail_dev = nullptr;
+	uint64_t mail_seq = 0;
+	unsigned long long *front_acc = nullptr;
+	int mailbox = 1;
 	std::string err;
 	bool profiling = false;
 	hipEvent_t ev_start = nullptr;
@@ -241,6 +246,25 @@
 	HIPCHK(c, hipStreamSynchronize(c->stream));
 	memcpy(&hc, c->pinned, sizeof hc);
 	return MSD_OK;
+}
+
+static int wait_mailbox(msd_ctx *c, const unsigned long long *word, unsigned long long seq, const char *area)
+{
+	using clock = std::chrono::steady_clock;
+	const auto arrived = [&] { return __atomic_load_n(word, __ATOMIC_ACQUIRE) == seq; };
+	auto asked = clock::now();
+	for (uint32_t spins = 0;; ++spins) {
+		if (arrived()) return MSD_OK;
+		__builtin_ia32_pause();
+		if (spins % 32 != 31 || clock::now() - asked < std::chrono::microseconds(40)) continue;
+		const hipError_t e = hipStreamQuery(c->stream);
+		if (e == hipSuccess) {
+			if (arrived()) return MSD_OK;
+			return fail(c, MSD_EINTERNAL, "mailbox: the stream has drained and no answer %llu has reached the %s area", seq, area);
+		}
+		if (e != hipErrorNotReady) return fail(c, MSD_EHIP, "waiting for the mailbox's %s area: %s", area, hipGetErrorString(e));
+		asked = clock::now();
+	}
 }
 
 template <typename T> static int fetch(msd_ctx *c, const T *src, size_t count, std::vector<T> &out)
@@ -634,12 +658,21 @@
 		HIPCHK(c, hipMemsetAsync(vres + 1, 0xFF, sizeof(unsigned long long), c->stream));
 		return MSD_OK;
 	}
-	int run_vary(uint64_t stride, uint64_t *vary_out)
-	{
-		if (int rc = vres_init()) return rc;
+	int run_vary(uint64_t stride, uint64_t *vary_out) { return run_vary(stride, vary_out, [] { return MSD_OK; }); }
+	template <typename F> int run_vary(uint64_t stride, uint64_t *vary_out, F &&meanwhile)
+	{
 		const uint64_t cnt = (n + stride - 1) / stride;
 		const unsigned grid = (unsigned)std::min<uint64_t>((uint64_t)c->sm_count * 8, (cnt + 255) / 256);
-		LAUNCH(c, (vary_kernel<K>), grid, 256, 0, keys, n, stride, vres);
+		if (c->mailbox) {
+			const unsigned long long seq = ++c->mail_seq;
+			LAUNCH(c, (vary_kernel<K>), grid, 256, 0, keys, n, stride, c->front_acc, &c->mail_dev->front, seq);
+			if (int rc = meanwhile()) return rc;
+			if (int rc = wait_mailbox(c, &c->mail->front.seq, seq, "front")) return rc;
+			*vary_out = c->mail->front.vor ^ c->mail->front.vand;
+			return MSD_OK;
+		}
+		if (int rc = vres_init()) return rc;
+		LAUNCH(c, (vary_kernel<K>), grid, 256, 0, keys, n, stride, vres, nullptr, 0);
 		HIPCHK(c, hipMemcpyAsync(c->pinned, vres, 2 * sizeof(unsigned long long), hipMemcpyDeviceToHost, c->stream));
 		HIPCHK(c, hipStreamSynchronize(c->stream));
 		const unsigned long long *h = (const unsigned long long *)c->pinned;
@@ -651,7 +684,7 @@
 	{
 		if (job.single_pass() || job.segmented() || cur.empty() || n < 4096) return MSD_OK;
 		uint64_t vary = 0;
-		int rc = run_vary(std::max<uint64_t>(1, n / 8192), &vary);
+		int rc = run_vary(std::max<uint64_t>(1, n / 8192), &vary, [this] { return plan_round0_ahead(); });
 		if (rc) return rc;
 		vary &= low_mask;
 		const int top_sample = vary ? 64 - __builtin_clzll(vary) : 0;
@@ -740,8 +773,11 @@
 					}
 				}
 			}
-			Round r;
-			if ((rc = plan_upload(r)) || (rc = classify(r)) || (rc = permute_blocks(r)) || (rc = cleanup_collect(r)) ||
+			const bool planned = ahead0_valid && round == 0 && cur.size() == 1 && cur[0].bits == ahead0_bits;
+			ahead0_valid = false;
+			Round fresh;
+			Round &r = planned ? ahead0 : fresh;
+			if ((!planned && (rc = plan_reserve(r))) || (rc = plan_upload(r, planned)) || (rc = classify(r)) || (rc = permute_blocks(r)) || (rc = cleanup_collect(r)) ||
 			    (rc = r.leaves_follow ? early_summary(r) : r.plan_ahead ? plan_next_early(r) : round_summary(r)))
 				return rc;
 		}
@@ -821,7 +857,7 @@
 		phase_mark(c, "A register partition");
 		LAUNCH(c, collect_kernel, (np + (256u >> wmax) - 1) / (256u >> wmax), 256, 0, d_parents, np, wmax, ca, small_max, small_max,
 		       std::min<size_t>(c->lists_cap, 0xFFFFFFFFu), count_bits, d_next, small(), small_count(), HV ? nullptr : big, big_cap, ctr,
-		       nullptr, nc, job.stop_bits);
+		       nullptr, nc, job.stop_bits, nullptr, 0, 0);
 		phase_mark(c, "C cleanup");
 		Counters hc;
 		const size_t ahead = std::min<size_t>(next_cap, 2048);
@@ -850,9 +886,11 @@
 		bool hist_checks = false;
 		bool leaves_follow = false;
 		size_t plan_ahead = 0;
+		unsigned long long mail_seq = 0;
 	};
 	static constexpr size_t kReadAhead = 2048, kSegOff = 256, kVresOff = kSegOff - 2 * sizeof(unsigned long long);
 	static constexpr size_t kEarlyOff = kSegOff + kReadAhead * sizeof(Segment), kStagingBytes = kEarlyOff + sizeof(Counters);
+	static_assert(kReadAhead == kMailSegs, "the mailbox's early area holds the next parents that travel early");
 	static_assert(sizeof(Counters) <= kVresOff, "counters and the OR/AND words share the head of the staging buffer");
 	static constexpr size_t kPlanCtrOff = (kStagingBytes + 255) / 256 * 256, kPlanSegOff = kPlanCtrOff + 256;
 	static constexpr size_t kParkOff = kPlanSegOff + kReadAhead * sizeof(Segment), kStage2Off = (kParkOff + sizeof(Counters) + 255) / 256 * 256;
@@ -872,10 +910,9 @@
 	{
 		plan_round<K, V>(segs, small_max, c->sm_count, rp, count_bits, job.single_pass() ? job.width : 0u, job.splitters ? job.nsplit : 0u);
 	}
-	int plan_upload(Round &r)
+	int plan_reserve(Round &r)
 	{
 		const bool ahead = enqueue_ahead;
-		enqueue_ahead = false;
 		plan_next(cur, r.rp);
 		const bool first = round == 0;
 		int rc = slab_carve(c, [&](Bump &b) { carve_round<K, V>(b, r.rp, small_max, r.rb); },
@@ -887,16 +924,36 @@
 			for (size_t i = 0; i < r.np && r.leaves_follow; ++i) r.leaves_follow = r.rp.parents[i].shift <= count_bits;
 		}
 		if ((rc = lists_reserve(c, (size_t)std::max(nsmall_host, ncount_host) + r.nc + 16, nsmall_host, ncount_host))) return rc;
+		const size_t next_stripes = (size_t)std::max<uint64_t>((uint64_t)c->sm_count * MSD_STRIPE_WANT, n >> MSD_STRIPE_CAP_LOG) + 2 * kReadAhead + 64;
+		const size_t want = !ahead && c->early_plan && !job.single_pass() ? stage2_bytes(kReadAhead, next_stripes) : 0;
+		return pinned_reserve(c, std::max({ kStagingBytes, r.np * sizeof(Parent) + r.ns * sizeof(Stripe), want }));
+	}
+
+	Round ahead0;
+	uint32_t ahead0_bits = 0;
+	bool ahead0_valid = false;
+	int plan_round0_ahead()
+	{
+		if (cur.size() != 1 || n <= small_max || (!HV && cur[0].bits <= count_bits)) return MSD_OK;
+		if constexpr (sizeof(K) == 8)
+			if (c->regpart && n + 1 <= kRpCap) return MSD_OK;
+		if (int rc = plan_reserve(ahead0)) return rc;
+		ahead0_bits = cur[0].bits;
+		ahead0_valid = true;
+		return MSD_OK;
+	}
+
+	int plan_upload(Round &r, bool staging_idle = false)
+	{
+		const bool ahead = enqueue_ahead;
+		enqueue_ahead = false;
 		{
 			static_assert(sizeof(Parent) % 4 == 0 && sizeof(Stripe) % 4 == 0, "the plan travels as 32-bit words");
 			const uint64_t plan_words = (r.np <= kDirectMaxParents ? r.np : 1) * sizeof(DirectPlan) / sizeof(uint32_t);
 			const uint64_t ntiles = (r.nc + kScanTile - 1) / kScanTile + 1;
 			const uint64_t parent_words = r.np * sizeof(Parent) / 4, stripe_words = r.ns * sizeof(Stripe) / 4;
-			const size_t next_stripes = (size_t)std::max<uint64_t>((uint64_t)c->sm_count * MSD_STRIPE_WANT, n >> MSD_STRIPE_CAP_LOG) + 2 * kReadAhead + 64;
-			const size_t want = !ahead && c->early_plan && !job.single_pass() ? stage2_bytes(kReadAhead, next_stripes) : 0;
-			if ((rc = pinned_reserve(c, std::max({ kStagingBytes, r.np * sizeof(Parent) + r.ns * sizeof(Stripe), want })))) return rc;
 			char *stage = (char *)c->pinned + (ahead ? kStage2Off : 0);
-			if (!ahead) HIPCHK(c, hipStreamSynchronize(c->stream));
+			if (!ahead && !staging_idle) HIPCHK(c, hipStreamSynchronize(c->stream));
 			memcpy(stage, r.rp.parents.data(), r.np * sizeof(Parent));
 			memcpy(stage + r.np * sizeof(Parent), r.rp.stripes.data(), r.ns * sizeof(Stripe));
 			void *staged = nullptr;
@@ -931,7 +988,8 @@
 		if (np == 1) {
 			const uint64_t nruns = rp.parents[0].count / 256;
 			const uint32_t every = (uint32_t)std::min<uint64_t>(64, std::max<uint64_t>(1, nruns / 16384));
-			const uint32_t sgrid = (uint32_t)std::min<uint64_t>(1024, std::max<uint64_t>(1, nruns / every / 4));
+			const uint64_t nsamp = (nruns + every - 1) / every;
+			const uint32_t sgrid = (uint32_t)std::min<uint64_t>((uint64_t)c->sm_count * 4, std::max<uint64_t>(1, (nsamp + kSampleRunsPerStep<K> - 1) / kSampleRunsPerStep<K>));
 			LAUNCH(c, (direct_sample_kernel<K>), sgrid, 256, 0, keys, rb.parents, rb.plans, every);
 		} else {
 			r.hist_checks = unverified && rp.round_keys == n;
@@ -1018,17 +1076,21 @@
 		uint32_t wmax = 1;
 		for (size_t i = 0; i < np; ++i) wmax = std::max(wmax, r.rp.parents[i].width);
 		const uint32_t small_cap = (uint32_t)std::min<size_t>(c->lists_cap, 0xFFFFFFFFu);
+		if (!r.leaves_follow && c->early_plan && !sp && !r.hist_checks && !parked.open && c->pinned_bytes >= kStage2Off && may_leave_parents(r))
+			r.plan_ahead = std::min<size_t>(r.rp.round_keys / (small_max + 1) + 2, kReadAhead);
+		if (c->mailbox && (r.leaves_follow || r.plan_ahead)) r.mail_seq = ++c->mail_seq;
 		LAUNCH(c, collect_kernel, (np + (256u >> wmax) - 1) / (256u >> wmax), 256, 0, rb.parents, np, wmax, rb.ca,
 		       sp ? ~0ull : small_max, (HV || sp) ? small_max : std::max<uint64_t>(small_max, kCountMedMax),
 		       small_cap, sp ? 0u : count_bits,
 		       rb.next_parents, small(), small_count(), (HV || sp) ? nullptr : big, big_cap, ctr,
-		       (sp && job.counts) ? job.counts : nullptr, job.splitters ? job.nsplit + 1u : nc, job.stop_bits);
+		       (sp && job.counts) ? job.counts : nullptr, job.splitters ? job.nsplit + 1u : nc, job.stop_bits,
+		       r.mail_seq ? &c->mail_dev->early : nullptr, r.plan_ahead, r.mail_seq);
+		if (r.mail_seq) return MSD_OK;
 		if (r.leaves_follow) {
 			if (!c->ev_early) HIPCHK(c, hipEventCreateWithFlags(&c->ev_early, hipEventDisableTiming));
 			HIPCHK(c, hipMemcpyAsync((char *)c->pinned + kEarlyOff, ctr, sizeof(Counters), hipMemcpyDeviceToHost, c->stream));
 			HIPCHK(c, hipEventRecord(c->ev_early, c->stream));
-		} else if (c->early_plan && !sp && !r.hist_checks && !parked.open && c->pinned_bytes >= kStage2Off && may_leave_parents(r)) {
-			r.plan_ahead = std::min<size_t>(r.rp.round_keys / (small_max + 1) + 2, kReadAhead);
+		} else if (r.plan_ahead) {
 			if (!c->ev_early) HIPCHK(c, hipEventCreateWithFlags(&c->ev_early, hipEventDisableTiming));
 			HIPCHK(c, hipMemcpyAsync((char *)c->pinned + kPlanCtrOff, ctr, sizeof(Counters), hipMemcpyDeviceToHost, c->stream));
 			HIPCHK(c, hipMemcpyAsync((char *)c->pinned + kPlanSegOff, rb.next_parents, r.plan_ahead * sizeof(Segment), hipMemcpyDeviceToHost, c->stream));
@@ -1064,27 +1126,40 @@
 		set_stat(c, "excess_blocks", hc.nexcess);
 	}
 
-	int parked_summary()
+	int parked_summary(const Counters *from = nullptr)
 	{
 		if (!parked.open) return MSD_OK;
 		parked.open = false;
 		Counters pc;
-		memcpy(&pc, (char *)c->pinned + kParkOff, sizeof pc);
+		memcpy(&pc, from ? (const void *)from : (const void *)((char *)c->pinned + kParkOff), sizeof pc);
 		if (pc.errors) return round_errors(pc, parked.round, parked.np, parked.ns, parked_direct ? "used" : "not used");
 		round_stats(pc, parked.np, parked.ns, parked.nc, parked.nslots);
 		return MSD_OK;
 	}
 	ToHost parked_piece() const { return { kParkOff, park(), parked.open ? sizeof(Counters) : 0 }; }
 
+	int early_answer(const Round &r, size_t ctr_off, size_t seg_off, Counters &hc, const Segment *&sg)
+	{
+		if (r.mail_seq) {
+			if (int rc = wait_mailbox(c, &c->mail->early.seq, r.mail_seq, "early")) return rc;
+			memcpy(&hc, &c->mail->early.ctr, sizeof hc);
+			sg = c->mail->early.segs;
+		} else {
+			HIPCHK(c, hipEventSynchronize(c->ev_early));
+			memcpy(&hc, (char *)c->pinned + ctr_off, sizeof hc);
+			sg = (const Segment *)((char *)c->pinned + seg_off);
+		}
+		return MSD_OK;
+	}
+
 	int plan_next_early(Round &r)
 	{
-		HIPCHK(c, hipEventSynchronize(c->ev_early));
 		Counters hc;
-		memcpy(&hc, (char *)c->pinned + kPlanCtrOff, sizeof hc);
+		const Segment *sg = nullptr;
+		if (int rc = early_answer(r, kPlanCtrOff, kPlanSegOff, hc, sg)) return rc;
 		bool ok = !hc.errors && hc.next_parents != 0 && hc.next_parents <= r.plan_ahead;
 		std::vector<Segment> next;
 		if (ok) {
-			const Segment *sg = (const Segment *)((char *)c->pinned + kPlanSegOff);
 			next.assign(sg, sg + hc.next_parents);
 			sort_by_start(next);
 			if constexpr (sizeof(K) == 8) {
@@ -1122,9 +1197,9 @@
 
 	int early_summary(Round &r)
 	{
-		HIPCHK(c, hipEventSynchronize(c->ev_early));
 		Counters hc;
-		memcpy(&hc, (char *)c->pinned + kEarlyOff, sizeof hc);
+		const Segment *sg = nullptr;
+		if (int rc = early_answer(r, kEarlyOff, kSegOff, hc, sg)) return rc;
 		if (hc.next_parents || hc.ncount == 0 || hc.errors) return round_summary(r);
 		prev_direct = r.tried_direct && (hc.direct_uneven == 0 || c->direct_mode == 2);
 		if (prev_direct) add_stat(c, "direct_rounds", 1);
@@ -1235,10 +1310,17 @@
 					walk_list = slow2;
 				}
 			}
-			LAUNCH(c, (count_walk_kernel<K>), count_grid, kCountTh, kCountLds, keys, walk_list, walk_n, small(), nsmall_host, small_max, big, big_cap, ctr);
+			const unsigned long long seq = c->mailbox ? ++c->mail_seq : 0;
+			LAUNCH(c, (count_walk_kernel<K>), count_grid, kCountTh, kCountLds, keys, walk_list, walk_n, small(), nsmall_host, small_max, big, big_cap, ctr,
+			       seq ? &c->mail_dev->end : nullptr, seq && parked.open ? park() : nullptr, seq);
 			phase_mark(c, "count sort");
 			Counters hc;
-			if ((rc = read_counters(c, ctr, hc, { parked_piece() })) || (rc = parked_summary())) return rc;
+			if (seq) {
+				if ((rc = wait_mailbox(c, &c->mail->end.seq, seq, "end"))) return rc;
+				memcpy(&hc, &c->mail->end.ctr, sizeof hc);
+				if ((rc = parked_summary(&c->mail->end.parked))) return rc;
+			} else if ((rc = read_counters(c, ctr, hc, { parked_piece() })) || (rc = parked_summary()))
+				return rc;
 			if (pending.open) {
 				pending.open = false;
 				if (hc.errors && (hc.err_sites & ~0x80u || !hc.err_sites))
@@ -1524,6 +1606,21 @@
 }
 
 
+static int mailbox_create(msd_ctx *c)
+{
+	void *host = nullptr, *dev = nullptr;
+	if (hipHostMalloc(&host, sizeof(Mailbox), hipHostMallocMapped | hipHostMallocCoherent) != hipSuccess)
+		return fail(c, MSD_ENOMEM, "mailbox hipHostMalloc failed");
+	c->mail = static_cast<Mailbox *>(host);
+	memset(host, 0, sizeof(Mailbox));
+	HIPCHK(c, hipHostGetDevicePointer(&dev, host, 0));
+	c->mail_dev = static_cast<Mailbox *>(dev);
+	const unsigned long long preset[4] = { 0ull, ~0ull, 0ull, 0ull };
+	if (hipMalloc((void **)&c->front_acc, sizeof preset) != hipSuccess) return fail(c, MSD_ENOMEM, "accumulator hipMalloc failed");
+	HIPCHK(c, hipMemcpy(c->front_acc, preset, sizeof preset, hipMemcpyHostToDevice));
+	return MSD_OK;
+}
+
 extern "C" {
 
 const char *msd_version(void) { return MSD_VERSION; }
@@ -1558,8 +1655,12 @@
 	if (!rc) rc = with_layout(8, 8, attrs);
 	if (!rc) rc = set_row_kernels_lds_attrs(c);
 	if (!rc && hipMalloc((void **)&c->fix_plan, kFixWords * sizeof(uint64_t)) != hipSuccess) rc = fail(c, MSD_ENOMEM, "plan words hipMalloc failed");
+	if (!rc) rc = mailbox_create(c);
 	if (rc) {
 		fprintf(stderr, "msd_create: %s\n", c->err.c_str());
+		if (c->fix_plan) (void)hipFree(c->fix_plan);
+		if (c->front_acc) (void)hipFree(c->front_acc);
+		if (c->mail) (void)hipHostFree(c->mail);
 		delete c;
 		return rc;
 	}
@@ -1578,6 +1679,8 @@
 	if (c->sel) (void)hipFree(c->sel);
 	if (c->rows_stage) (void)hipFree(c->rows_stage);
 	if (c->fix_plan) (void)hipFree(c->fix_plan);
+	if (c->front_acc) (void)hipFree(c->front_acc);
+	if (c->mail) (void)hipHostFree(c->mail);
 	if (c->pinned) (void)hipHostFree(c->pinned);
 	if (c->ev_start) (void)hipEventDestroy(c->ev_start);
 	if (c->ev_early) (void)hipEventDestroy(c->ev_early);
@@ -3014,6 +3117,8 @@
 		c->early_leaves = value != 0;
 	} else if (!strcmp(name, "early_plan")) {
 		c->early_plan = value != 0;
+	} else if (!strcmp(name, "mailbox")) {
+		c->mailbox = value != 0;
 	} else if (!strcmp(name, "merge_leaf")) {
 		if (value < 0 || value > 2) return fail(c, MSD_EINVAL, "merge_leaf must be 0, 1 or 2");
 		c->merge_leaf = (int)value;
```
